# ikergarcia1996/AI-Generated-GTAV

Hardware: AMD Instinct MI355X
Metric: generated frames/sec (32-frame clip, 100 noise steps) (higher is better)
Workload: dtype fp16 (fp32 accumulate/residual)

## Files before the change

ai-generated-gtav_amd/csrc/api.hip:

```cpp
#include "api_internal.h"

#include <type_traits>

namespace gtav_shared {
thread_local hipEvent_t g_launch_ev[2] = {nullptr, nullptr};
static thread_local char g_err[1024] = "";
void set_error(const char* fmt, ...) {
    va_list ap;
    va_start(ap, fmt);
    vsnprintf(g_err, sizeof(g_err), fmt, ap);
    va_end(ap);
}
const char* last_error() { return g_err; }
}

namespace {
template <class T> struct twin_arg { typedef T type; };
template <> struct twin_arg<const f16*> { typedef const __bf16* type; };
template <> struct twin_arg<f16*> { typedef __bf16* type; };
#define GTAV_TWIN_STRUCT(S)                                                                                                                     \
    static_assert(sizeof(S) == sizeof(gtav_bf16::S) && alignof(S) == alignof(gtav_bf16::S) && std::is_standard_layout<S>::value &&             \
                      std::is_standard_layout<gtav_bf16::S>::value, #S ": the fp16 and the bf16 view differ");                                  \
    template <> struct twin_arg<const S&> { typedef const gtav_bf16::S& type; };                                                                \
    template <> struct twin_arg<const S*> { typedef const gtav_bf16::S* type; };
// ... 260 lines not shown
int gtav_op_gemm_dw_grouped(int32_t n, const void* const* x, const void* const* w, float* const* out, const int32_t* M, const int32_t* N, const int32_t* ldo,
                            int32_t K, void* stream) {
    GTAV_REQUIRE(n >= 1 && n <= GEMM_DW_MAX_GROUPS && x && w && out && M && N && ldo, "op_gemm_dw_grouped: 1 .. %d groups", GEMM_DW_MAX_GROUPS);
    GemmDwGroup g[GEMM_DW_MAX_GROUPS];
    for (int i = 0; i < n; ++i) g[i] = GemmDwGroup{(const f16*)x[i], (const f16*)w[i], out[i], M[i], N[i], ldo[i]};
    return op_ops().gemm_dw_grouped(g, n, K, nullptr, (hipStream_t)stream, false);
}
int gtav_op_gemm_splitk_ln(const void* x, int32_t ldx, const void* w, const float* bias, int32_t M, int32_t N, int32_t K,
                           int32_t splitk, float* parts, float* resid, const float* gate, int32_t gate_stride,
                           int32_t rows_per_gate, void* out_f16, const float* shift, const float* scale, int32_t mod_stride,
                           void* stream) {
    GemmParams g = gemm_params((const f16*)x, ldx, (const f16*)w, M, N, K);
    g.out = parts; g.ldo = N;
    g.splitk = splitk > 0 ? splitk : gemm_choose_splitk(M, N, K);
    RET_IF(op_ops().gemm(g, EPI_PARTIAL, (hipStream_t)stream));
    LnPending pd;
    memset(&pd, 0, sizeof(pd));
    pd.parts = parts; pd.nsplit = g.splitk; pd.slab_stride = (size_t)M * N; pd.ld = N; pd.bias = bias; pd.gate = gate;
    pd.gate_stride = gate_stride; pd.rows_per_gate = rows_per_gate;
    return op_ops().ln_modulate(resid, N, (f16*)out_f16, N, M, N, shift, scale, mod_stride, nullptr, rows_per_gate, &pd, nullptr, (hipStream_t)stream);
}
int gtav_op_ln_pending(int32_t mode, float* x, int32_t ldx, void* out, int32_t M, int32_t D, const float* p0, const float* p1, int32_t mod_stride,
                       const int32_t* rows, int32_t rows_per_mod, const float* parts, int32_t nsplit, int64_t slab_stride, int32_t ld,
                       const float* bias, const float* gate, int32_t gate_stride, const int32_t* gate_rows, int32_t rows_per_gate, float* x_out, void* y_save,
                       int32_t tperm_T, int32_t tperm_P, float* k_save, const float* k_load, int32_t* err, void* stream) {
    LnPending pd;
    memset(&pd, 0, sizeof(pd));
    pd.parts = parts; pd.nsplit = nsplit; pd.slab_stride = (size_t)slab_stride; pd.ld = ld; pd.bias = bias; pd.gate = gate;
    pd.gate_stride = gate_stride; pd.gate_rows = gate_rows; pd.rows_per_gate = rows_per_gate; pd.x_out = x_out; pd.y_save = (f16*)y_save;
    pd.tperm_T = tperm_T; pd.tperm_P = tperm_P; pd.k_save = k_save; pd.k_load = k_load;
    if (mode == 0) return op_ops().ln_modulate(x, ldx, (f16*)out, D, M, D, p0, p1, mod_stride, rows, rows_per_mod, &pd, err, (hipStream_t)stream);
    return op_ops().ln_affine(x, ldx, (f16*)out, D, M, D, p0, p1, &pd, err, (hipStream_t)stream);
}
int gtav_op_branch_rows(const float* parts, int32_t nsplit, int64_t slab_stride, int32_t ld, const float* bias, void* y, int32_t M, int32_t N, int32_t* err,
                        void* stream) {
    return op_ops().branch_rows(parts, nsplit, (size_t)slab_stride, ld, bias, (f16*)y, M, N, err, (hipStream_t)stream);
}
int gtav_op_rope_interleave(const float* cos_t, const float* sin_t, float* cs, int32_t npos, void* stream) {
    return launch_rope_interleave(cos_t, sin_t, cs, npos, (hipStream_t)stream);
}
int gtav_op_gemm_choose_splitk(int32_t M, int32_t N, int32_t K) { return gemm_choose_splitk(M, N, K); }
int gtav_op_gemm_resid_inplace(int32_t M, int32_t N, int32_t K) { return gemm_resid_inplace_ok(M, N, K, 0) ? 1 : 0; }
int gtav_op_gemm_plan(int32_t M, int32_t N, int32_t K, int32_t epilogue, int32_t qkv_mode, int32_t S, int32_t splitk, int32_t rows_per_gate, int32_t* plan8) {
    static_assert(sizeof(gtav_shared::GemmPlan) == 8 * sizeof(int32_t), "plan8 is the GemmPlan");
    GTAV_REQUIRE(plan8, "op_gemm_plan: null argument");
    return gtav_shared::gemm_plan(gtav_shared::GemmProblem{M, N, K, epilogue, qkv_mode, S, splitk, rows_per_gate}, (gtav_shared::GemmPlan*)plan8);
}
void gtav_op_gemm_set_stages(int32_t ns) { gtav_shared::gemm_set_stages(ns); }
#ifdef GTAV_EXPERIMENTS
void gtav_op_gemm_set_debug(int32_t bits) { gtav_shared::gemm_set_debug(bits); }
void gtav_op_gemm_set_stamps(void* buf_dev, int32_t max_blocks) { gemm_set_stamps((unsigned long long*)buf_dev, max_blocks); }
#endif
void gtav_op_gemm_set_wm(int32_t wm) { gtav_shared::gemm_set_wm(wm); }
void gtav_op_set_operand_dtype(int32_t dtype) { g_op_bf16 = dtype == GTAV_OPERAND_BF16; }

int gtav_timer_calibrate(int32_t spin_us, int32_t reps, double* event_us_mean, double* device_us_mean, void* stream) {
    GTAV_REQUIRE(spin_us >= 0 && spin_us <= 1000 && reps >= 1 && reps <= 256 && event_us_mean && device_us_mean, "timer_calibrate: bad argument");
    hipStream_t s = (hipStream_t)stream;
    unsigned long long* dev = nullptr;
    GTAV_CHECK_HIP(hipMalloc(&dev, sizeof(unsigned long long) * reps));
    std::vector<hipEvent_t> ev(2 * reps, nullptr);
    int rc = 0;
    for (int i = 0; i < 2 * reps && !rc; ++i)
        if (hipEventCreate(&ev[i]) != hipSuccess) { set_error("timer_calibrate: hipEventCreate failed"); rc = 1; }
    if (!rc) rc = launch_calib_spin((unsigned long long)spin_us * 100ull, dev, s);
    if (!rc && hipStreamSynchronize(s) != hipSuccess) { set_error("timer_calibrate: synchronize failed"); rc = 1; }
// ... 137 lines not shown
```

ai-generated-gtav_amd/csrc/api_dit.hip:

```cpp
#include "api_internal.h"

#ifdef GTAV_EXPERIMENTS
static int fold_alloc(gtav_dit* h) {
    gtav_dit::Fold& f = h->fold;
    if (f.ok) return 0;
    GTAV_REQUIRE(f.geom_ok, "dit_set_fold: this geometry has no LayerNorm fold (tokens per frame %d must be a multiple of 16 and >= 64, hidden %% 256 == 0)", h->P);
    Arena& a = h->arena;
    const int D = h->D;
    const size_t Mx = round_up(h->Mmax, 128);
    int rc = 0;
#define A_(expr) do { if (!rc) rc = (expr); } while (0)
    {
        const int nhb = h->L * 2, nseam = 2 * nhb + 1;
        f.col_c.assign(nseam, 0);
        int col = 0;
        for (int hb = 0; hb < nhb; ++hb) { f.col_c[2 * hb + 1] = col; col += 2 * h->Hm; }
        for (int hb = 0; hb < nhb; ++hb) { f.col_c[2 * hb] = col; col += 2 * 3 * D; }
        f.col_c[2 * nhb] = col; col += 2 * h->Nfin;
        f.CTW = col;
        f.n_groups = 2 * nseam; f.n_groups_a = 2 * nhb;
        f.Rp = round_up(h->max_rows, 128);
        A_(a.alloc_t(&f.ctab, (size_t)h->max_rows * f.CTW));
        A_(a.alloc_t(&f.ctab_cur, (size_t)h->maxB * h->maxT * f.CTW));
        A_(a.alloc_t(&f.stats, Mx * (size_t)(D / 64) * 2));
// ... 92 lines not shown
    const gtav_dit* h;
    int M, Tq, t0;
    bool on;
    DitPrefetch(const gtav_dit* h_, int M_, int Tq_, int t0_) : h(h_), M(M_), Tq(Tq_), t0(t0_) {
        const int pf_max_m = 1536;
        static const int pf_min_m = GTAV_ENV_INT("GTAV_PF_MIN_M", 256);
        on = h->w_prefetch && M >= pf_min_m && M <= pf_max_m;
        fill_on = M <= pf_max_m;
    }
    bool fill_on;
    int fill(int cls) const { return fill_on ? h->w_fill_cls[cls] : 0; }
    PrefetchDesc after(int hb, int pos) const {
        const int q = pos + 1, hb2 = hb + q / 4, consumer = (q + 3) % 4;
        if (!on || hb2 >= 2 * h->L) return kNoPrefetch;
        const int v = h->w_prefetch_cls[consumer];
        if (!v) return kNoPrefetch;
        const gtav_dit::Half& w2 = h->halves[hb2];
        const int D = h->D;
        const f16* W; int N, K, sk = 1;
        if (consumer == 3) { W = dit_half_fused(h, hb2, M, Tq, t0) ? w2.w_qkv_hm : w2.w_qkv; N = 3 * D; K = D; }
        else if (consumer == 0) { W = w2.w_out; N = D; K = D; sk = gemm_choose_splitk(M, D, D); }
        else if (consumer == 1) { W = w2.w_fc1; N = h->Hm; K = D; }
        else { W = w2.w_fc2; N = D; K = h->Hm_pad; sk = gemm_choose_splitk(M, D, h->Hm_pad); }
        const int nkt = K / 64;
        if (sk < 1 || nkt % sk || (sk >= 8 ? sk % 8 : 8 % sk)) sk = 1;
        return PrefetchDesc{W, cdiv(N, 128), nkt, sk, v >= 2 ? v : 0};
    }
};

static bool dit_resid_inplace(const gtav_dit* h, int M, int K) {
    return gemm_pp_ok(M, h->D, K, EPI_RESID) || (gemm_choose_splitk(M, h->D, K) == 1 && M >= h->resid_inplace_min_m) || gemm_resid_inplace_ok(M, h->D, K, h->P);
}

static int dit_forward_core(gtav_dit* h, const float* x_src, const int* frame_index, int B, int Tq, int t0,
                            const float* mod, const int* mod_rows, const float* ctab, float* v_out, hipStream_t s) {
    const int D = h->D, P = h->P, NB = B * Tq, M = NB * P;
    GTAV_REQUIRE(M <= h->Mmax, "forward: %d tokens exceed workspace (%d)", M, h->Mmax);
    bool fold_a, fold_b;
    fold_policy(h, M, fold_a, fold_b);
    const DitPrefetch pf(h, M, Tq, t0);
    DeferredResid rd{h->parts, h->parts_rows * (size_t)D, h->resid, M, D, &h->prof, s};
    auto gate = [&](const float* g) { return ResidGate{g, h->MODW, mod_rows, P}; };
    auto ln = [&](const OperandOps& o, const float* shift, const float* scale, int* ef) -> int {
        PROF(h, PC_LN, s, o.ln_modulate(h->resid, D, h->xn, D, M, D, shift, scale, h->MODW, mod_rows, P, rd.take(), ef, s));
        return 0;
    };
    const int g_embed = 2 * h->L, g_final = 2 * h->L + 1;
    PROF(h, PC_OTHER, s, h->ops(g_embed).patchify(x_src, frame_index, NB, h->C, h->H, h->W, h->p, h->xp, h->Kpe, 1.f, 0.f, h->err_of(g_embed), s));
    GemmParams pe = gemm_params(h->xp, h->Kpe, h->w_pe, M, D, h->Kpe);
    pe.bias = h->b_pe; pe.out = h->resid; pe.ldo = D;
    PROF(h, PC_OTHER, s, h->ops(g_embed).gemm(pe, EPI_F32, s));
    bool folded_in = false;
    for (int hb = 0; hb < 2 * h->L; ++hb) {
        const int l = hb / 2, hf = hb % 2;
        const gtav_dit::Half& w = h->halves[hb];
        const OperandOps& ops = h->ops(hb);
        int* const ef = h->err_of(hb);
        const float* mb = mod + (size_t)hb * 6 * D;
        const bool fused = dit_half_fused(h, hb, M, Tq, t0), fused_t = fused && hf == 1, fused_s = fused && hf == 0 && !folded_in;
        if (fused_t) rd.permute_rows(Tq, P);
        if (!folded_in) RET_IF(ln(ops, mb, mb + D, ef));
        GemmParams g = gemm_params(h->xn, D, fused_t || fused_s ? w.w_qkv_hm : w.w_qkv, M, 3 * D, D);
        g.D = D; g.S = P; g.err_flag = ef; g.pf = pf.after(hb, 0); g.wfill = pf.fill(3);
        if (folded_in) fold_consumer(h, g, 2 * hb, 3 * D, mod_rows, ctab);
        if (hf == 0) { g.qkv_mode = QKV_SPATIAL; g.rope_cs = h->rope_s.cs_dev; }
        else { g.qkv_mode = QKV_TEMPORAL; g.k = h->kvcache[l]; g.v = h->kvcache[l]; g.Tq = Tq; g.t0 = t0; g.Tmax = h->maxT; g.rope_cs = h->rope_t.cs_dev; }
        if (fused_t || fused_s) {
            g.out = h->ao; g.ldo = D;
            if (fused_t) PROF(h, PC_ATTN_T, s, launch_gemm_qkvt_attn(g, s));
            else PROF(h, PC_ATTN_S, s, launch_gemm_qkvs_attn(g, s));
        } else {
            if (hf == 0) { g.q = h->qs; g.k = h->ks; g.v = h->vts; }
            else g.q = h->qt;
            PROF(h, PC_QKV, s, ops.gemm(g, folded_in ? EPI_QKV_FOLD : EPI_QKV, s));
            if (hf == 0) PROF(h, PC_ATTN_S, s, ops.attn_spatial(h->qs, h->ks, h->vts, h->ao, NB, h->heads, P, s, false));
            else PROF(h, PC_ATTN_T, s, ops.attn_temporal(h->qt, h->kvcache[l], h->ao, B, P, D, Tq, t0, h->maxT, s));
        }
        folded_in = false;
        GemmParams fc1 = gemm_params(h->xn, D, w.w_fc1, M, h->Hm, D);
        fc1.bias = w.b_fc1; fc1.out = h->hbuf; fc1.ldo = h->Hm_pad; fc1.err_flag = ef; fc1.pf = pf.after(hb, 2); fc1.wfill = pf.fill(1);
        if (fold_a) {
            RET_IF(fold_producer(h, PC_OUT, h->ao, w.w_out, M, D, w.b_out, gate(mb + 2 * D), mb + 4 * D, s));
            fold_consumer(h, fc1, 2 * hb + 1, h->Hm, mod_rows, ctab);
            PROF(h, PC_FC1, s, launch_gemm(fc1, EPI_GELU_TANH_FOLD, s));
        } else {
            RET_IF(rd.gemm(ops, PC_OUT, h->ao, D, w.w_out, D, w.b_out, gate(mb + 2 * D), dit_resid_inplace(h, M, D), pf.after(hb, 1), nullptr, nullptr, pf.fill(0)));
            RET_IF(ln(ops, mb + 3 * D, mb + 4 * D, ef));
            PROF(h, PC_FC1, s, ops.gemm(fc1, EPI_GELU_TANH, s));
        }
        if (fold_b) {
            const float* next_scale = hb + 1 < 2 * h->L ? mod + (size_t)(hb + 1) * 6 * D + D : mod + (size_t)h->L * 12 * D + D;
            RET_IF(fold_producer(h, PC_FC2, h->hbuf, w.w_fc2, M, h->Hm_pad, w.b_fc2, gate(mb + 5 * D), next_scale, s));
            folded_in = true;
        } else {
            RET_IF(rd.gemm(ops, PC_FC2, h->hbuf, h->Hm_pad, w.w_fc2, h->Hm_pad, w.b_fc2, gate(mb + 5 * D), dit_resid_inplace(h, M, h->Hm_pad), pf.after(hb, 3), nullptr, nullptr, pf.fill(2)));
        }
    }
    const float* mf = mod + (size_t)h->L * 12 * D;
    if (!folded_in) RET_IF(ln(h->ops(g_final), mf, mf + D, h->err_of(g_final)));
    GemmParams fin = gemm_params(h->xn, D, h->w_final, M, h->Nfin, D);
    fin.bias = h->b_final; fin.out = h->fo; fin.ldo = h->Nfin;
    if (folded_in) fold_consumer(h, fin, 4 * h->L, h->Nfin, mod_rows, ctab);
    PROF(h, PC_OTHER, s, h->ops(g_final).gemm(fin, folded_in ? EPI_F32_FOLD : EPI_F32, s));
    PROF(h, PC_OTHER, s, launch_unpatchify(h->fo, h->Nfin, v_out, NB, h->C, h->H, h->W, h->p, 0, 1.f, 0.f, s));
    return h->prof.collect(s);
}

extern "C" {

int gtav_dit_create(const gtav_dit_config* c, gtav_dit** out) {
    GTAV_REQUIRE(c && out, "dit_create: null argument");
    GTAV_REQUIRE(c->hidden_size % 256 == 0 && c->hidden_size <= 2048, "hidden_size=%d must be a multiple of 256, <= 2048", c->hidden_size);
    GTAV_REQUIRE(c->num_heads > 0 && c->hidden_size / c->num_heads == 64 && c->hidden_size % c->num_heads == 0,
                 "only head_dim 64 is implemented (hidden %d, heads %d)", c->hidden_size, c->num_heads);
    GTAV_REQUIRE(c->input_h % c->patch_size == 0 && c->input_w % c->patch_size == 0, "input %dx%d not divisible by patch %d",
                 c->input_h, c->input_w, c->patch_size);
    GTAV_REQUIRE(c->max_frames >= 1 && c->max_frames <= 32, "max_frames=%d must be in [1, 32]", c->max_frames);
    GTAV_REQUIRE(c->max_batch >= 1 && c->depth >= 1, "bad max_batch/depth");
    RET_IF(skinny_init());
    gtav_dit* h = new gtav_dit();
    h->cfg = *c;
    h->D = c->hidden_size; h->L = c->depth; h->heads = c->num_heads; h->C = c->in_channels; h->p = c->patch_size;
    h->H = c->input_h; h->W = c->input_w; h->gh = h->H / h->p; h->gw = h->W / h->p; h->P = h->gh * h->gw;
    const int D = h->D;
    if ((h->P % 8) != 0) {
        set_error("tokens per frame P=%d must be a multiple of 8", h->P);
        delete h;
        return 2;
    }
    h->Hm = (int)(D * c->mlp_ratio); h->Hm_pad = round_up(h->Hm, 128);
    h->A = c->external_cond_dim > 0 ? c->external_cond_dim : 0; h->Apad = round_up(h->A > 0 ? h->A : 1, 32);
    h->MODW = h->L * 12 * D + 2 * D;
    h->Kpe = round_up(h->C * h->p * h->p, 64);
    h->Nfin = h->p * h->p * h->C;
    h->maxB = c->max_batch; h->maxT = c->max_frames; h->Mmax = h->maxB * h->maxT * h->P;
    h->max_rows = c->max_cond_rows > h->maxB * h->maxT ? c->max_cond_rows : h->maxB * h->maxT;
    Arena& a = h->arena;
// ... 143 lines not shown
    }
    RET_IF(launch_rope_interleave(h->rope_s.cos_dev, h->rope_s.sin_dev, h->rope_s.cs_dev, h->P, s));
    RET_IF(launch_rope_interleave(h->rope_t.cos_dev, h->rope_t.sin_dev, h->rope_t.cs_dev, h->maxT, s));
    GTAV_CHECK_HIP(hipStreamSynchronize(s));
    h->finalized = true;
    return 0;
}

int gtav_dit_forward(gtav_dit* h, const float* x, const int64_t* t, const float* actions, float* out, int32_t B, int32_t T,
                     void* stream) {
    GTAV_REQUIRE(h && x && t && out, "dit_forward: null argument");
    GTAV_REQUIRE(h->finalized, "dit_forward: call gtav_dit_finalize first");
    GTAV_REQUIRE(B >= 1 && B <= h->maxB && T >= 1 && T <= h->maxT, "dit_forward: B=%d T=%d outside capacity (%d, %d)", B, T, h->maxB, h->maxT);
    GTAV_REQUIRE(!actions || h->A > 0, "dit_forward: model has no external_cond");
    hipStream_t s = (hipStream_t)stream;
    h->prepared.valid = false;
    h->kvrec.valid = false;
    RET_IF(dit_cond(h, t, B * T, 1, nullptr, 0, actions, h->A, 0, s));
    return dit_forward_core(h, x, nullptr, B, T, 0, h->mod, nullptr, h->fold.ctab, out, s);
}

int gtav_dit_set_schedule(gtav_dit* h, const float* ac, int32_t n) {
    GTAV_REQUIRE(h && ac && n == 1000, "dit_set_schedule: expected 1000 alphas_cumprod values");
    h->ac_host.assign(ac, ac + n);
    GTAV_CHECK_HIP(hipMemcpy(h->ac_table, ac, n * sizeof(float), hipMemcpyHostToDevice));
    return 0;
}

static int denoise_step_body(gtav_dit* h, float* x, int B, int F, int T, const float* actions, int mode, float* v_out,
                             bool prepared, hipStream_t s) {
    const size_t fsz = (size_t)h->C * h->H * h->W;
    const int Tq = mode == 1 ? 1 : T, t0 = mode == 1 ? T - 1 : 0;
    if (!prepared) RET_IF(dit_cond(h, nullptr, B * Tq, Tq, h->step_dev, mode == 1, actions, (int64_t)F * h->A, h->A, s));
    RET_IF(dit_forward_core(h, x, h->frame_idx, B, Tq, t0, prepared ? h->mod_cur : h->mod, nullptr, prepared ? h->fold.ctab_cur : h->fold.ctab, h->vout, s));
    const float* vlast = h->vout + (size_t)(Tq - 1) * fsz;
    RET_IF(launch_ddim_update_step(x, F, vlast, (size_t)Tq * fsz, B, (int)fsz, h->step_dev, s));
    if (v_out) RET_IF(launch_copy_rows_f32(vlast, (size_t)Tq * fsz, v_out, fsz, B, fsz, s));
    return 0;
}

int gtav_dit_prepare_frame(gtav_dit* h, int32_t B, int32_t F, int32_t start, int32_t cur, int32_t t_ctx,
                           const int32_t* t_steps_host, int32_t n_steps, const float* actions, void* stream) {
    GTAV_REQUIRE(h && t_steps_host, "prepare_frame: null argument");
    GTAV_REQUIRE(h->finalized, "prepare_frame: finalize the model first");
    const int T = cur - start + 1;
    GTAV_REQUIRE(start >= 0 && cur < F && T >= 1 && T <= h->maxT && B >= 1 && B <= h->maxB && n_steps >= 1 && n_steps <= 1024,
                 "prepare_frame: bad window [%d, %d] / steps %d", start, cur, n_steps);
    GTAV_REQUIRE(!actions || h->A > 0, "prepare_frame: model has no external_cond");
    const int rows = B * (T - 1) + n_steps * B;
    GTAV_REQUIRE(rows <= h->max_rows, "prepare_frame: %d conditioning rows exceed max_cond_rows %d", rows, h->max_rows);
    hipStream_t s = (hipStream_t)stream;
    GTAV_CHECK_HIP(hipStreamSynchronize(s));
    GTAV_CHECK_HIP(hipMemcpy(h->t_steps_dev, t_steps_host, n_steps * sizeof(int), hipMemcpyHostToDevice));
    RET_IF(launch_cond_inputs_frame(rows, B, T, F, start, cur, t_ctx, h->t_steps_dev, h->sincos, h->E, actions, h->A, h->HC, h->D + h->Apad,
                                    h->D, h->Apad, h->err_flag, s));
    RET_IF(dit_cond_mlp(h, rows, actions != nullptr, s));
    {
        bool fa, fb, fa1, fb1;
        fold_policy(h, B * T * h->P, fa, fb);
        fold_policy(h, B * h->P, fa1, fb1);
        RET_IF(dit_fold_tables(h, rows, fa || fa1, fb || fb1, s));
        h->prepared.fold_tables = fa || fa1 || fb || fb1;
    }
    GTAV_CHECK_HIP(hipMemsetAsync(h->mod_last, 0xFF, (size_t)h->maxB * h->maxT * sizeof(int), s));
    h->prepared.valid = true; h->prepared.B = B; h->prepared.F = F; h->prepared.start = start; h->prepared.cur = cur;
    h->prepared.n_steps = n_steps; h->prepared.actions = actions;
    return 0;
// ... 70 lines not shown

int gtav_dit_set_graph(gtav_dit* h, int32_t enable) {
    GTAV_REQUIRE(h, "dit_set_graph: null handle");
    h->use_graph = enable != 0;
    return 0;
}

int gtav_dit_set_weight_prefetch(gtav_dit* h, int32_t enable) {
    GTAV_REQUIRE(h, "dit_set_weight_prefetch: null handle");
    GTAV_REQUIRE(enable == 0 || enable == 1 || (enable >> 16) == 1,
                 "dit_set_weight_prefetch: mode %d (0 off, 1 on, 0x10000 | per-class nibbles: bits 0-3 out-proj's weight, 4-7 fc1's, 8-11 fc2's, 12-15 to_qkv's; "
                 "nibble 0 = not prefetched, 1 = the whole slice, k >= 2 = the first k K tiles of every row tile)", enable);
    int cls[4];
    for (int c = 0; c < 4; ++c) cls[c] = enable == 0 ? 0 : enable == 1 ? 1 : (enable >> (4 * c)) & 15;
    const bool on = cls[0] || cls[1] || cls[2] || cls[3];
    if (h->w_prefetch != on || memcmp(cls, h->w_prefetch_cls, sizeof(cls))) h->drop_graphs();
    h->w_prefetch = on;
    memcpy(h->w_prefetch_cls, cls, sizeof(cls));
    return 0;
}

int gtav_dit_set_weight_fill_policy(gtav_dit* h, int32_t mode) {
    GTAV_REQUIRE(h, "dit_set_weight_fill_policy: null handle");
    GTAV_REQUIRE((mode & ~0x1111) == 0,
                 "dit_set_weight_fill_policy: mode %d (one nibble per class: bits 0-3 out-proj's weight, 4-7 fc1's, 8-11 fc2's, 12-15 to_qkv's; "
                 "nibble 0 = default cache policy, 1 = non-temporal fills)", mode);
    int cls[4];
    for (int c = 0; c < 4; ++c) cls[c] = (mode >> (4 * c)) & 15;
    if (memcmp(cls, h->w_fill_cls, sizeof(cls))) h->drop_graphs();
    memcpy(h->w_fill_cls, cls, sizeof(cls));
    return 0;
}

#ifdef GTAV_EXPERIMENTS
int gtav_dit_set_fold(gtav_dit* h, int32_t mode, int32_t min_tokens_a, int32_t min_tokens_b) {
    GTAV_REQUIRE(h && mode >= 0 && mode <= 2, "dit_set_fold: mode %d", mode);
    if (min_tokens_a >= 0) h->fold.min_m_a = min_tokens_a;
    if (min_tokens_b >= 0) h->fold.min_m_b = min_tokens_b;
    if (mode == 2 || (mode == 1 && (h->fold.min_m_a < (1 << 30) || h->fold.min_m_b < (1 << 30)))) RET_IF(fold_alloc(h));
    h->drop_graphs();
    h->prepared.valid = false;
    h->fold.mode = mode;
    return 0;
}
#endif

static int dit_set_fused(gtav_dit* h, bool& flag, int hf, bool geom_ok, bool enable) {
    if (flag != enable) h->drop_graphs();
    if (enable && geom_ok) {
        for (int l = 0; l < h->L; ++l) {
            gtav_dit::Half& w = h->halves[l * 2 + hf];
            if (w.w_qkv_hm) continue;
            RET_IF(h->arena.alloc_t(&w.w_qkv_hm, (size_t)3 * h->D * h->D));
            if (h->finalized) RET_IF(launch_qkv_head_major(w.w_qkv, w.w_qkv_hm, h->D, nullptr, hf ? 0 : 1));
        }
        if (h->finalized) GTAV_CHECK_HIP(hipDeviceSynchronize());
    }
    flag = enable;
    return 0;
}
int gtav_dit_set_fused_temporal(gtav_dit* h, int32_t enable) {
    GTAV_REQUIRE(h, "dit_set_fused_temporal: null handle");
    return dit_set_fused(h, h->fuse_tattn, 1, h->P % 16 == 0 && h->D % 256 == 0 && h->maxT >= 5, enable != 0);
}
int gtav_dit_set_fused_spatial(gtav_dit* h, int32_t enable) {
    GTAV_REQUIRE(h, "dit_set_fused_spatial: null handle");
// ... 96 lines not shown
```

ai-generated-gtav_amd/csrc/api_internal.h:

```cpp
#pragma once
#include "../../include/gtav_amd.h"
#include "../../include/gtav_amd_testing.h"
#include "ops.h"
#include "ops_bf16.h"

#include <cmath>
#include <cstdarg>
#include <cstdio>
#include <cstdlib>
#include <cstring>
#include <map>
#include <string>
#include <tuple>
#include <vector>

using namespace gtav;

#define RET_IF(expr)            \
    do {                        \
        int _rc = (expr);       \
        if (_rc) return _rc;    \
    } while (0)

namespace gtav {
// ... 202 lines not shown
#define PROF(h, c, s, expr)            \
    do {                               \
        RET_IF((h)->prof.begin(c, s)); \
        RET_IF(expr);                  \
        RET_IF((h)->prof.end(s));      \
    } while (0)

inline int report_err_flag(int flag, const char* who) {
    GTAV_REQUIRE(!(flag & ERR_TIMESTEP), "%s: a timestep outside [0, 999] was passed", who);
    GTAV_REQUIRE(!(flag & ERR_NONFINITE), "%s: a NaN or inf was found in the input tensor", who);
    GTAV_REQUIRE(!(flag & ERR_F16_SAT), "%s: an activation exceeded the fp16 range (|x| > 65504) and was saturated; results since the "
                 "last check are finite but clipped (the reference runs this path in bf16, which has fp32 range)", who);
    return 0;
}

inline GemmParams gemm_params(const f16* X, int ldx, const f16* W, int M, int N, int K) {
    GemmParams g;
    memset(&g, 0, sizeof(g));
    g.X = X; g.ldx = ldx; g.W = W; g.M = M; g.N = N; g.K = K;
    return g;
}

const PrefetchDesc kNoPrefetch{nullptr, 0, 0, 0, 0};

struct ResidGate { const float* gate; int stride; const int* rows; int rows_per_gate; };
struct DeferredResid {
    float* parts; size_t parts_floats;
    float* resid;
    int M, N;
    Profiler* prof;
    hipStream_t s;
    LnPending pend;
    bool pending = false;
    int gemm(const OperandOps& ops, int cls, const f16* X, int ldx, const f16* W, int K, const float* bias, const ResidGate& gt, bool inplace,
             const PrefetchDesc& pf = kNoPrefetch, float* x_out = nullptr, f16* y_save = nullptr, int wfill = 0) {
        GemmParams q = gemm_params(X, ldx, W, M, N, K);
        q.out = parts; q.ldo = N; q.pf = pf; q.wfill = wfill;
        if (inplace) {
            q.out = resid; q.bias = bias; q.gate = gt.gate; q.gate_stride = gt.stride; q.gate_rows = gt.rows; q.rows_per_gate = gt.rows_per_gate;
        } else {
            q.splitk = gemm_choose_splitk(M, N, K);
            GTAV_REQUIRE((size_t)q.splitk * M * N <= parts_floats, "split-K slabs exceed workspace");
        }
        if (prof) RET_IF(prof->begin(cls, s));
        RET_IF(ops.gemm(q, inplace ? EPI_RESID : EPI_PARTIAL, s));
        if (prof) RET_IF(prof->end(s));
        pending = !inplace;
        if (inplace) return 0;
        memset(&pend, 0, sizeof(pend));
        pend.parts = parts; pend.nsplit = q.splitk; pend.slab_stride = (size_t)M * N; pend.ld = N; pend.bias = bias;
        pend.gate = gt.gate; pend.gate_stride = gt.stride; pend.gate_rows = gt.rows; pend.rows_per_gate = gt.rows_per_gate;
        pend.x_out = x_out; pend.y_save = y_save;
        return 0;
    }
    const LnPending* take() {
        const bool was = pending;
        pending = false;
        return was ? &pend : nullptr;
    }
    void permute_rows(int T, int P) {
        if (!pending) memset(&pend, 0, sizeof(pend));
        pend.tperm_T = T; pend.tperm_P = P;
        pending = true;
    }
    void save_shift(float* k) { pend.k_save = k; }
    int load_shift(const float* k) {
        GTAV_REQUIRE(!pending, "train_block_forward: a re-run starts from a stored block input");
        memset(&pend, 0, sizeof(pend));
        pend.k_load = k;
        pending = true;
// ... 20 lines not shown
    bool sincos_set = false;
    RopeTable rope_s, rope_t;
    std::vector<float> freqs_s, freqs_t;
    float *freqs_s_dev = nullptr, *freqs_t_dev = nullptr;
    f16 *xp, *xn, *qs, *ks, *vts, *qt, *ao, *hbuf;
    std::vector<f16*> kvcache;
    float *resid, *fo, *vout, *E, *HC, *Sc, *mod, *parts;
    size_t parts_rows = 0;
    int* err_flag = nullptr;
    std::vector<unsigned char> grp_bf16;
    int n_groups = 0;
    bool any_bf16 = false;
    const OperandOps& ops(int g) const { return operand_ops(grp_bf16[g] != 0); }
    int* err_of(int g) const { return err_flag + 4 + g; }
    int* frame_idx = nullptr;
    StepParams* step_dev = nullptr;
    int* mod_rows_dev = nullptr;
    float* mod_cur = nullptr;
    int *mod_last = nullptr, *mod_changed = nullptr;
    int* t_steps_dev = nullptr;
    struct { bool valid = false, fold_tables = false; int B = 0, F = 0, start = 0, cur = 0, n_steps = 0; const float* actions = nullptr; } prepared;
    struct { bool valid = false; int B = 0, F = 0, start = 0, cur = 0; const void* x = nullptr; } kvrec;
    struct GraphKey {
        int B, F, T, mode;
        const void *x, *actions, *vout;
        bool operator<(const GraphKey& o) const {
            return std::tie(B, F, T, mode, x, actions, vout) < std::tie(o.B, o.F, o.T, o.mode, o.x, o.actions, o.vout);
        }
    };
    std::map<GraphKey, hipGraphExec_t> graphs;
    bool use_graph = true;
    bool fuse_tattn = false;
    bool fuse_sattn = false;
    bool w_prefetch = true;
    int w_prefetch_cls[4] = {1, 4, 4, 1};
    int w_fill_cls[4] = {0, 0, 0, 0};
    int resid_inplace_min_m = GTAV_ENV_INT("GTAV_RESID_INPLACE_MIN_M", 1 << 30);
    struct Fold {
        bool geom_ok = false;
        bool ok = false;
        int mode = 1;
        int min_m_a = 1 << 30, min_m_b = 1 << 30;
        int CTW = 0, n_groups = 0, n_groups_a = 0, Rp = 0;
        std::vector<int> col_c;
        float *ctab = nullptr, *ctab_cur = nullptr, *stats = nullptr;
        f16* sx = nullptr;
        GemmGroup* groups_dev = nullptr;
        int *gcol_dev = nullptr, *gscale_dev = nullptr;
    } fold;
    hipStream_t cap_stream = nullptr;
    void drop_graphs() {
        for (auto& kv : graphs)
            if (kv.second) (void)hipGraphExecDestroy(kv.second);
        graphs.clear();
    }
    ~gtav_dit() {
        drop_graphs();
        if (cap_stream) (void)hipStreamDestroy(cap_stream);
    }
    float* ac_table = nullptr;
    std::vector<float> ac_host;
    bool finalized = false;
    struct Train {
        bool on = false, have_fwd = false, have_actions = false;
        bool bf16 = false;
        bool mixed = false;
// ... 37 lines not shown
```

ai-generated-gtav_amd/csrc/common.h:

```cpp
#pragma once
#include <hip/hip_runtime.h>
#include <hip/hip_fp16.h>
#include <hip/hip_ext.h>
#include <stdint.h>

#ifdef GTAV_BF16_OPERANDS
#define GTAV_F16_T __bf16
#else
#define GTAV_F16_T _Float16
#endif

namespace gtav {

typedef GTAV_F16_T f16;
typedef GTAV_F16_T f16x4 __attribute__((ext_vector_type(4)));
typedef GTAV_F16_T f16x8 __attribute__((ext_vector_type(8)));
typedef GTAV_F16_T f16x2 __attribute__((ext_vector_type(2)));
typedef float f32x4 __attribute__((ext_vector_type(4)));
typedef float f32x16 __attribute__((ext_vector_type(16)));

__device__ __forceinline__ f32x4 mfma16(f16x8 a, f16x8 b, f32x4 c, int, int, int) {
#ifdef GTAV_BF16_OPERANDS
    return __builtin_amdgcn_mfma_f32_16x16x32_bf16(a, b, c, 0, 0, 0);
#else
// ... 50 lines not shown
#define GTAV_REQUIRE(cond, ...)                                                           \
    do {                                                                                  \
        if (!(cond)) {                                                                    \
            gtav::set_error(__VA_ARGS__);                                                 \
            return 2;                                                                     \
        }                                                                                 \
    } while (0)

#ifdef GTAV_EXPERIMENTS
#define GTAV_ENV_INT(name, dflt) (getenv(name) ? atoi(getenv(name)) : (dflt))
#define GTAV_DBG(p, bits) ((p).debug & (bits))
#define GTAV_LAB_BUILD true
#else
#define GTAV_ENV_INT(name, dflt) (dflt)
#define GTAV_DBG(p, bits) false
#define GTAV_LAB_BUILD false
#endif

static inline int cdiv(int a, int b) { return (a + b - 1) / b; }
static inline int round_up(int a, int b) { return cdiv(a, b) * b; }

__host__ __device__ __forceinline__ size_t tiled_off(int r, int k, int K) {
    return ((size_t)(r >> 7) * (size_t)(K >> 6) + (size_t)(k >> 6)) * 8192 + (size_t)((r & 127) * 64) +
           (size_t)(((((k >> 3) & 7) ^ (r & 7)) << 3) + (k & 7));
}

}
namespace gtav_shared {
struct PrefetchDesc {
    const void* next;
    int rt, nkt, splitk;
    int kt_limit;
};
}
namespace gtav {
using gtav_shared::PrefetchDesc;
__device__ __forceinline__ void l2_prefetch_slice(const PrefetchDesc& d, int xcd, int j, int nb, int t, int nt, unsigned& sink) {
    const int sk = d.splitk;
    int ks0, ksn, rt0, rtn;
    if (sk >= 8) {
        ksn = sk >> 3; ks0 = xcd * ksn; rt0 = 0; rtn = d.rt;
    } else {
        const int per = 8 / sk, part = xcd % per;
        ks0 = xcd / per; ksn = 1;
        rt0 = part * d.rt / per; rtn = (part + 1) * d.rt / per - rt0;
    }
    const int kpt = d.nkt / sk;
    const int lim = d.kt_limit > 0 && d.kt_limit < kpt ? d.kt_limit : kpt;
    const int per_rt = ksn * lim;
    const int lines = rtn * per_rt * 128;
    const int l0 = (int)((long long)lines * j / nb), l1 = (int)((long long)lines * (j + 1) / nb);
    for (int l = l0 + t; l < l1; l += nt) {
        const int tile = l >> 7, r = tile / per_rt, rem = tile - r * per_rt, sl = rem / lim, k = rem - sl * lim;
        const char* a = (const char*)d.next + ((size_t)(rt0 + r) * d.nkt + (size_t)(ks0 + sl) * kpt + k) * 16384 + (l & 127) * 128;
        asm volatile("global_load_dword %0, %1, off" : "+v"(sink) : "v"(a) : "memory");
    }
}
static inline bool prefetch_desc_ok(const PrefetchDesc& d) {
    return !d.next || (d.rt > 0 && d.nkt > 0 && d.splitk >= 1 && d.nkt % d.splitk == 0 && (d.splitk >= 8 ? d.splitk % 8 == 0 : 8 % d.splitk == 0));
}

#ifdef GTAV_BF16_OPERANDS
constexpr float F16_MAX = 3.3895313892515355e38f;
#else
constexpr float F16_MAX = 65504.0f;
#endif
constexpr int ERR_TIMESTEP = 1, ERR_F16_SAT = 2, ERR_NONFINITE = 4;
__device__ __forceinline__ f16x4 sat4(float a, float b, float c, float d, float& amax) {
    amax = __builtin_fmaxf(__builtin_fmaxf(__builtin_fabsf(a), __builtin_fabsf(b)), amax);
// ... 129 lines not shown
```

ai-generated-gtav_amd/csrc/elementwise.hip:

```cpp
#include "ops.h"

#include <cstdlib>
#include <type_traits>

#include <cstring>

namespace gtav {

namespace {

template <int MODE, int NV>
__global__ __launch_bounds__(256) void ln_wave_row_kernel(const float* __restrict__ x, int ldx, f16* __restrict__ out, int M, int D,
                                                          const float* __restrict__ p0, const float* __restrict__ p1, int mod_stride,
                                                          const int* __restrict__ rows, int rows_per_mod, int flags, int* err_flag) {
    const int lane = threadIdx.x & 63;
    const int m = blockIdx.x * 4 + (threadIdx.x >> 6);
    if (m >= M) return;
    const float* xr = x + (size_t)m * ldx;
    f32x4 v[NV], av[NV], bv[NV];
#pragma unroll
    for (int i = 0; i < NV; ++i) v[i] = *(const f32x4*)(xr + i * 256 + lane * 4);
    const float *a, *b;
    if (MODE == 0) {
        int row = m / rows_per_mod;
// ... 15 lines not shown
    for (int i = 0; i < NV; ++i) {
        const float a0 = v[i][0] - kshift, a1 = v[i][1] - kshift, a2 = v[i][2] - kshift, a3 = v[i][3] - kshift;
        s1 += (a0 + a1) + (a2 + a3);
        s2 += (a0 * a0 + a1 * a1) + (a2 * a2 + a3 * a3);
    }
    const float t1 = wave_sum_dpp(s1), t2 = wave_sum_dpp(s2);
    const float m1 = t1 / (float)D;
    const float var = fmaxf(t2 / (float)D - m1 * m1, 0.f);
    const float rstd = 1.0f / sqrtf(var + 1e-6f);
    float amax = 0.f;
#pragma unroll
    for (int i = 0; i < NV; ++i) {
        float yv[4];
#pragma unroll
        for (int e = 0; e < 4; ++e) {
            const float xh = ((v[i][e] - kshift) - m1) * rstd;
            if (MODE == 0) {
                const float sc = av[i][e] + 1e-6f;
                yv[e] = xh * (1.0f + sc) + bv[i][e];
            } else {
                yv[e] = xh * av[i][e] + bv[i][e];
            }
        }
        store_f16x4_paired<1>(out + tiled_off(m, i * 256 + lane * 4, D), sat4(yv[0], yv[1], yv[2], yv[3], amax), lane, flags & 2);
    }
    sat_report(amax, err_flag);
}

#ifdef GTAV_EXPERIMENTS
#define LN_DBG(pd, b) ((pd).flags & (b))
#else
#define LN_DBG(pd, b) false
#endif
template <int MODE, bool PEND, int KS = 0>
__global__ __launch_bounds__(512) void ln_row_block_kernel(float* __restrict__ x, int ldx, int D, const float* __restrict__ h_parts, size_t h_slab_stride, int h_ld,
                                                           int h_nsplit, int h_flags, int rows_per_mod, f16* __restrict__ out, int M,
                                                           const float* __restrict__ p0, const float* __restrict__ p1,
                                                           int mod_stride, const int* __restrict__ rows,
                                                           LnPending pd) {
    __shared__ float red[16];
    pd.parts = h_parts; pd.slab_stride = h_slab_stride; pd.ld = h_ld; pd.nsplit = h_nsplit; pd.flags = h_flags;
    const int m = blockIdx.x;
    const int c = threadIdx.x * 4;
    const int nw = (blockDim.x + 63) >> 6, wid = threadIdx.x >> 6, lane = threadIdx.x & 63;
    float* xr = x + (size_t)m * ldx;
    const bool act = c < D;
    const bool nt = PEND && (pd.flags & 4);
    f32x4 v = f32x4{0.f, 0.f, 0.f, 0.f}, av = v, bv = v;
    if (act) v = nt ? __builtin_nontemporal_load((const f32x4*)(xr + c)) : *(const f32x4*)(xr + c);
    f32x4 sl[8];
    int nchunk = 0;
    if (PEND && act) {
        const float* pp = pd.parts + (size_t)m * pd.ld + c;
        auto slab = [&](int sp) -> f32x4 {
            const f32x4* q = (const f32x4*)(pp + (size_t)sp * pd.slab_stride);
            return nt ? __builtin_nontemporal_load(q) : *q;
        };
        nchunk = pd.nsplit <= 1 ? 1 : pd.nsplit <= 2 ? 2 : pd.nsplit <= 4 ? 4 : 8;
        if (nchunk == 1) {
            sl[0] = slab(0);
        } else if (nchunk == 2) {
#pragma unroll
            for (int sp = 0; sp < 2; ++sp) sl[sp] = slab(sp < pd.nsplit ? sp : 0);
        } else if (nchunk == 4) {
#pragma unroll
            for (int sp = 0; sp < 4; ++sp) sl[sp] = slab(sp < pd.nsplit ? sp : 0);
        } else {
#pragma unroll
            for (int sp = 0; sp < 8; ++sp) sl[sp] = slab(sp < pd.nsplit ? sp : 0);
        }
    }
    int row = 0, gr = 0;
    if (MODE == 0) {
        row = m / rows_per_mod;
        if (rows && !LN_DBG(pd, 0x2000)) row = rows[row];
// ... 108 lines not shown
    const int x = m % gw, y = (m / gw) % gh, nb = m / (gw * gh);
    const int f = frame_index ? frame_index[nb] : nb;
    const float* base = img + ((size_t)f * C * H + (size_t)y * p) * W + x * p;
    int flags = 0;
    for (int k = 4 * threadIdx.x; k < ldo; k += 4 * blockDim.x) {
        float v[4] = {0.f, 0.f, 0.f, 0.f};
        if (k < Kp) {
            const int c = k / pp, rem = k - c * pp, ph = rem / p, pw = rem - ph * p;
            const float4 t = *(const float4*)(base + ((size_t)c * H + ph) * W + pw);
            v[0] = a * t.x + b; v[1] = a * t.y + b; v[2] = a * t.z + b; v[3] = a * t.w + b;
#pragma unroll
            for (int e = 0; e < 4; ++e)
                if (!(__builtin_fabsf(v[e]) <= F16_MAX)) {
                    flags |= (v[e] != v[e] || __builtin_isinf(v[e])) ? ERR_NONFINITE : ERR_F16_SAT;
                    if (v[e] == v[e]) v[e] = __builtin_amdgcn_fmed3f(v[e], -F16_MAX, F16_MAX);
                }
        }
        *(f16x4*)(out + tiled_off(m, k, ldo)) = f16x4{(f16)v[0], (f16)v[1], (f16)v[2], (f16)v[3]};
    }
    if (flags && err_flag) atomicOr(err_flag, flags);
}

__global__ void unpatchify_kernel(const float* __restrict__ y, int ldy, float* __restrict__ img, int NB, int C, int H, int W,
                                  int p, int order, float a, float b) {
    const int gh = H / p, gw = W / p;
    const size_t total = (size_t)NB * C * H * W;
    for (size_t idx = (size_t)blockIdx.x * blockDim.x + threadIdx.x; idx < total; idx += (size_t)gridDim.x * blockDim.x) {
        const int xx = (int)(idx % W), yy = (int)((idx / W) % H), c = (int)((idx / ((size_t)W * H)) % C);
        const int nb = (int)(idx / ((size_t)W * H * C));
        const int ph = yy % p, pw = xx % p;
        const size_t m = ((size_t)nb * gh + yy / p) * gw + xx / p;
        const int f = order == 0 ? (ph * p + pw) * C + c : (c * p + ph) * p + pw;
        img[idx] = a * y[m * ldy + f] + b;
    }
}

__global__ void convert_pad_f16_kernel(const float* __restrict__ src, int lds, int R, int C, f16* __restrict__ dst, int Rp,
                                       int Cp, float scale, int tiled, int* err_flag) {
    const size_t total = (size_t)Rp * Cp;
    bool sat = false;
    for (size_t idx = (size_t)blockIdx.x * blockDim.x + threadIdx.x; idx < total; idx += (size_t)gridDim.x * blockDim.x) {
        const int c = (int)(idx % Cp);
        const size_t r = idx / Cp;
        float v = 0.f;
        if (r < (size_t)R && c < C) v = src[r * lds + c] * scale;
        if (v == v) {
            sat |= __builtin_fabsf(v) > F16_MAX;
            v = __builtin_amdgcn_fmed3f(v, -F16_MAX, F16_MAX);
        }
        dst[tiled ? tiled_off((int)r, c, Cp) : idx] = (f16)v;
    }
    if (sat && err_flag) atomicOr(err_flag, ERR_F16_SAT);
}

__global__ void copy_f32_kernel(const float* __restrict__ src, int lds, int R, int C, float* __restrict__ dst, int ldd, int c0) {
    const size_t total = (size_t)R * C;
    for (size_t idx = (size_t)blockIdx.x * blockDim.x + threadIdx.x; idx < total; idx += (size_t)gridDim.x * blockDim.x) {
        const int c = (int)(idx % C);
        const size_t r = idx / C;
        dst[r * ldd + c0 + c] = src[r * lds + c];
    }
}

__global__ void rope_interleave_kernel(const float* cos_t, const float* sin_t, float* cs, int npos) {
    const int i = blockIdx.x * blockDim.x + threadIdx.x;
    if (i < npos * 32) {
// ... 402 lines not shown
    const int nd = (int)(i / cpr), kc = (int)(i - (size_t)nd * cpr);
    const int hd = nd / 192, rem = nd - hd * 192;
    int which, d;
    if (mode == 0) {
        which = rem >> 6;
        d = rem & 63;
    } else {
        const int w = rem / 48, r48 = rem - w * 48;
        which = r48 >> 4;
        d = 16 * w + (r48 & 15);
    }
    const int ns = which * D + hd * 64 + d;
    *(uint4*)(dst + tiled_off(nd, kc * 8, D)) = *(const uint4*)(src + tiled_off(ns, kc * 8, D));
}

__global__ void calib_spin_kernel(unsigned long long ticks, unsigned long long* __restrict__ dev_ticks) {
    const unsigned long long t0 = __builtin_amdgcn_s_memrealtime();
    unsigned long long t1 = t0;
    while (t1 - t0 < ticks) {
        __builtin_amdgcn_s_sleep(2);
        t1 = __builtin_amdgcn_s_memrealtime();
    }
    if (threadIdx.x == 0) dev_ticks[0] = t1 - t0;
}

}

static int g_ln_flags = GTAV_ENV_INT("GTAV_LN_FLAGS", 7);

static int g_ln_wave_row_min = GTAV_ENV_INT("GTAV_LN_WAVE_ROW_MIN", 0);

#define LN_WAVE_ROW_(MODE, NV, P0, P1, STRIDE, ROWS, RPM) \
    GTAV_LAUNCH((ln_wave_row_kernel<MODE, NV>), dim3(cdiv(M, 4)), dim3(256), 0, stream, x, ldx, out, M, D, P0, P1, STRIDE, ROWS, RPM, pd_.flags, err_flag)
#define LN_ROW_BLOCK_ARGS_(P0, P1, STRIDE, ROWS, RPM) x, ldx, D, pd_.parts, pd_.slab_stride, pd_.ld, pd_.nsplit, pd_.flags, RPM, out, M, P0, P1, STRIDE, ROWS, pd_
#define LN_DISPATCH(MODE, P0, P1, STRIDE, ROWS, RPM)                                                     \
    do {                                                                                                  \
        LnPending pd_;                                                                                    \
        memset(&pd_, 0, sizeof(pd_));                                                                     \
        if (pend) pd_ = *pend;                                                                            \
        pd_.flags = g_ln_flags;                                                                           \
        pd_.err_flag = err_flag;                                                                          \
        GTAV_REQUIRE(pd_.tperm_T == 0 || (pd_.tperm_P % 16 == 0 && M % (pd_.tperm_T * pd_.tperm_P) == 0), "ln: bad output row permutation"); \
        const bool upd_ = pend && pend->parts;    \
        GTAV_REQUIRE(!pd_.k_save || (upd_ && !pd_.k_load), "ln: k_save needs a pending update and excludes k_load");                          \
        GTAV_REQUIRE(!pd_.k_load || !upd_, "ln: k_load excludes a pending update");                                                            \
        if (pd_.k_save || pd_.k_load) {                  \
            const dim3 g_(M), b_(round_up(D / 4, 64));                                                    \
            if (pd_.k_save) GTAV_LAUNCH((ln_row_block_kernel<MODE, true, 1>), g_, b_, 0, stream, LN_ROW_BLOCK_ARGS_(P0, P1, STRIDE, ROWS, RPM)); \
            else GTAV_LAUNCH((ln_row_block_kernel<MODE, false, 2>), g_, b_, 0, stream, LN_ROW_BLOCK_ARGS_(P0, P1, STRIDE, ROWS, RPM));      \
        } else if (!upd_ && pd_.tperm_T == 0 && M >= g_ln_wave_row_min && (D == 256 || D == 512 || D == 1024 || D == 2048)) { \
            if (D == 256) LN_WAVE_ROW_(MODE, 1, P0, P1, STRIDE, ROWS, RPM);                               \
            else if (D == 512) LN_WAVE_ROW_(MODE, 2, P0, P1, STRIDE, ROWS, RPM);                          \
            else if (D == 1024) LN_WAVE_ROW_(MODE, 4, P0, P1, STRIDE, ROWS, RPM);                         \
            else LN_WAVE_ROW_(MODE, 8, P0, P1, STRIDE, ROWS, RPM);                                        \
        } else {                                                                   \
            const dim3 g_(M), b_(round_up(D / 4, 64));                                                    \
            if (upd_) GTAV_LAUNCH((ln_row_block_kernel<MODE, true>), g_, b_, 0, stream, LN_ROW_BLOCK_ARGS_(P0, P1, STRIDE, ROWS, RPM)); \
            else GTAV_LAUNCH((ln_row_block_kernel<MODE, false>), g_, b_, 0, stream, LN_ROW_BLOCK_ARGS_(P0, P1, STRIDE, ROWS, RPM));     \
        }                                                                                                 \
    } while (0)

int launch_ln_modulate(float* x, int ldx, f16* out, int ldo, int M, int D, const float* shift, const float* scale,
                       int mod_stride, const int* rows, int rows_per_mod, const LnPending* pend, int* err_flag, hipStream_t stream) {
    GTAV_REQUIRE(D % 64 == 0 && D <= 2048 && rows_per_mod > 0 && ldo == D, "ln_modulate: D=%d must be %%64, <= 2048, ldo == D", D);
    GTAV_REQUIRE(!pend || !pend->parts || (pend->nsplit >= 1 && pend->nsplit <= 8 && pend->ld % 4 == 0 && (!pend->gate || pend->rows_per_gate > 0)),
                 "ln_modulate: bad pending update");
    LN_DISPATCH(0, shift, scale, mod_stride, rows, rows_per_mod);
    GTAV_CHECK_HIP(hipGetLastError());
    return 0;
}

int launch_ln_affine(float* x, int ldx, f16* out, int ldo, int M, int D, const float* gamma, const float* beta,
                     const LnPending* pend, int* err_flag, hipStream_t stream) {
    GTAV_REQUIRE(D % 64 == 0 && D <= 2048 && ldo == D, "ln_affine: D=%d must be %%64, <= 2048, ldo == D", D);
    GTAV_REQUIRE(!pend || !pend->parts || (pend->nsplit >= 1 && pend->nsplit <= 8 && pend->ld % 4 == 0 && (!pend->gate || pend->rows_per_gate > 0)),
                 "ln_affine: bad pending update");
    LN_DISPATCH(1, gamma, beta, 0, (const int*)nullptr, 1);
    GTAV_CHECK_HIP(hipGetLastError());
    return 0;
}
#undef LN_DISPATCH
#undef LN_WAVE_ROW_

int launch_branch_rows(const float* parts, int nsplit, size_t slab_stride, int ld, const float* bias, f16* y, int M, int N, int* err_flag, hipStream_t stream) {
    GTAV_REQUIRE(parts && y && nsplit >= 1 && nsplit <= 8 && M > 0 && N > 0 && N % 4 == 0 && ld % 4 == 0 && N <= ld && slab_stride >= (size_t)M * ld,
                 "branch_rows: bad slabs (nsplit=%d, M=%d, N=%d, ld=%d)", nsplit, M, N, ld);
    const size_t n4 = (size_t)M * (N / 4);
    hipLaunchKernelGGL(branch_rows_kernel, dim3((unsigned)cdiv((long long)n4, 256)), dim3(256), 0, stream, parts, nsplit, slab_stride, ld, bias, y, N, n4, err_flag);
    GTAV_CHECK_HIP(hipGetLastError());
    return 0;
}

int launch_patchify(const float* img, const int* frame_index, int NB, int C, int H, int W, int p, f16* out, int ldo,
                    float a, float b, int* err_flag, hipStream_t stream) {
    GTAV_REQUIRE(H % p == 0 && W % p == 0 && ldo >= C * p * p, "patchify: bad geometry");
    const size_t total = (size_t)NB * (H / p) * (W / p) * ldo;
    if (p % 4 == 0 && W % 4 == 0 && ldo % 4 == 0 && ((uintptr_t)img & 15) == 0 && (size_t)NB * (H / p) * (W / p) < (1u << 31)) {
        hipLaunchKernelGGL(patchify4_kernel, dim3(NB * (H / p) * (W / p)), dim3(256), 0, stream, img, frame_index, C, H, W, p, out, ldo, a, b, err_flag);
        GTAV_CHECK_HIP(hipGetLastError());
        return 0;
    }
    hipLaunchKernelGGL(patchify_kernel, dim3(grid_for(total)), dim3(256), 0, stream, img, frame_index, NB, C, H, W, p, out,
                       ldo, a, b, err_flag);
    GTAV_CHECK_HIP(hipGetLastError());
    return 0;
}

int launch_unpatchify(const float* y, int ldy, float* img, int NB, int C, int H, int W, int p, int order, float a,
                      float b, hipStream_t stream) {
    GTAV_REQUIRE(H % p == 0 && W % p == 0 && ldy >= C * p * p, "unpatchify: bad geometry");
    const size_t total = (size_t)NB * C * H * W;
    hipLaunchKernelGGL(unpatchify_kernel, dim3(grid_for(total)), dim3(256), 0, stream, y, ldy, img, NB, C, H, W, p, order,
                       a, b);
    GTAV_CHECK_HIP(hipGetLastError());
    return 0;
}

int launch_convert_pad_f16(const float* src, int lds, int R, int C, f16* dst, int Rp, int Cp, float scale, int tiled,
                           hipStream_t stream, int* err_flag) {
    GTAV_REQUIRE(Rp >= R && Cp >= C, "convert_pad: padded shape smaller than source");
    GTAV_REQUIRE(!tiled || (Rp % 128 == 0 && Cp % 64 == 0), "convert_pad: tile-major needs Rp %% 128 == 0 and Cp %% 64 == 0");
    hipLaunchKernelGGL(convert_pad_f16_kernel, dim3(grid_for((size_t)Rp * Cp)), dim3(256), 0, stream, src, lds, R, C, dst,
                       Rp, Cp, scale, tiled, err_flag);
    GTAV_CHECK_HIP(hipGetLastError());
    return 0;
}

int launch_qkv_head_major(const f16* src, f16* dst, int D, hipStream_t stream, int mode) {
    GTAV_REQUIRE(D % 128 == 0 && (mode == 0 || mode == 1), "qkv_head_major: D=%d must be a multiple of 128, mode=%d 0 or 1", D, mode);
    const size_t total = (size_t)3 * D * (D / 8);
    hipLaunchKernelGGL(qkv_head_major_kernel, dim3((unsigned)cdiv((long long)total, 256)), dim3(256), 0, stream, src, dst, D, mode);
    GTAV_CHECK_HIP(hipGetLastError());
    return 0;
}

int launch_copy_f32(const float* src, int lds, int R, int C, float* dst, int ldd, int c0, hipStream_t stream) {
    hipLaunchKernelGGL(copy_f32_kernel, dim3(grid_for((size_t)R * C)), dim3(256), 0, stream, src, lds, R, C, dst, ldd, c0);
    GTAV_CHECK_HIP(hipGetLastError());
    return 0;
}

int launch_rope_interleave(const float* cos_t, const float* sin_t, float* cs, int npos, hipStream_t stream) {
    hipLaunchKernelGGL(rope_interleave_kernel, dim3(cdiv(npos * 32, 256)), dim3(256), 0, stream, cos_t, sin_t, cs, npos);
    GTAV_CHECK_HIP(hipGetLastError());
    return 0;
}

int launch_fill_f32(float* dst, size_t n, float v, hipStream_t stream) {
    hipLaunchKernelGGL(fill_f32_kernel, dim3(grid_for(n)), dim3(256), 0, stream, dst, n, v);
    GTAV_CHECK_HIP(hipGetLastError());
// ... 177 lines not shown
```

ai-generated-gtav_amd/csrc/gemm.hip:

```cpp
#include "gemm.h"
#include "attn_tile.h"

#include <cstdlib>
#include <cstring>
#include <type_traits>
#include <hip/hip_ext.h>

namespace gtav {
using namespace gtav_shared;

namespace {

constexpr int TN = 128, TK = 64;
constexpr int TILE_BYTES = 128 * TK * 2;

typedef const __attribute__((address_space(1))) void* gptr_t;
typedef __attribute__((address_space(3))) void* lptr_t;

__device__ __forceinline__ void glds16(const char* src, char* lds_wave_base) {
    __builtin_amdgcn_global_load_lds((gptr_t)src, (lptr_t)lds_wave_base, 16, 0, 0);
}

__device__ __forceinline__ void glds16_s(const void* sbase, unsigned voff, unsigned lds_addr) {
    unsigned keep;
// ... 792 lines not shown

template <int EPIX, int FI, int WM, int WN = 2, int WOFF = 0>
__device__ __forceinline__ void prefetch_bias(const GemmParams& p, int n0, f32x4 (&pbias)[FI]) {
    constexpr int EPI = epi_base(EPIX);
    const int w = (int)(threadIdx.x >> 6) - WOFF;
    const int lane = threadIdx.x & 63, wn = w % WN, g = lane >> 4;
#pragma unroll
    for (int i = 0; i < FI; ++i) {
        const int n = n0 + 16 * FI * wn + 16 * i + 4 * g;
        pbias[i] = f32x4{0.f, 0.f, 0.f, 0.f};
        if (EPI != EPI_PARTIAL && p.bias && n < p.N && w >= 0 && w < WN * WM) pbias[i] = *(const f32x4*)(p.bias + n);
    }
}

template <int FI, int FJ, int WM, int WN = 2, int WOFF = 0>
__device__ __forceinline__ void prefetch_resid(const GemmParams& p, int n0, int m0, f32x4 (&xpre)[FI][FJ], int qlo, int qhi) {
    const int lane = threadIdx.x & 63, w = (int)(threadIdx.x >> 6) - WOFF;
    const int wn = w % WN, wm = w / WN, li = lane & 15, g = lane >> 4;
    const bool cw = w >= 0 && w < WN * WM;
#pragma unroll
    for (int i = 0; i < FI; ++i) {
        const int n = n0 + 16 * FI * wn + 16 * i + 4 * g;
#pragma unroll
        for (int j = 0; j < FJ; ++j) {
            const int q = i * FJ + j;
            if (q < qlo || q >= qhi) continue;
            const int m = m0 + 16 * FJ * wm + 16 * j + li;
            xpre[i][j] = f32x4{0.f, 0.f, 0.f, 0.f};
            if (cw && n < p.N && m < p.M) xpre[i][j] = *(const f32x4*)((const float*)p.out + (size_t)m * p.ldo + n);
        }
    }
}

template <int EPIX, int FI, int FJ, int WM, int WN = 2, int WOFF = 0, bool PRE = false>
__device__ __forceinline__ void epilogue(const GemmParams& p, f32x4 (&acc)[FI][FJ], const f32x4 (&pbias)[FI], char* smem, int n0, int m0, int ks, bool tr,
                                         const f32x4 (&prope)[FI][FJ], FoldTok<FJ>& ft) {
    constexpr int EPI = epi_base(EPIX);
    constexpr bool FOLD = epi_is_fold_consumer(EPIX);
    constexpr int TM = WM * 16 * FJ, TNB = 16 * FI * WN;
    constexpr int CT = 16 * FI * WN / 64;
    const int lane = threadIdx.x & 63, wraw = threadIdx.x >> 6, w = wraw - WOFF;
    const int wn = w % WN, wm = w / WN, li = lane & 15, g = lane >> 4;
    const bool compute_wave = w >= 0 && w < WN * WM;
    float amax = 0.f;

    if constexpr (EPI == EPI_RESID_FOLD) {
        static_assert(EPI != EPI_RESID_FOLD || (FI == 2 || FI == 4), "a 64-feature statistics slot is one wave (FI = 4) or two (FI = 2)");
        constexpr int WPS = 4 / FI;
        float2* sc = (float2*)(smem + CT * TM * 128);
        __syncthreads();
        if (compute_wave) {
            int rowA, rowB, boundary;
            fold_frames(p, __builtin_amdgcn_readfirstlane(m0 + 16 * FJ * wm), rowA, rowB, boundary);
            const float *gA = p.gate + (size_t)rowA * p.gate_stride, *gB = p.gate + (size_t)rowB * p.gate_stride;
            const float *sA = p.f_scale + (size_t)rowA * p.gate_stride, *sB = p.f_scale + (size_t)rowB * p.gate_stride;
            float s1[FJ], s2[FJ];
#pragma unroll
            for (int j = 0; j < FJ; ++j) s1[j] = 0.f, s2[j] = 0.f;
#pragma unroll
            for (int i = 0; i < FI; ++i) {
                const int nl = 16 * FI * wn + 16 * i + 4 * g;
                const int n = n0 + nl;
                const bool nok = n < p.N;
                const int nc = nok ? n : 0;
                const f32x4 bv = pbias[i];
                f32x4 gA4, gB4, sA4, sB4;
                if (GTAV_DBG(p, 0x100000)) {
// ... 85 lines not shown
                        const float* cf = (const float*)ft.cb + fold_frame_of(ft, m0 + 16 * FJ * wm + 16 * j) * 2 * TNB + nl;
                        v = fold_apply(acc[i][j], ft.mu[j], ft.rs[j], *(const f32x4*)cf, *(const f32x4*)(cf + TNB));
                    } else {
                        v = acc[i][j] + bv;
                    }
                    if constexpr (EPI == EPI_GELU_TANH)
                        {
                            if (GTAV_DBG(p, 16384)) {
                                *(uint2*)dst = pack4(amax, gelu_tanh_f(v[0]), gelu_tanh_f(v[1]), gelu_tanh_f(v[2]), gelu_tanh_f(v[3]));
                            } else {
                                const float xin[4] = {v[0], v[1], v[2], v[3]};
                                float yo[4];
                                gelu_tanh_f4(xin, yo);
                                *(uint2*)dst = pack4(amax, yo[0], yo[1], yo[2], yo[3]);
                            }
                        }
                    else if constexpr (EPI == EPI_GELU_ERF) {
                        const float xin[4] = {v[0], v[1], v[2], v[3]};
                        float yo[4];
                        gelu_erf_f4(xin, yo);
                        *(uint2*)dst = pack4(amax, yo[0], yo[1], yo[2], yo[3]);
                    } else
                        *(uint2*)dst = pack4(amax, v[0], v[1], v[2], v[3]);
                }
            }
        }
        sat_report(amax, p.err_flag);
        __syncthreads();
        const int nkt_out = p.ldo >> 6, last_rt = (p.M - 1) >> 7;
        constexpr int PR = TM / 8;
        auto copy_out = [&](void* out) {
            for (int q = wraw; q < CT * PR; q += (int)(blockDim.x >> 6)) {
                const int cs = q / PR, pq = q - cs * PR;
                const int gr = m0 + 8 * pq;
                const int rt = gr >> 7;
                if (rt > last_rt || (n0 >> 6) + cs >= nkt_out) continue;
                const uint4 val = *(const uint4*)(smem + (cs * TM + 8 * pq) * 128 + lane * 16);
                char* dst = (char*)out + ((size_t)rt * nkt_out + (n0 >> 6) + cs) * TILE_BYTES + ((gr & 127) >> 3) * 1024 + lane * 16;
                if (p.out_sc1) store16q_sc1(dst, val);
                else *(uint4*)dst = val;
            }
        };
        copy_out(p.out);
        if constexpr (EPI == EPI_F16_TILED && !FOLD) {
            if (p.out2) {
                __syncthreads();
                if (compute_wave) {
                    float dummy = 0.f;
#pragma unroll
                    for (int i = 0; i < FI; ++i) {
                        const int nl = 16 * FI * wn + 16 * i + 4 * g;
                        const f32x4 bv = pbias[i];
                        const int c = nl & 63;
#pragma unroll
                        for (int j = 0; j < FJ; ++j) {
                            const int ml = 16 * FJ * wm + 16 * j + li;
                            char* dst = smem + ((nl >> 6) * TM + ml) * 128 + (((c >> 3) ^ (ml & 7)) << 4) + (c & 7) * 2;
                            const f32x4 v = acc[i][j] + bv;
                            const f16x4 u16 = sat4(v[0], v[1], v[2], v[3], dummy);
                            *(uint2*)dst = pack4(dummy, gelu_tanh_f((float)u16[0]), gelu_tanh_f((float)u16[1]), gelu_tanh_f((float)u16[2]), gelu_tanh_f((float)u16[3]));
                        }
                    }
                }
                __syncthreads();
                copy_out(p.out2);
            }
        }
        return;
    }
// ... 85 lines not shown
#pragma unroll
        for (int i = 0; i < FI; ++i) {
            if (i + 1 < FI) loads(i + 1, xo[(i + 1) & 1], gt[(i + 1) & 1]);
            const int n = n0 + 16 * FI * wn + 16 * i + 4 * g;
#pragma unroll
            for (int j = 0; j < FJ; ++j) {
                const int m = m0 + 16 * FJ * wm + 16 * j + li;
                if (n < p.N && m < p.M) {
                    const f32x4 x = xo[i & 1][j] + gt[i & 1][j] * (acc[i][j] + pbias[i]);
                    float* dst = (float*)p.out + (size_t)m * p.ldo + n;
                    if (p.out_sc1) store16_sc1(dst, x);
                    else *(f32x4*)dst = x;
                }
            }
        }
        return;
    }
#pragma unroll
    for (int i = 0; i < FI; ++i) {
        const int n = n0 + 16 * FI * wn + 16 * i + 4 * g;
        if (n >= p.N) continue;
        const f32x4 bv = pbias[i];
        int which = 0, nn = n, head = 0, d = 0;
        if constexpr (EPI == EPI_QKV) {
            which = n >= 2 * p.D ? 2 : (n >= p.D ? 1 : 0);
            nn = n - which * p.D;
            head = nn >> 6;
            d = nn & 63;
        }
#pragma unroll
        for (int j = 0; j < FJ; ++j) {
            const int m = m0 + 16 * FJ * wm + 16 * j + li;
            if (m >= p.M) continue;
            f32x4 v;
            if constexpr (FOLD) {
                const float* cf = (const float*)ft.cb + fold_frame_of(ft, m0 + 16 * FJ * wm + 16 * j) * 2 * TNB + (n - n0);
                v = fold_apply(acc[i][j], ft.mu[j], ft.rs[j], *(const f32x4*)cf, *(const f32x4*)(cf + TNB));
            } else {
                v = acc[i][j] + bv;
            }
            if constexpr (EPI == EPI_PARTIAL) {
                float* dst = (float*)p.out + ((size_t)ks * p.M + m) * p.ldo + n;
                if (p.out_sc1) store16_sc1(dst, v);
                else *(f32x4*)dst = v;
            } else if constexpr (EPI == EPI_F32) {
                *(f32x4*)((float*)p.out + (size_t)m * p.ldo + n) = v;
            } else if constexpr (EPI == EPI_F16) {
                *(uint2*)((f16*)p.out + (size_t)m * p.ldo + n) = pack4(amax, v[0], v[1], v[2], v[3]);
            } else if constexpr (EPI == EPI_QKV) {
                if (which < 2) {
                    const f32x4 cs = *(const f32x4*)(rope_tab(p, n) + tok_pos[j] * 64 + d);
                    v = rope4(v, cs);
                }
                const uint2 pk = pack4(amax, v[0], v[1], v[2], v[3]);
                if (p.qkv_mode == QKV_SPATIAL) {
                    const int heads = p.D >> 6;
                    f16* base = which == 0 ? p.q : p.k;
                    f16* dst = base + ((size_t)(tok_a[j] * heads + head) * p.S + tok_b[j]) * 64 + d;
                    *(uint2*)dst = pk;
                } else {
                    if (which == 0) {
                        *(uint2*)(p.q + (size_t)m * p.D + nn) = pk;
                    } else {
                        f16* base = p.k + (size_t)tok_a[j] * 2 * p.D + (which == 2 ? p.D : 0);
                        *(uint2*)(base + nn) = pk;
                    }
                }
            }
        }
    }
    if constexpr (EPI == EPI_F16 || EPI == EPI_QKV) sat_report(amax, p.err_flag);
}

template <int EPIX, int FI, int FJ, int WM, int WN = 2, int WOFF = 0>
__device__ __forceinline__ void epilogue(const GemmParams& p, f32x4 (&acc)[FI][FJ], const f32x4 (&pbias)[FI], char* smem, int n0, int m0, int ks, bool tr) {
    static_assert(!epi_is_fold_consumer(EPIX), "a fold consumer passes its prefetched FoldTok");
    FoldTok<FJ> ft;
    epilogue<EPIX, FI, FJ, WM, WN, WOFF, false>(p, acc, pbias, smem, n0, m0, ks, tr, acc, ft);
}
// ... 371 lines not shown
    bs.end(p);
}

template <int NS, int FI, int FJ, int WM>
__global__ __launch_bounds__(128 * WM, 1) void gemm_grouped_kernel(GemmParams p0, const GemmGroup* __restrict__ groups) {
    constexpr int TNB = 32 * FI, TM = 16 * FJ * WM;
    constexpr int STAGE = (4 * FI + 2 * FJ * WM) * 1024;
    __shared__ __attribute__((aligned(16))) char smem[NS * STAGE];
    GemmParams p = p0;
    {
        const GemmGroup* gr = groups + blockIdx.y;
        p.X = gr->X; p.W = gr->W; p.out = gr->out; p.bias = gr->bias; p.N = gr->N; p.ldo = gr->ldo;
    }
    const int tiles_m = (p.M + TM - 1) / TM, tiles_n = (p.N + TNB - 1) / TNB, tiles = tiles_m * tiles_n;
    const int bid = blockIdx.x;
    if (bid >= tiles) return;
    const int xcd = bid & 7, qq = tiles >> 3, rr = tiles & 7;
    const bool inrange = (bid >> 3) < qq + (xcd < rr ? 1 : 0);
    const int tile_id = inrange ? (xcd < rr ? xcd * (qq + 1) : rr * (qq + 1) + (xcd - rr) * qq) + (bid >> 3) : bid;
    const int tile_m = tile_id / tiles_n, tile_n = tile_id - tile_m * tiles_n;
    const int n0 = tile_n * TNB, m0 = tile_m * TM;
    BlockStamps bs;
    f32x4 acc[FI][FJ];
#pragma unroll
    for (int i = 0; i < FI; ++i)
#pragma unroll
        for (int j = 0; j < FJ; ++j) acc[i][j] = f32x4{0.f, 0.f, 0.f, 0.f};
    f32x4 pbias[FI];
    auto pf = [&]() { prefetch_bias<EPI_F32, FI, WM>(p, n0, pbias); };
    mainloop_g<false, NS, FI, FJ, WM>(p, smem, n0, m0, 0, p.K / TK, acc, bs, pf);
    epilogue<EPI_F32, FI, FJ, WM>(p, acc, pbias, smem, n0, m0, 0, false);
}

template <bool TR, int NS, int FI, int FJ, int WN, int WM, int NL, int TRI = FI, bool HALFSTEP = (FI * FJ >= 16), typename AfterPrologue>
__device__ __forceinline__ void mainloop_l(const GemmParams& p, char* smem, int n0, int m0, int kt0, int nkt,
                                           f32x4 (&acc)[FI][FJ], BlockStamps& bs, AfterPrologue after_prologue) {
    static_assert(NS >= 3 && NL >= 1, "loader-wave ring: at least 3 stages and one loader wave");
    constexpr int NCW = WN * WM;
    constexpr int WPC = 2 * FI * WN, XPC = 2 * FJ * WM, NP = WPC + XPC;
    constexpr int G = (NP + NL - 1) / NL;
    constexpr int STAGE_BYTES = NP * 1024;
    const int tid = threadIdx.x, lane = tid & 63;
    const int wraw = __builtin_amdgcn_readfirstlane(tid >> 6);
    const int nktot = p.K / TK;
    if (wraw < NL) {
        const int lw = wraw;
        const int last_wt = ((p.N + 127) >> 7) - 1, last_rt = (p.M - 1) >> 7;
        const unsigned voff = (unsigned)lane * 16u;
        const unsigned smem0 = lds_offset(smem);
        const char* sb[G];
        unsigned ldso[G];
        unsigned wmask = 0;
#pragma unroll
        for (int i = 0; i < G; ++i) {
            int q = lw * G + i;
            q = q < NP ? q : NP - 1;
            const bool isw = q < WPC;
            wmask |= (unsigned)isw << i;
            const int row = isw ? n0 + 8 * q : m0 + 8 * (q - WPC);
            int rt = row >> 7;
            const int lim = isw ? last_wt : last_rt;
            rt = rt < lim ? rt : lim;
            sb[i] = (const char*)(isw ? p.W : p.X) + ((size_t)rt * nktot + kt0) * TILE_BYTES + ((row & 127) >> 3) * 1024;
            ldso[i] = smem0 + q * 1024;
        }
        auto stage = [&](int t) {
            const unsigned so = (unsigned)(t % NS) * STAGE_BYTES;
            const size_t go = (size_t)t * TILE_BYTES;
#pragma unroll
            for (int i = 0; i < G; ++i) glds16_s(sb[i] + go, voff, ldso[i] + so);
        };
        const int npro = nkt < NS - 1 ? nkt : NS - 1;
        GTAV_STAMP_SLOT(lw == 0 && lane == 0, 7);
        if (p.wfill) {
            auto stage_nt = [&](int t) {
                const unsigned so = (unsigned)(t % NS) * STAGE_BYTES;
                const size_t go = (size_t)t * TILE_BYTES;
#pragma unroll
                for (int i = 0; i < G; ++i) {
                    if (wmask >> i & 1) glds16_s_nt(sb[i] + go, voff, ldso[i] + so);
                    else glds16_s(sb[i] + go, voff, ldso[i] + so);
                }
            };
            for (int t = 0; t < npro; ++t) stage_nt(t);
            for (int t = 0; t < nkt; ++t) {
                wait_vm_ring<NS, G>(nkt - 1 - t);
                GTAV_STAMP_SLOT_HI(t == 0 && lw == 0 && lane == 0, 6);
                wg_barrier();
                if (t == 0) GTAV_STAMP(bs.t[1]);
                if (t + NS - 1 < nkt) stage_nt(t + NS - 1);
            }
            return;
// ... 79 lines not shown
            __builtin_amdgcn_sched_barrier(0);
        }
        if (domm) mmh(wb, xb);
    } else {
        f16x8 wA[2][FI], xA[2][FJ], wB[2][FI], xB[2][FJ];
        auto step = [&](int t, f16x8 (&wr)[2][FI], f16x8 (&xr)[2][FJ], const f16x8 (&wm_)[2][FI], const f16x8 (&xm_)[2][FJ]) {
            GTAV_STAMP_SLOT(GTAV_DBG(p, 32) && w == 0 && lane == 0 && t < 24, 32 + t);
            wait_lgkm0();
            wg_barrier();
            if (t == 0) GTAV_STAMP(bs.t[1]);
            if (t > 0 && !GTAV_DBG(p, 2)) {
                rd(t, wr, xr);
                mm(wm_, xm_);
                interleave_mfma_dsread<2 * FI * FJ, 2 * (FI + FJ), 1>();
            } else {
                rd(t, wr, xr);
            }
            __builtin_amdgcn_sched_barrier(0);
        };
        int t = 0;
        for (; t + 1 < nkt; t += 2) {
            step(t, wA, xA, wB, xB);
            step(t + 1, wB, xB, wA, xA);
        }
        if (t < nkt) {
            step(t, wA, xA, wB, xB);
            if (!GTAV_DBG(p, 2)) mm(wA, xA);
        } else if (!GTAV_DBG(p, 2)) {
            mm(wB, xB);
        }
    }
}

template <int EPIX, int NS, int FI, int FJ, int WN, int WM, int NL>
__global__ __launch_bounds__(64 * (WN * WM + NL), 1) void gemm_l_kernel(GTAV_HEAD_PARAMS, GemmParams p) {
    constexpr int EPI = epi_base(EPIX);
    constexpr int TNB = 16 * FI * WN, TM = 16 * FJ * WM;
    constexpr int STAGE = (2 * FI * WN + 2 * FJ * WM) * 1024;
    constexpr int PNB = (TNB / 8 + 7) / 8 * 8 * 16, PTB = (TM / 8 + 7) / 8 * 8 * 16;
    constexpr int EPIB = (TM * PNB > TNB * PTB ? TM * PNB : TNB * PTB) + TM * 8 + (epi_is_fold_consumer(EPIX) ? fold_lds_bytes(TNB) : 0);
    extern __shared__ __attribute__((aligned(16))) char smem_l[];
    static_assert(NS * STAGE >= EPIB, "the ring must cover the epilogue's LDS image");
    char* smem = smem_l;
    GTAV_HEAD_APPLY(p);
    auto pin_args = [&]() { asm volatile("" ::"s"(p.bias), "s"(p.out), "s"(p.ldo), "s"(p.qkv_mode), "s"(p.D)); };
    BlockStamps bs;
    bs.begin(p);
    int n0, m0, ks, kt0, nkt;
    tile_map_fast<EPI == EPI_PARTIAL, TNB, TM>(p, n0, m0, ks, kt0, nkt, EPI == EPI_PARTIAL ? p.tm.tiles * p.splitk : p.tm.tiles);
    f32x4 acc[FI][FJ];
#pragma unroll
    for (int i = 0; i < FI; ++i)
#pragma unroll
        for (int j = 0; j < FJ; ++j) acc[i][j] = f32x4{0.f, 0.f, 0.f, 0.f};
    bool tr = false;
    f32x4 pbias[FI];
    constexpr bool FOLDC = epi_is_fold_consumer(EPIX), FOLDP = EPI == EPI_RESID_FOLD;
    FoldTok<FJ> ft;
    auto pff = [&]() {
        if constexpr (FOLDC) {
            const int cw = (int)(threadIdx.x >> 6) - NL;
            fold_prefetch<TNB, TM, FJ>(p, n0, m0, (int)threadIdx.x - 64 * NL, __builtin_amdgcn_readfirstlane(m0 + 16 * FJ * (cw / WN)), cw >= 0, ft);
        }
    };
    if constexpr (EPI == EPI_QKV && FI * FJ <= 6 && WN * WM + NL <= 12) {
        tr = (p.qkv_mode == QKV_SPATIAL) && (n0 >= 2 * p.D);
        f32x4 prope[FI][FJ];
        auto pfq = [&]() {
            pin_args();
            prefetch_bias<EPI, FI, WM, WN, NL>(p, n0, pbias);
            prefetch_rope<FI, FJ, WM, WN, NL>(p, n0, m0, prope);
            pff();
        };
        if (tr) mainloop_l<true, NS, FI, FJ, WN, WM, NL>(p, smem, n0, m0, kt0, nkt, acc, bs, pfq);
        else mainloop_l<false, NS, FI, FJ, WN, WM, NL>(p, smem, n0, m0, kt0, nkt, acc, bs, pfq);
        GTAV_STAMP(bs.t[2]);
        epilogue<EPIX, FI, FJ, WM, WN, NL, true>(p, acc, pbias, smem, n0, m0, ks, tr, prope, ft);
    } else if constexpr (EPI == EPI_QKV) {
        tr = (p.qkv_mode == QKV_SPATIAL) && (n0 >= 2 * p.D);
        auto pf = [&]() { pin_args(); prefetch_bias<EPI, FI, WM, WN, NL>(p, n0, pbias); pff(); };
        if (tr) mainloop_l<true, NS, FI, FJ, WN, WM, NL>(p, smem, n0, m0, kt0, nkt, acc, bs, pf);
        else mainloop_l<false, NS, FI, FJ, WN, WM, NL>(p, smem, n0, m0, kt0, nkt, acc, bs, pf);
        GTAV_STAMP(bs.t[2]);
        epilogue<EPIX, FI, FJ, WM, WN, NL, false>(p, acc, pbias, smem, n0, m0, ks, tr, acc, ft);
    } else if constexpr (FOLDP) {
        f32x4 xpre[FI][FJ];
        auto pf = [&]() { pin_args(); prefetch_bias<EPI, FI, WM, WN, NL>(p, n0, pbias); prefetch_resid<FI, FJ, WM, WN, NL>(p, n0, m0, xpre, 0, FI * FJ); };
        mainloop_l<false, NS, FI, FJ, WN, WM, NL>(p, smem, n0, m0, kt0, nkt, acc, bs, pf);
        GTAV_STAMP(bs.t[2]);
        epilogue<EPIX, FI, FJ, WM, WN, NL, true>(p, acc, pbias, smem, n0, m0, ks, tr, xpre, ft);
    } else {
        auto pf = [&]() { pin_args(); prefetch_bias<EPI, FI, WM, WN, NL>(p, n0, pbias); pff(); };
        mainloop_l<false, NS, FI, FJ, WN, WM, NL>(p, smem, n0, m0, kt0, nkt, acc, bs, pf);
        GTAV_STAMP(bs.t[2]);
        epilogue<EPIX, FI, FJ, WM, WN, NL, false>(p, acc, pbias, smem, n0, m0, ks, tr, acc, ft);
    }
    bs.template end<true>(p);
}

template <int NS>
__global__ __launch_bounds__(512, 1) void gemm_qkvt_attn_kernel(GTAV_HEAD_PARAMS, GemmParams p) {
    constexpr int FI = 3, FJ = 5, WN = 4, WM = 1, NL = 4, TNB = 192, TM = 80, TMAX = 5;
    constexpr int PN = 384;
    extern __shared__ __attribute__((aligned(16))) char smem_l[];
    static_assert(NS * (2 * FI * WN + 2 * FJ * WM) * 1024 >= TM * PN, "the ring must cover the epilogue's LDS image");
    char* smem = smem_l;
    GTAV_HEAD_APPLY(p);
    BlockStamps bs;
    bs.begin(p);
    int n0, m0, ks, kt0, nkt;
    tile_map_fast<false, TNB, TM>(p, n0, m0, ks, kt0, nkt, p.tm.tiles);
    f32x4 acc[FI][FJ];
#pragma unroll
    for (int i = 0; i < FI; ++i)
#pragma unroll
        for (int j = 0; j < FJ; ++j) acc[i][j] = f32x4{0.f, 0.f, 0.f, 0.f};
    mainloop_l<false, NS, FI, FJ, WN, WM, NL>(p, smem, n0, m0, kt0, nkt, acc, bs, []() {});
    GTAV_STAMP(bs.t[2]);
    const int tid = threadIdx.x, lane = tid & 63, w = (tid >> 6) - NL, li = lane & 15, g = lane >> 4;
    const int head = n0 / TNB;
    const int pgs = p.S >> 4, tile_m = m0 / TM, b = tile_m / pgs, pg = tile_m - b * pgs;
    float amax = 0.f;
    __syncthreads();
    if (w >= 0) {
#pragma unroll
        for (int i = 0; i < FI; ++i) {
            const int nl = 16 * FI * w + 16 * i + 4 * g;
            const bool rope = nl < 128;
// ... 407 lines not shown
    }
    if (cus) *cus = n;
    return 0;
}

static int fill_tile_map(GemmParams::TileMap& tm, int M, int N, int tmb, int tnb, int splitk, int gn) {
    tm.tiles_m = cdiv(M, tmb);
    tm.tiles_n = cdiv(N, tnb);
    tm.tiles = tm.tiles_m * tm.tiles_n;
    tm.gn = gn;
    tm.group = tm.tiles_m * tm.gn;
    const int gnlast = tm.tiles_n % tm.gn ? tm.tiles_n % tm.gn : tm.gn;
    auto rcp = [](int d) { return (unsigned)((0x100000000ull + (unsigned)d - 1) / (unsigned)d); };
    GTAV_REQUIRE((long long)tm.tiles * splitk < 65536, "gemm: grid of %d tiles x %d slices is too large for the 32-bit reciprocal tile map", tm.tiles, splitk);
    tm.rcp_tiles = tm.tiles > 1 ? rcp(tm.tiles) : 0;
    tm.rcp_group = tm.group > 1 ? rcp(tm.group) : 0;
    tm.rcp_gn = tm.gn > 1 ? rcp(tm.gn) : 0;
    tm.rcp_gnlast = gnlast > 1 ? rcp(gnlast) : 0;
    return 0;
}

template <int EPI, int SHAPE>
static int launch_plain(const GemmParams& p, const GemmPlan& plan, hipStream_t stream) {
    constexpr GemmShape R = *gemm_shape(SHAPE);
    static_assert(R.wn == 2 && (R.family == GF_G || R.family == GF_T256 || (R.family == GF_K128 && R.features() == TN)), "two waves along the features");
    const dim3 grid(plan.blocks), block(R.threads());
    if constexpr (R.family == GF_G) GEMM_LAUNCH((gemm_g_kernel<EPI, R.ns, R.fi, R.fj, R.wm>), grid, block);
    else if constexpr (R.family == GF_T256) GEMM_LAUNCH((gemm256_kernel<EPI>), grid, block);
    else if (plan.ns <= 2) GEMM_LAUNCH((gemm_kernel<EPI, 2, R.wm, R.fj>), grid, block);
    else GEMM_LAUNCH((gemm_kernel<EPI, 4, R.wm, R.fj>), grid, block);
    GTAV_CHECK_HIP(hipGetLastError());
    return 0;
}
template <int EPI, int SHAPE>
static int launch_l(const GemmParams& p, const GemmPlan& plan, hipStream_t stream) {
    constexpr GemmShape R = *gemm_shape(SHAPE);
    static_assert(R.family == GF_L, "gemm_l_kernel");
    if (int rc_ = lds_opt_in<gemm_l_kernel<EPI, R.ns, R.fi, R.fj, R.wn, R.wm, R.nl>>(R.ring_bytes())) return rc_;
    GemmParams q = p;
    if (int rc_ = fill_tile_map(q.tm, p.M, p.N, R.tokens(), R.features(), plan.splitk, plan.gn)) return rc_;
    GTAV_REQUIRE(q.splitk >= 0 && q.splitk < 256, "gemm: %d K slices do not fit the launch-head arguments", q.splitk);
    GTAV_LAUNCH((gemm_l_kernel<EPI, R.ns, R.fi, R.fj, R.wn, R.wm, R.nl>), dim3(plan.blocks), dim3(R.threads()), R.ring_bytes(), stream, GTAV_HEAD_VALUES(q), q);
    GTAV_CHECK_HIP(hipGetLastError());
    return 0;
}

template <int EPI, int SHAPE>
static int launch_lp(const GemmParams& p, const GemmPlan& plan, hipStream_t stream) {
    constexpr GemmShape R = *gemm_shape(SHAPE);
    static_assert(R.family == GF_LP, "gemm_lp_kernel");
    if constexpr (!(EPI == EPI_GELU_TANH || EPI == EPI_PARTIAL || EPI == EPI_F16_TILED || EPI == EPI_RESID)) {
        GTAV_REQUIRE(false, "gemm: the persistent loader-wave kernel (shape %d) has no epilogue %d", SHAPE, (int)EPI);
    } else {
        constexpr int TNB = R.features(), TM = R.tokens();
        constexpr int LDS = R.ns * (TNB + TM) * 128 + (EPI == EPI_RESID ? 2 * (LP_MAXF + 1) * TNB * 4 : 0);
        GTAV_REQUIRE(plan.splitk == 1 && p.N % 8 == 0, "gemm: the persistent loader-wave kernel runs the whole K in one slice (N %% 8 == 0)");
        if constexpr (EPI == EPI_RESID) GTAV_REQUIRE(!p.gate || (p.rows_per_gate > 0 && (TM - 1) / p.rows_per_gate + 2 <= LP_MAXF), "gemm/resid on the persistent kernel: %d tokens per gate row are too few (a tile may touch at most %d rows)", p.rows_per_gate, LP_MAXF);
        int cus = 0;
        if (int rc_ = lds_opt_in<gemm_lp_kernel<EPI, R.ns, R.fi, R.fj, R.wn, R.wm>>(LDS, &cus)) return rc_;
        GemmParams q = p;
        if (EPI == EPI_RESID && !q.gate) q.rows_per_gate = 1 << 30;
        GTAV_LAUNCH((gemm_lp_kernel<EPI, R.ns, R.fi, R.fj, R.wn, R.wm>), dim3(plan.blocks < cus ? plan.blocks : cus), dim3(R.threads()), LDS, stream, q);
        GTAV_CHECK_HIP(hipGetLastError());
    }
    return 0;
}

#ifdef GTAV_EXPERIMENTS
#include "gemm_experiments.inc"
#endif

template <int EPI>
static int launch_epi(const GemmParams& p, const GemmPlan& plan, hipStream_t stream) {
    const int shape = plan.shape;
    constexpr bool FOLDISH = EPI == EPI_RESID_FOLD || epi_is_fold_consumer(EPI);
    if constexpr (FOLDISH) GTAV_REQUIRE(shape == 2 || shape == 3 || shape == 11 || shape == 12 || shape == 13 || shape == 14 || shape == 20 || shape == 24 || shape == 26 || shape == 27 || shape == 28,
                                        "gemm: block shape %d has no LayerNorm-fold epilogue", shape);
    if (shape == 20) return launch_l<EPI, 20>(p, plan, stream);
    if (shape == 24) return launch_l<EPI, 24>(p, plan, stream);
    if (shape == 26) return launch_l<EPI, 26>(p, plan, stream);
    GTAV_REQUIRE(!p.out2 || (EPI == EPI_F16_TILED && shape != 31), "gemm: a second output image (out2) exists for EPI_F16_TILED on the staged epilogue only (epilogue %d, block shape %d)", (int)EPI, shape);
    if (shape == 31) return launch_lp<EPI, 31>(p, plan, stream);
    if constexpr (!FOLDISH) if (shape == 29) return launch_l<EPI, 29>(p, plan, stream);
    if (shape == 14) return launch_plain<EPI, 14>(p, plan, stream);
    if (shape == 13) return launch_plain<EPI, 13>(p, plan, stream);
    if (shape == 12) return launch_plain<EPI, 12>(p, plan, stream);
    if (shape == 11) return launch_plain<EPI, 11>(p, plan, stream);
    if (shape == 3) return launch_plain<EPI, 3>(p, plan, stream);
    if (shape == 2) return launch_plain<EPI, 2>(p, plan, stream);
    if (shape == 7) {
#ifndef GTAV_EXPERIMENTS
        if constexpr (EPI == EPI_QKV) {
            GTAV_REQUIRE(false, "gemm: the 256 x 256 tile has no QKV epilogue in the product build");
        } else
#endif
        if constexpr (!FOLDISH) return launch_plain<EPI, 7>(p, plan, stream);
    }
#ifdef GTAV_EXPERIMENTS
    return launch_experiment_shape<EPI>(p, plan, stream);
#endif
    GTAV_REQUIRE(false, "gemm: block shape %d has no kernel for epilogue %d", shape, (int)EPI);
    return 0;
}

bool gemm_qkvt_attn_ok(int M, int D, int S, int Tq, int t0) {
    static const int max_blocks = GTAV_ENV_INT("GTAV_QKVT_MAX_BLOCKS", 256);
    return Tq == 5 && t0 == 0 && S % 16 == 0 && D % 64 == 0 && M % (Tq * S) == 0 && (M / 80) * (D / 64) <= max_blocks;
}
int launch_gemm_qkvt_attn(const GemmParams& p_in, hipStream_t stream) {
    GemmParams q = p_in;
    GTAV_REQUIRE(gemm_qkvt_attn_ok(q.M, q.D, q.S, q.Tq, q.t0), "gemm/qkvt_attn: unsupported geometry M=%d D=%d S=%d Tq=%d t0=%d", q.M, q.D, q.S, q.Tq, q.t0);
    GTAV_REQUIRE(q.N == 3 * q.D && q.K % TK == 0 && q.k && q.out && q.rope_cs && q.Tmax >= q.Tq, "gemm/qkvt_attn: missing buffers");
    GTAV_REQUIRE(((uintptr_t)q.X & 15) == 0 && ((uintptr_t)q.W & 15) == 0, "gemm: operands must be 16-byte aligned");
    constexpr int NS = 4, LDS = NS * 34 * 1024;
    if (int rc_ = lds_opt_in<gemm_qkvt_attn_kernel<NS>>(LDS)) return rc_;
    lab_fields(q, 3 | 32 | 512);
    q.out_sc1 = 1;
    q.splitk = 1;
    if (int rc_ = fill_tile_map(q.tm, q.M, q.N, 80, 192, 1, gemm_choose_gn(q.M, q.N, q.K, 80, 192, 1))) return rc_;
    GTAV_LAUNCH((gemm_qkvt_attn_kernel<NS>), dim3(q.tm.tiles), dim3(512), LDS, stream, GTAV_HEAD_VALUES(q), q);
    GTAV_CHECK_HIP(hipGetLastError());
    return 0;
}

bool gemm_qkvs_attn_ok(int M, int D, int S) {
    static const int max_blocks = GTAV_ENV_INT("GTAV_QKVS_MAX_BLOCKS", 65535);
    return S == 144 && D % 64 == 0 && M > 0 && M % S == 0 && (long long)(M / S) * (D / 64) <= max_blocks;
}
int launch_gemm_qkvs_attn(const GemmParams& p_in, hipStream_t stream) {
    GemmParams q = p_in;
    GTAV_REQUIRE(gemm_qkvs_attn_ok(q.M, q.D, q.S), "gemm/qkvs_attn: unsupported geometry M=%d D=%d S=%d", q.M, q.D, q.S);
    GTAV_REQUIRE(q.N == 3 * q.D && q.K % TK == 0 && q.out && q.rope_cs && !q.rope_cs_q && !q.bias, "gemm/qkvs_attn: missing buffers (or a bias / a separate q table)");
    GTAV_REQUIRE(((uintptr_t)q.X & 15) == 0 && ((uintptr_t)q.W & 15) == 0, "gemm: operands must be 16-byte aligned");
    constexpr int NS = 3, LDS = NS * 44 * 1024;
    if (int rc_ = lds_opt_in<gemm_qkvs_attn_kernel<NS>>(LDS)) return rc_;
    lab_fields(q, 3 | 32 | 64);
    q.splitk = 1;
// ... 79 lines not shown
    const bool fold_c = epi_is_fold_consumer(epi_x), fold_p = epi_x == EPI_RESID_FOLD;
    if (fold_c || fold_p) {
        GTAV_REQUIRE(p.f_P > 0 && p.f_P % 16 == 0 && p.M % p.f_P == 0, "gemm/fold: %d tokens per frame must be a multiple of 16 and divide M=%d", p.f_P, p.M);
        if (fold_c) {
            GTAV_REQUIRE(p.f_stats && p.f_c1 && p.f_c2 && p.f_ldc >= p.N && p.f_nslot == p.K / 64 && p.f_nslot % 4 == 0,
                         "gemm/fold: consumer needs the row statistics (K/64 = %d slots, a multiple of 4) and the c1 / c2 tables", p.K / 64);
            GTAV_REQUIRE(!p.bias, "gemm/fold: the bias of a fold consumer lives in its c2 table");
            if (epi == EPI_QKV) GTAV_REQUIRE(p.qkv_mode == QKV_TEMPORAL || p.S % 16 == 0, "gemm/fold: spatial QKV needs S %% 16 == 0");
        } else {
            GTAV_REQUIRE(p.gate && p.f_scale && p.f_stats_out && p.f_a && p.N % 64 == 0 && p.ldo >= p.N,
                         "gemm/fold: producer needs gate, next scale, statistics and operand buffers, N %% 64 == 0");
        }
    }
    GTAV_REQUIRE(prefetch_desc_ok(p.pf), "gemm: bad prefetch descriptor (row tiles %d, K tiles %d, K slices %d)", p.pf.rt, p.pf.nkt, p.pf.splitk);
    GTAV_REQUIRE(p.K > 0 && p.K % TK == 0, "gemm: K=%d must be a positive multiple of %d", p.K, TK);
    GTAV_REQUIRE(p.M > 0 && p.N > 0 && p.N % 4 == 0, "gemm: bad M=%d N=%d", p.M, p.N);
    GTAV_REQUIRE(((uintptr_t)p.X & 15) == 0 && ((uintptr_t)p.W & 15) == 0, "gemm: operands must be 16-byte aligned");
    if (epi == EPI_QKV) {
        GTAV_REQUIRE(p.N == 3 * p.D && p.D % 128 == 0, "gemm/qkv: N=%d must equal 3*D, D=%d %% 128 == 0", p.N, p.D);
        GTAV_REQUIRE(p.S > 0 && p.q && p.k && p.rope_cs, "gemm/qkv: missing buffers");
        if (p.qkv_mode == QKV_SPATIAL) {
            GTAV_REQUIRE(p.S % 4 == 0 && p.M % p.S == 0 && p.v, "gemm/qkv spatial: S=%d must divide M=%d, S %% 4 == 0", p.S, p.M);
        } else {
            GTAV_REQUIRE(p.Tq > 0 && p.M % (p.S * p.Tq) == 0 && p.t0 + p.Tq <= p.Tmax, "gemm/qkv temporal: bad frame geometry");
        }
    } else {
        GTAV_REQUIRE(p.out && p.ldo >= p.N && p.ldo % 4 == 0, "gemm: bad output ldo=%d", p.ldo);
        if (epi == EPI_RESID && p.gate) GTAV_REQUIRE(p.rows_per_gate > 0, "gemm/resid: rows_per_gate");
        if (epi == EPI_GELU_TANH || epi == EPI_GELU_ERF || epi == EPI_F16_TILED) GTAV_REQUIRE(p.ldo % 64 == 0, "gemm/gelu: tile-major output needs ldo %% 64 == 0");
        if (fold_p) GTAV_REQUIRE(p.splitk <= 1, "gemm/fold: the producer epilogue needs the complete sum (no split-K)");
        if (epi == EPI_PARTIAL) GTAV_REQUIRE(p.splitk >= 1 && (p.K / TK) % p.splitk == 0, "gemm/partial: splitk=%d must divide K/64=%d", p.splitk, p.K / TK);
    }
    GemmPlan plan;
    if (int rc_ = gemm_plan(GemmProblem{p.M, p.N, p.K, epi_x, p.qkv_mode, p.S, p.splitk, p.gate ? p.rows_per_gate : 0}, &plan)) return rc_;
    if (fold_c || fold_p) {
        const int span = gemm_shape(plan.shape)->span();
        GTAV_REQUIRE(p.f_P >= span, "gemm/fold: frames of %d tokens are shorter than the token span (%d) of a wave of block shape %d", p.f_P, span, plan.shape);
    }
    const int dbg = gemm_debug();
    p.tm.gn = plan.gn;
    lab_fields(p, 3 | 16 | 32 | 2048 | 8192 | 16384 | 0x1F0000);
    p.out_sc1 = (dbg & 8) ? 0 : 1;
    if (dbg & 0x800000) p.pf.next = nullptr;
    switch (epi_x) {
#ifdef GTAV_EXPERIMENTS
        case EPI_RESID_FOLD: return launch_epi<EPI_RESID_FOLD>(p, plan, stream);
        case EPI_QKV_FOLD: return launch_epi<EPI_QKV_FOLD>(p, plan, stream);
        case EPI_GELU_TANH_FOLD: return launch_epi<EPI_GELU_TANH_FOLD>(p, plan, stream);
        case EPI_F32_FOLD: return launch_epi<EPI_F32_FOLD>(p, plan, stream);
#else
        case EPI_RESID_FOLD: case EPI_QKV_FOLD: case EPI_GELU_TANH_FOLD: case EPI_F32_FOLD:
            GTAV_REQUIRE(false, "gemm: the LayerNorm-fold epilogues exist only in the experiments build (csrc/build.sh exp)");
#endif
        case EPI_F32: return launch_epi<EPI_F32>(p, plan, stream);
        case EPI_F16: return launch_epi<EPI_F16>(p, plan, stream);
        case EPI_GELU_TANH: return launch_epi<EPI_GELU_TANH>(p, plan, stream);
        case EPI_GELU_ERF: return launch_epi<EPI_GELU_ERF>(p, plan, stream);
        case EPI_RESID: return launch_epi<EPI_RESID>(p, plan, stream);
        case EPI_QKV: return launch_epi<EPI_QKV>(p, plan, stream);
        case EPI_PARTIAL: return launch_epi<EPI_PARTIAL>(p, plan, stream);
        case EPI_F16_TILED: return launch_epi<EPI_F16_TILED>(p, plan, stream);
        default: GTAV_REQUIRE(false, "gemm: unknown epilogue %d", epi_x);
    }
    return 0;
}

}
```

ai-generated-gtav_amd/csrc/gemm_plan.h:

```cpp
#pragma once

namespace gtav_shared {

constexpr int GEMM_TK = 64;

enum GemmFamily : int {
    GF_K128,
    GF_G,
    GF_T256,
    GF_L,
    GF_LP,
    GF_LW,
    GF_LAB,
};

struct GemmShape {
    int id, family;
    int ns;
    int fi, fj, wn, wm, nl;
    bool product;
    constexpr int tokens() const { return 16 * fj * wm; }
    constexpr int features() const { return 16 * fi * wn; }
    constexpr int threads() const { return 64 * (wn * wm + nl); }
    constexpr int span() const { return 16 * fj; }
// ... 18 lines not shown
    {22, GF_LW,     4, 2, 3, 4, 2, 4, false},
    {23, GF_L,      4, 4, 3, 2, 2, 4, false},
    {24, GF_L,      4, 2, 1, 2, 3, 2, true},
    {25, GF_L,      5, 2, 3, 4, 2, 4, false},
    {26, GF_L,      4, 2, 2, 2, 3, 2, true},
    {27, GF_L,      8, 2, 1, 2, 3, 2, false},
    {28, GF_L,      8, 2, 1, 2, 3, 4, false},
    {29, GF_L,      4, 2, 3, 4, 3, 4, true},
    {30, GF_LP,     4, 4, 3, 2, 4, 4, false},
    {31, GF_LP,     3, 4, 3, 2, 4, 4, true},
    {32, GF_LP,     3, 4, 4, 4, 2, 4, false},
    {33, GF_LP,     3, 4, 4, 2, 4, 4, false},
    {40, GF_LAB,    2, 8, 4, 2, 4, 0, false},
    {41, GF_LAB,    2, 6, 4, 2, 4, 0, false},
    {42, GF_LAB,    2, 4, 4, 4, 4, 0, false},
};

constexpr const GemmShape* gemm_shape(int id) {
    for (const GemmShape& s : GEMM_SHAPES)
        if (s.id == id) return &s;
    return nullptr;
}
inline int gemm_tiles(int shape, int M, int N) {
    const GemmShape& s = *gemm_shape(shape);
    return ((M + s.tokens() - 1) / s.tokens()) * ((N + s.features() - 1) / s.features());
}

struct GemmProblem { int M, N, K, epi, qkv_mode, S, splitk, rows_per_gate; };
struct GemmPlan { int shape, ns, splitk, gn, tile_tokens, tile_features, blocks, threads; };

constexpr bool GEMM_LAB_BUILD = GTAV_LAB_BUILD;

int gemm_plan(const GemmProblem& g, GemmPlan* plan, bool lab = GEMM_LAB_BUILD);
int gemm_choose_gn(int M, int N, int K, int tmb, int tnb, int splitk, bool lab = GEMM_LAB_BUILD);
bool gemm_pp_ok(int M, int N, int K, int epi, bool lab = GEMM_LAB_BUILD);
bool gemm_resid_inplace_ok(int M, int N, int K, int rows_per_gate, bool lab = GEMM_LAB_BUILD);
int gemm_choose_splitk(int M, int N, int K, bool lab = GEMM_LAB_BUILD);

void gemm_set_stages(int ns);
void gemm_set_wm(int wm);
bool gemm_forced_wfill();
int gemm_debug(bool lab = GEMM_LAB_BUILD);
void gemm_set_debug(int bits);

}
```

ai-generated-gtav_amd/csrc/gemm_plan.hip:

```cpp
#include "gemm.h"

#include <cstdlib>

namespace gtav_shared {
using namespace gtav;

static thread_local int t_force_stages = 0, t_force_shape = 0, t_force_wfill = 0;
static thread_local int t_env_shape = GTAV_ENV_INT("GTAV_GEMM_SHAPE", 0);
void gemm_set_stages(int ns) { t_force_stages = ns; }
void gemm_set_wm(int wm) { t_force_shape = wm & 0xFF; t_force_wfill = wm >> 8 & 1; t_env_shape = 0; }
bool gemm_forced_wfill() { return t_force_wfill != 0; }
static int forced_shape(bool lab) { return t_force_shape ? t_force_shape : lab ? t_env_shape : 0; }

struct LabKnobs {
    int debug = 0;
    int lp = 1;
    int resid_inplace = 1;
    int splitk_old = 0;
    int l_for_8 = 1;
    int gn = 0;
    int pp = 0;
};
static const LabKnobs g_lab_off = {};
#ifdef GTAV_EXPERIMENTS
// ... 105 lines not shown
        else if (t13 > 256 && t13 <= 512 && !fold_p) wm = 13, narrow_pick = true;
        else if (fold_p && t12 > 128) wm = 12, narrow_pick = true;
    }
    if (splitk == 1 && ((epi_x == EPI_PARTIAL && lp_takes(M, N, K, lab)) || (epi_x == EPI_RESID && gemm_resid_inplace_ok(M, N, K, g.rows_per_gate, lab)))) wm = 31, narrow_pick = true;
    if (wm == 31 && epi_x == EPI_RESID && N % 256 == 0 && N <= 1024 && K >= 1024) {
        const int t256 = tiles(7), rounds = cdiv(t256, 256);
        if (rounds >= 2 && t256 * 10 >= rounds * 256 * 9) wm = 7;
    }
    wm = lab_shape_for_fc1(k, wm, epi_x, M, N);
    if (splitk == 1 && gemm_pp_ok(M, N, K, epi, lab) && !(spatial_qkv && g.S % 8 != 0)) wm = 16;
    if (splitk == 1 && epi != EPI_QKV && !foldish && !narrow_pick && N % 256 == 0 && N <= 1024 && K >= 1024) {
        const int t256 = tiles(7), rounds = cdiv(t256, 256);
        if (t256 * 10 >= rounds * 256 * 7) wm = 7;
    }
    return wm;
}

int gemm_plan(const GemmProblem& g, GemmPlan* plan, bool lab) {
    const int splitk = g.epi == EPI_PARTIAL ? g.splitk : 1;
    GTAV_REQUIRE(g.M > 0 && g.N > 0 && g.K > 0 && splitk >= 1, "gemm: bad M=%d N=%d K=%d splitk=%d", g.M, g.N, g.K, splitk);
    const int forced = forced_shape(lab);
    const int wm = forced ? forced : heuristic_shape(g, splitk, lab);
    const GemmShape* s = gemm_shape(wm);
    GTAV_REQUIRE(s, "gemm: unknown block shape %d", wm);
    GTAV_REQUIRE(s->product || (lab && GEMM_LAB_BUILD), "gemm: block shape %d exists only in the experiments build (csrc/build.sh exp)", wm);
    GTAV_REQUIRE(!(wm == 8 && epi_base(g.epi) == EPI_QKV && g.qkv_mode == QKV_SPATIAL), "gemm: 96-feature tiles straddle the K / V boundary (spatial QKV)");
    int gn = gemm_choose_gn(g.M, g.N, g.K, s->tokens(), s->features(), splitk, lab);
    if (s->family == GF_T256 && !knobs(lab).gn && splitk == 1 && g.N <= 1024 && (size_t)g.M >= 8 * (size_t)g.N) gn = cdiv(g.N, s->features());
    const int ns = t_force_stages ? t_force_stages : ((wm == 12 || wm == 13) ? 2 : wm >= 8 ? 4 : wm == 3 ? 4 : 2);
    *plan = GemmPlan{wm, ns, splitk, gn, s->tokens(), s->features(), gemm_tiles(wm, g.M, g.N) * splitk, s->threads()};
    return 0;
}

}
```

ai-generated-gtav_amd/csrc/gemm_typed.inc:

```
struct GemmParams {
    const f16* X;
    int ldx;
    int wfill;
    const f16* W;
    int M, N, K;
    int debug;
    unsigned long long* stamps;
    int* err_flag;
    int out_sc1;
    int splitk;
    const float* bias;
    void* out2;
    void* out;
    int ldo;
    const float* gate;
    int gate_stride;
    const int* gate_rows;
    int rows_per_gate;
    int qkv_mode;
    f16* q;
    f16* k;
    f16* v;
    int D;
    int S;
    int Tq;
    int t0;
    int Tmax;
    const float* rope_cs;
    const float* rope_cs_q;
    struct TileMap { int tiles_m, tiles_n, gn, group, tiles; unsigned rcp_tiles, rcp_group, rcp_gn, rcp_gnlast; } tm;
    int f_P;
    const int* f_rows;
    const float* f_stats;
    int f_nslot;
    const float* f_c1;
    const float* f_c2;
    int f_ldc;
    float* f_stats_out;
    const float* f_scale;
    f16* f_a;
    PrefetchDesc pf;
    float* sk_ws;
    int* sk_flags;
    int sk_dp, sk_r;
};
static_assert(sizeof(GemmParams) == 352, "GemmParams: every build and both operand types must see the same struct");

struct GemmGroup { const f16* X; const f16* W; float* out; const float* bias; int N; int ldo; };
int launch_gemm_grouped(const GemmGroup* groups_dev, int n_groups, int max_N, int M, int K, hipStream_t stream);

constexpr int GEMM_DW_MAX_GROUPS = 4;
struct GemmDwGroup { const f16* X; const f16* W; float* out; int M; int N; int ldo; };
static_assert(sizeof(GemmDwGroup) == 40, "GemmDwGroup: every build and both operand types must see the same struct");
bool gemm_dw_grouped_ok(const GemmDwGroup* g, int n, int K);
int launch_gemm_dw_grouped(const GemmDwGroup* g, int n, int K, int* err_flag, hipStream_t stream, bool tn = false);

int launch_gemm(const GemmParams& p, int epi, hipStream_t stream);
bool gemm_qkvt_attn_ok(int M, int D, int S, int Tq, int t0);
int launch_gemm_qkvt_attn(const GemmParams& p, hipStream_t stream);
bool gemm_qkvs_attn_ok(int M, int D, int S);
int launch_gemm_qkvs_attn(const GemmParams& p, hipStream_t stream);
bool gemm_tn_ok(int M, int N, int K);
bool gemm_tn_pays(int M, int N, int K);
int launch_gemm_tn(const GemmParams& p, hipStream_t stream);
```

ai-generated-gtav_amd/csrc/ops.h:

```cpp
#pragma once
#include "common.h"
#include "gemm.h"

namespace gtav {

#include "ops_typed.inc"

int launch_skinny_f32(const float* X, int ldx, const float* W, const float* bias, float* Y, int ldy, int M, int N,
                      int K, int act_silu, hipStream_t stream);
int skinny_init();

struct StepParams {
    int first;
    int cur;
    int t_ctx;
    int t_cur;
    int is_final;
    float alpha_t, alpha_next;
    int cond_step;
};
int launch_step_setup(StepParams* dst, const StepParams& v, int* frame_idx, int* mod_rows, int* last_rows, int* changed, int B, int Tq, int T, int F,
                      int use_cur, hipStream_t stream);
int launch_gather_rows(const float* table, const int* rows, const int* changed, float* cur, int slots, int W, const float* table2, float* cur2, int W2,
                       hipStream_t stream);
int launch_cond_inputs_frame(int rows, int B, int T, int F, int start, int cur, int t_ctx, const int* t_steps, const float* sincos,
                             float* E, const float* actions, int A, float* HC, int ldhc, int D, int Apad, int* err_flag,
                             hipStream_t stream);

int launch_unpatchify(const float* y, int ldy, float* img, int NB, int C, int H, int W, int p, int order, float a,
                      float b, hipStream_t stream);

int launch_copy_f32_strided(const float* src, int lds, int R, int C, float* dst, int ldd, hipStream_t stream);
int launch_copy_rows_f32(const float* src, size_t src_stride, float* dst, size_t dst_stride, int rows, size_t n, hipStream_t stream);
int launch_clamp_cols(float* buf, int M, int ld, int c0, int c1, float lo, float hi, hipStream_t stream);
int launch_frames_to_u8(const float* img, uint8_t* out, int N, int H, int W, hipStream_t stream);
int launch_moments_to_latents(const float* mom, float* lat, int N, int hw, int latent, int mom_ch, float scale, hipStream_t stream);
int launch_latents_to_tokens(const float* lat, float* z, int N, int hw, int latent, hipStream_t stream);
int launch_resize_aa(const void* src, int src_is_u8_strip, float* dst, int n, int H, int W, int OH, int OW, hipStream_t stream);
int launch_copy_f32(const float* src, int lds, int R, int C, float* dst, int ldd, int c0, hipStream_t stream);
int launch_fill_f32(float* dst, size_t n, float v, hipStream_t stream);
int launch_rope_interleave(const float* cos_t, const float* sin_t, float* cs, int npos, hipStream_t stream);
int launch_add_f32(const float* a, const float* b, float* out, size_t n, hipStream_t stream);
int launch_calib_spin(unsigned long long ticks, unsigned long long* dev_ticks, hipStream_t stream);
int launch_axpy_f32(float* y, const float* x, float alpha, size_t n, hipStream_t stream);

int launch_cond_inputs(const int64_t* t64, int rows, int Tq, const StepParams* sp, int use_cur, const float* sincos ,
                       float* E, const float* actions, int64_t act_outer, int64_t act_inner, int A, float* HC, int ldhc,
                       int D, int Apad, int* err_flag, hipStream_t stream);

int launch_ddim_update(const float* x, size_t x_stride, const float* v, size_t v_stride, float* out, size_t out_stride,
                       int B, int n, const float* alpha_t, const float* alpha_next, int is_final, hipStream_t stream);
int launch_ddim_update_step(float* x, size_t frames_per_sample, const float* v, size_t v_stride, int B, int n,
                            const StepParams* sp, hipStream_t stream);

int launch_add_noise(const float* x, const float* noise, const float* alpha , float* out, int rows, int n,
                     float clamp_abs, hipStream_t stream);
int launch_vtarget(const float* x, const float* noise, const float* alpha , float* vt, int rows, int n,
                   float clamp_abs, hipStream_t stream);
int launch_mse(const float* a, size_t a_stride, const float* b, size_t b_stride, int rows, int n, float* out_scalar,
               hipStream_t stream);

struct RngDraw {
    uint64_t seed;
// ... 40 lines not shown
```

ai-generated-gtav_amd/csrc/ops_bf16.h:

```cpp
#pragma once
#include "ops.h"

namespace gtav_bf16 {
typedef __bf16 f16;
using gtav_shared::PrefetchDesc;
#include "gemm_typed.inc"
#include "ops_typed.inc"
}

namespace gtav {

#define GTAV_OPERAND_OPS(F)                                 \
    F(gemm, launch_gemm)                                    \
    F(ln_modulate, launch_ln_modulate)                      \
    F(ln_affine, launch_ln_affine)                          \
    F(patchify, launch_patchify)                            \
    F(convert_pad, launch_convert_pad_f16)                  \
    F(unpad, launch_unpad_f16_to_f32)                       \
    F(attn_spatial, launch_attn_spatial)                    \
    F(attn_temporal, launch_attn_temporal)                  \
                     \
    F(gemm_tn, launch_gemm_tn)                              \
    F(gemm_dw_grouped, launch_gemm_dw_grouped)              \
    F(transpose_tiled, launch_transpose_tiled_f16)          \
    F(convert_T, launch_convert_T_f16)                      \
    F(gelu_tiled, launch_gelu_tiled)                        \
    F(gelu_bwd_tiled, launch_gelu_bwd_tiled)                \
    F(gelu_bwd_tiled_colsum, launch_gelu_bwd_tiled_colsum)  \
    F(gate_bwd, launch_gate_bwd)                            \
    F(frame_reduce_gate, launch_frame_reduce_gate)          \
    F(gate_bwd_fused, launch_gate_bwd_fused)                \
    F(colsum_tiled, launch_colsum_tiled_f16)                \
    F(to_tiled, launch_to_tiled_f16)                        \
    F(mse_bwd_patch, launch_mse_bwd_patch)                  \
    F(attn_spatial_bwd, launch_attn_spatial_bwd)            \
    F(attn_temporal_bwd, launch_attn_temporal_bwd)          \
    F(adamw_multi, launch_adamw_multi)                      \
    F(branch_rows, launch_branch_rows)

struct OperandOps {
#define GTAV_OPS_FIELD(field, launcher) decltype(&launcher) field;
    GTAV_OPERAND_OPS(GTAV_OPS_FIELD)
#undef GTAV_OPS_FIELD
    bool bf16;
};
const OperandOps& operand_ops(bool bf16);

// ... 2 lines not shown
```

ai-generated-gtav_amd/csrc/ops_typed.inc:

```

int launch_ctab_inputs(const float* mod, int MODW, int R, int Rp, int D, const int* col, const int* is_scale, int n_groups, f16* sx, size_t group_stride,
                       hipStream_t stream);

struct LnPending {
    const float* parts;
    int nsplit;
    size_t slab_stride;
    int ld;
    const float* bias;
    const float* gate;
    int gate_stride;
    const int* gate_rows;
    int rows_per_gate;
    int flags;
    int* err_flag;
    float* x_out;
    f16* y_save;
    int tperm_T, tperm_P;
    float* k_save;
    const float* k_load;
};
static_assert(sizeof(LnPending) == 120, "LnPending: every build and both operand types must see the same struct");

int launch_ln_modulate(float* x, int ldx, f16* out, int ldo, int M, int D, const float* shift, const float* scale,
                       int mod_stride, const int* rows, int rows_per_mod, const LnPending* pend, int* err_flag, hipStream_t stream);
int launch_ln_affine(float* x, int ldx, f16* out, int ldo, int M, int D, const float* gamma, const float* beta,
                     const LnPending* pend, int* err_flag, hipStream_t stream);
int launch_branch_rows(const float* parts, int nsplit, size_t slab_stride, int ld, const float* bias, f16* y, int M, int N, int* err_flag, hipStream_t stream);

int launch_patchify(const float* img, const int* frame_index, int NB, int C, int H, int W, int p, f16* out, int ldo,
                    float a, float b, int* err_flag, hipStream_t stream);

int launch_convert_pad_f16(const float* src, int lds, int R, int C, f16* dst, int Rp, int Cp, float scale, int tiled,
                           hipStream_t stream, int* err_flag = nullptr);
int launch_unpad_f16_to_f32(const f16* src, int lds, int R, int C, float* dst, int tiled, hipStream_t stream);
int launch_qkv_head_major(const f16* src, f16* dst, int D, hipStream_t stream, int mode = 0);

int launch_transpose_tiled_f16(const f16* src, int R, int C, f16* dst, hipStream_t stream);
int launch_convert_T_f16(const float* src, int lds, int R, int C, f16* dst, hipStream_t stream);
int launch_gelu_tiled(const f16* u, f16* h, size_t n, hipStream_t stream);
int launch_gelu_bwd_tiled(const f16* dh, const f16* u, f16* du, size_t n, int* err_flag, hipStream_t stream);
int launch_gelu_bwd_tiled_colsum(const f16* dh, const f16* u, f16* du, int M, int N, float* db, float* ws, int* err_flag, hipStream_t stream);
int launch_gate_bwd(const float* dres, const float* gate, int mod_stride, int rows_per_mod, int M, int D, f16* dy_tiled, int* err_flag, hipStream_t stream);
int launch_frame_reduce_gate(const float* dres, const f16* y, int frames, int P, int D, float* dgate, int mod_stride, hipStream_t stream);
int launch_gate_bwd_fused(const float* dres, const f16* y, const float* gate, int mod_stride, int frames, int P, int D, f16* dy_tiled, float* dgate, float* db,
                          float* ws, int* err_flag, hipStream_t stream);
int launch_colsum_tiled_f16(const f16* dy, int M, int N, float* db, float* ws, hipStream_t stream);
int launch_to_tiled_f16(const float* a, int M, int D, f16* out, int* err_flag, hipStream_t stream);
int launch_mse_bwd_patch(const float* vpred, const float* vtarget, int B, int T, int C, int H, int W, int p, float scale, f16* dfo, int ldf, int* err_flag,
                         hipStream_t stream);
int launch_attn_spatial_bwd(const f16* Q, const f16* K, const f16* Vt, const f16* dO, int NB, int heads, int S, int D, const float* rope_cs, f16* dqkv,
                            int* err_flag, hipStream_t stream);
int launch_attn_temporal_bwd(const f16* q, const f16* kv, const f16* dO, int B, int P, int D, int T, int Tmax, const float* rope_cs, f16* dqkv, int* err_flag,
                             hipStream_t stream);
struct AdamParam {
    float* p; int ldp, R, C;
    const float* g; float *m, *v;
    f16* w16; int Cp16;
// ... 12 lines not shown
```

ai-generated-gtav_amd/lib.py:

```python
from __future__ import annotations

import ctypes as C
import os
import subprocess

_HERE = os.path.dirname(os.path.abspath(__file__))
LIB_PATH = os.path.join(_HERE, "libgtav_amd.so")
HEADER_PATH = os.path.join(os.path.dirname(_HERE), "include", "gtav_amd.h")


class GtavError(RuntimeError):
    pass


class GtavRangeSwitch(GtavError):

    def __init__(self, msg, groups=()):
        super().__init__(msg)
        self.groups = list(groups)


def build(force: bool = False) -> str:
    src_dir = os.path.join(_HERE, "csrc")
    srcs = [os.path.join(src_dir, f) for f in os.listdir(src_dir)] + [HEADER_PATH]
# ... 35 lines not shown
    "gtav_dit_operand_groups": [_p, C.POINTER(C.c_int32)],
    "gtav_dit_set_operand_dtype": [_p, _i, _i],
    "gtav_dit_get_operand_dtype": [_p, _i, C.POINTER(C.c_int32)],
    "gtav_dit_autorange": [_p, C.POINTER(C.c_int32), _p],
    "gtav_dit_train_param_count": [_p, C.POINTER(C.c_int64)],
    "gtav_dit_train_allow_window": [_p, _i],
    "gtav_dit_train_set_recompute": [_p, _i],
    "gtav_dit_train_saved_bytes": [_p, C.POINTER(C.c_int64)],
    "gtav_dit_train_allow_mixed": [_p, _i],
    "gtav_dit_train_set_group_dtype": [_p, _i, _i, _p],
    "gtav_dit_train_range_words": [_p, C.POINTER(C.c_int32), _p],
    "gtav_dit_train_autorange": [_p, C.POINTER(C.c_int32), C.POINTER(C.c_int32), _p],
    "gtav_dit_train_enable": [_p, _p, _l],
    "gtav_dit_train_enable_typed": [_p, _p, _l, _i],
    "gtav_dit_set_loss_scale": [_p, _f],
    "gtav_dit_set_grad_divisor": [_p, _f],
    "gtav_dit_zero_grad": [_p, _p],
    "gtav_dit_train_forward": [_p, _p, _p, _p, _p, _i, _i, _p],
    "gtav_dit_train_backward": [_p, _p, _p, _p],
    "gtav_dit_train_backward_phases": [_p, _p, _p, _i, _i, _p],
    "gtav_dit_train_param_range": [_p, C.c_char_p, C.POINTER(C.c_int64), C.POINTER(C.c_int64)],
    "gtav_dit_get_grad": [_p, C.c_char_p, _p, _l, _p],
    "gtav_dit_train_get_residual": [_p, _i, _p, _l, _p],
    "gtav_dit_adamw_step": [_p, _f, _f, _f, _f, _f, _f, _p],
    "gtav_dit_train_stats": [_p, C.POINTER(C.c_float), _p],
    "gtav_dit_get_opt_state": [_p, C.c_char_p, _p, _p, _l, _p],
    "gtav_dit_set_opt_state": [_p, C.c_char_p, _p, _p, _l, _p],
    "gtav_dit_get_opt_step": [_p, C.POINTER(C.c_int64), C.POINTER(C.c_int64), _p],
    "gtav_dit_set_opt_step": [_p, _l, _l, _p],
    "gtav_dit_set_graph": [_p, _i],
    "gtav_dit_set_fused_temporal": [_p, _i],
    "gtav_dit_set_fused_spatial": [_p, _i],
    "gtav_dit_fused_launches": [_p, _i, _i, _i],
    "gtav_dit_set_weight_prefetch": [_p, _i],
    "gtav_dit_set_weight_fill_policy": [_p, _i],
    "gtav_dit_profile": [_p, _i],
    "gtav_dit_profile_read": [_p, C.POINTER(C.c_double), C.POINTER(C.c_int64)],
    "gtav_timer_calibrate": [_i, _i, C.POINTER(C.c_double), C.POINTER(C.c_double), _p],
    "gtav_comm_unique_id": [_p],
    "gtav_comm_init": [C.POINTER(_p), _i, _i, _p],
    "gtav_comm_allreduce_f32": [_p, _p, _l, _i, _p],
    "gtav_comm_allgather": [_p, _p, _p, _l, _p],
    "gtav_comm_destroy": [_p],
    "gtav_vae_create": [C.POINTER(VaeConfig), C.POINTER(_p)],
    "gtav_vae_destroy": [_p],
    "gtav_vae_set_weight": [_p, C.c_char_p, _p, _l, _p],
    "gtav_vae_finalize": [_p, _p],
    "gtav_vae_get_weight": [_p, C.c_char_p, _p, _l, _p],
    "gtav_vae_encode": [_p, _p, _f, _f, _p, _i, _p],
    "gtav_vae_decode": [_p, _p, _f, _p, _f, _f, _i, _p],
    "gtav_vae_check": [_p, _p],
    "gtav_vae_set_operand_dtype": [_p, _i],
    "gtav_vae_get_operand_dtype": [_p, C.POINTER(C.c_int32)],
    "gtav_vae_profile": [_p, _i],
    "gtav_vae_profile_read": [_p, C.POINTER(C.c_double), C.POINTER(C.c_int64)],
    "gtav_clamp_frames": [_p, _i, _i, _i, _i, _f, _f, _p],
    "gtav_ddim_update": [_p, _p, _p, _i, _i, _p, _p, _i, _p],
    "gtav_add_noise": [_p, _p, _p, _p, _i, _i, _f, _p],
    "gtav_vtarget": [_p, _p, _p, _p, _i, _i, _f, _p],
    "gtav_rng_normal": [_p, _l, _i, _i, _u64, _u32, _u32, _u32, _u32, _f, _p],
    "gtav_noise_window_rng": [_p, _p, _p, _p, _i, _i, _i, _u64, _u32, _u32, _f, _p],
    "gtav_vae_posterior_sample": [_p, _p, _i, _i, _i, _u64, _u32, _u32, _u32, _u32, _p],
    "gtav_op_rng_bits": [_p, _i, _i, _u64, _u32, _u32, _u32, _u32, _p],
    "gtav_mse": [_p, _l, _p, _l, _i, _i, _p, _p],
    "gtav_axpy_f32": [_p, _p, _f, _l, _p],
    "gtav_frames_to_u8": [_p, _p, _i, _i, _i, _p],
    "gtav_moments_to_latents": [_p, _p, _i, _i, _i, _i, _f, _p],
    "gtav_latents_to_tokens": [_p, _p, _i, _i, _i, _p],
    "gtav_strip_to_frames": [_p, _i, _i, _i, _p, _i, _i, _p],
    "gtav_resize_frames": [_p, _p, _i, _i, _i, _i, _i, _p],
    "gtav_op_gemm_f16": [_p, _i, _p, _p, _p, _i, _i, _i, _i, _i, _p, _i, _i, _p],
    "gtav_op_gemm_qkv": [_p, _i, _p, _p, _i, _i, _i, _p, _p, _p, _i, _i, _i, _i, _p, _p],
    "gtav_op_rope_interleave": [_p, _p, _p, _i, _p],
    "gtav_op_skinny_f32": [_p, _i, _p, _p, _p, _i, _i, _i, _i, _i, _p],
    "gtav_op_ln_modulate": [_p, _p, _i, _i, _p, _p, _i, _i, _p],
    "gtav_op_ln_affine": [_p, _p, _i, _i, _p, _p, _p],
    "gtav_op_attn_spatial": [_p, _p, _p, _p, _i, _i, _i, _p],
    "gtav_op_attn_temporal": [_p, _p, _p, _i, _i, _i, _i, _i, _i, _p],
    "gtav_op_attn_temporal_bf16": [_p, _p, _p, _i, _i, _i, _i, _i, _i, _p],
    "gtav_op_qkv_head_major": [_p, _p, _i, _p],
    "gtav_op_gemm_tn": [_p, _p, _i, _i, _i, _p, _i, _p],
    "gtav_op_gemm_dw_grouped": [_i, _p, _p, _p, _p, _p, _p, _i, _p],
    "gtav_op_attn_spatial_bwd": [_p, _p, _p, _p, _i, _i, _i, _p, _p, _p],
    "gtav_op_attn_spatial_bwd_bf16": [_p, _p, _p, _p, _i, _i, _i, _p, _p, _p],
    "gtav_op_attn_temporal_bwd": [_p, _p, _p, _i, _i, _i, _i, _i, _p, _p, _p],
    "gtav_op_attn_temporal_bwd_bf16": [_p, _p, _p, _i, _i, _i, _i, _i, _p, _p, _p],
    "gtav_op_gemm_qkvt_attn": [_p, _p, _i, _i, _i, _i, _i, _i, _p, _p, _p, _p],
    "gtav_op_qkv_head_major_spatial": [_p, _p, _i, _p],
    "gtav_op_gemm_qkvs_attn": [_p, _p, _i, _i, _i, _p, _p, _p],
    "gtav_op_convert_f16": [_p, _i, _i, _i, _p, _i, _i, _i, _p],
    "gtav_op_gemm_splitk_ln": [_p, _i, _p, _p, _i, _i, _i, _i, _p, _p, _p, _i, _i, _p, _p, _p, _i, _p],
    "gtav_op_gemm_choose_splitk": [_i, _i, _i],
    "gtav_op_gemm_plan": [_i, _i, _i, _i, _i, _i, _i, _i, _p],
    "gtav_op_gemm_resid_inplace": [_i, _i, _i],
    "gtav_op_gemm_set_stages": [_i],
    "gtav_op_gemm_set_wm": [_i],
    "gtav_op_set_operand_dtype": [_i],
    "gtav_op_attn_spatial_prescaled": [_p, _p, _p, _p, _i, _i, _i, _p],
    "gtav_op_train_ln_mod_bwd": [_i, _p, _p, _p, _i, _i, _i, _i, _p, _i, _p, _p, _p, _l, _p],
    "gtav_op_train_gate_bwd": [_i, _p, _p, _p, _i, _i, _i, _i, _p, _p, _p, _p, _l, _p, _p],
    "gtav_op_train_gelu_bwd": [_i, _p, _p, _p, _i, _i, _p, _p, _l, _p, _p],
    "gtav_op_train_colsum_tiled": [_p, _i, _i, _p, _p, _l, _p],
    "gtav_op_train_colsum_f32": [_p, _i, _i, _i, _p, _p, _l, _p],
    "gtav_op_train_colsum_reduce_multi": [C.POINTER(_p), C.POINTER(_p), C.POINTER(_i), C.POINTER(_i), _i, _p],
    "gtav_op_train_mse_bwd_patch": [_p, _p, _i, _i, _i, _i, _i, _i, _f, _p, _i, _p, _p],
    "gtav_op_train_to_tiled": [_p, _i, _i, _p, _p, _p],
    "gtav_op_train_transpose_tiled": [_p, _i, _i, _p, _p],
    "gtav_op_train_convert_t": [_p, _i, _i, _i, _p, _p],
    "gtav_op_train_silu": [_p, _i, _p, _i, _i, _i, _p],
    "gtav_op_train_silu_bwd": [_p, _i, _p, _i, _p, _i, _i, _i, _p],
    "gtav_op_train_gemm_tn_f32": [_p, _i, _p, _i, _i, _i, _i, _p, _i, _p],
    "gtav_op_train_gemm_nn_f32": [_p, _i, _p, _i, _i, _i, _i, _p, _i, _p],
    "gtav_op_train_ada_bwd_dx": [_p, _i, _p, _i, _i, _p, _p, _l, _p],
    "gtav_op_ln_pending": [_i, _p, _i, _p, _i, _i, _p, _p, _i, _p, _i, _p, _i, _l, _i, _p, _p, _i, _p, _i, _p, _p, _i, _i, _p, _p, _p, _p],
    "gtav_op_branch_rows": [_p, _i, _l, _i, _p, _p, _i, _i, _p, _p],
}
_RESTYPES = {"gtav_last_error": C.c_char_p, "gtav_dit_destroy": None, "gtav_vae_destroy": None, "gtav_op_gemm_set_stages": None,
             "gtav_op_gemm_set_wm": None, "gtav_op_set_operand_dtype": None}

_lib = None


def load() -> C.CDLL:
    global _lib
    if _lib is not None:
        return _lib
# ... 61 lines not shown
```

ai-generated-gtav_amd/model/dit.py:

```python
from __future__ import annotations

import ctypes as C
import math
from collections import OrderedDict
from typing import Dict, Iterator, Optional

import torch

from .. import lib as _lib
from .. import weights as _w


def _rope_tables_axial(freqs: torch.Tensor, gh: int, gw: int):
    def ang(n):
        a = torch.linspace(-1, 1, steps=n)[:, None] * freqs[None, :]
        return a.repeat_interleave(2, dim=-1)
    ah, aw = ang(gh), ang(gw)
    a = torch.cat([ah[:, None, :].expand(gh, gw, -1), aw[None, :, :].expand(gh, gw, -1)], dim=-1).reshape(gh * gw, -1)
    cos, sin = torch.ones(gh * gw, 64), torch.zeros(gh * gw, 64)
    cos[:, : a.shape[1]] = a.cos()
    sin[:, : a.shape[1]] = a.sin()
    return cos.contiguous(), sin.contiguous()


# ... 208 lines not shown
                v = torch.randn(shp) * 0.02
            self._sd[k] = v
        self._dirty = True

    def _ensure(self, B: int, T: int, cond_rows: int = 0):
        if T > MAX_FRAMES:
            raise ValueError(f"a window of {T} frames: the temporal attention serves at most {MAX_FRAMES} (max_frames <= {MAX_FRAMES})")
        if self._trainable and self._train_max_frames is not None and T > self._train_max_frames:
            raise ValueError(f"a window of {T} frames on a trainable DiT constructed with train_max_frames={self._train_max_frames}: the handle's saved "
                             f"activations are sized for at most {self._train_max_frames} frames (train_max_frames <= {MAX_FRAMES})")
        if self._trainable and self._train_max_frames is None and T > TRAIN_MAX_FRAMES:
            raise ValueError(f"a window of {T} frames on a trainable DiT: the training step (backward temporal attention, adaLN-gradient reduction) is "
                             f"implemented for at most {TRAIN_MAX_FRAMES} frames; windows up to {MAX_FRAMES} need trainable=False")
        grow = (cond_rows > max(self._capacity_rows, self._capacity_b * self._capacity_t)) or T > self._capacity_t or B > self._capacity_b
        if grow and self._handle and self._trainable and self._grads is not None:
            raise RuntimeError(f"a trainable DiT cannot grow its workspace after training was enabled (batch {B} > {self._capacity_b}, window {T} > "
                               f"{self._capacity_t} or {cond_rows} conditioning rows > {max(self._capacity_rows, self._capacity_b * self._capacity_t)}): "
                               "size it with max_batch / max_frames / reserve() before the first step")
        if grow:
            self._capacity_rows = max(self._capacity_rows, cond_rows)
            self._capacity_t = max(self._capacity_t, T)
            self._capacity_b = max(self._capacity_b, B)
            self._free()
        if not self._handle:
            L = _lib.load()
            cfg = _lib.DitConfig(max_frames=self._capacity_t, max_batch=self._capacity_b,
                                 max_cond_rows=max(self._capacity_b * self._capacity_t, self._capacity_rows), **self._cfg_kwargs)
            with torch.cuda.device(self.device):
                _lib.check(L.gtav_dit_create(C.byref(cfg), C.byref(self._handle)))
                if getattr(self, "_fused_temporal", False):
                    _lib.check(L.gtav_dit_set_fused_temporal(self._handle, 1))
                if getattr(self, "_fused_spatial", None) is not None:
                    _lib.check(L.gtav_dit_set_fused_spatial(self._handle, int(self._fused_spatial)))
                if getattr(self, "_fold", None) is not None:
                    _lib.check(L.gtav_dit_set_fold(self._handle, *self._fold))
                if getattr(self, "_weight_prefetch", None) is not None:
                    _lib.check(L.gtav_dit_set_weight_prefetch(self._handle, int(self._weight_prefetch)))
                if getattr(self, "_weight_fill_policy", None) is not None:
                    _lib.check(L.gtav_dit_set_weight_fill_policy(self._handle, int(self._weight_fill_policy)))
                if not self._train_mixed:
                    for g in sorted(self._bf16_groups):
                        _lib.check(L.gtav_dit_set_operand_dtype(self._handle, g, 1))
                if self._trainable:
                    n = C.c_int64(0)
                    _lib.check(L.gtav_dit_train_param_count(self._handle, C.byref(n)))
                    self._grads = torch.zeros(n.value, device=self.device, dtype=torch.float32)
                    if self._train_max_frames is not None:
                        _lib.check(L.gtav_dit_train_allow_window(self._handle, self._train_max_frames))
                    if self._train_recompute:
                        _lib.check(L.gtav_dit_train_set_recompute(self._handle, 1))
                    if self._train_mixed:
                        _lib.check(L.gtav_dit_train_allow_mixed(self._handle, 1))
                    if self._train_bf16:
                        _lib.check(L.gtav_dit_train_enable_typed(self._handle, self._grads.data_ptr(), n.value, 1))
                    else:
                        _lib.check(L.gtav_dit_train_enable(self._handle, self._grads.data_ptr(), n.value))
                    if self._train_mixed:
                        start = set(range(self.n_operand_groups)) if self._train_bf16 else set()
                        for g in sorted(self._bf16_groups ^ start):
                            _lib.check(L.gtav_dit_train_set_group_dtype(self._handle, g, 1 if g in self._bf16_groups else 0, _lib.current_stream()))
                    _lib.check(L.gtav_dit_set_loss_scale(self._handle, self._loss_scale))
                    if self.grad_divisor != 1.0:
                        _lib.check(L.gtav_dit_set_grad_divisor(self._handle, self.grad_divisor))
            self._dirty = True
        if self._dirty:
            gh, gw = self.input_h // self.patch_size, self.input_w // self.patch_size
# ... 257 lines not shown
        B, F = x.shape[:2]
        if cond_step < 0:
            self._ensure(B, cur - start + 1)
        with torch.cuda.device(self.device):
            _lib.check(_lib.load().gtav_dit_denoise_step(
                self._handle, x.data_ptr(), B, F, start, cur, int(t_ctx), int(t_cur), int(t_next), int(bool(is_final)),
                _lib.ptr(actions), 1 if cached else 0, int(cond_step), _lib.ptr(v_out), _lib.current_stream()))

    PROFILE_CLASSES = ("ln_modulate", "gemm_qkv", "attn_spatial", "attn_temporal", "gemm_out", "gemm_fc1", "gemm_fc2", "other",
                       "empty_event_pair")

    def profile(self, enable: bool):
        _lib.check(_lib.load().gtav_dit_profile(self._handle, int(bool(enable))))

    def profile_read(self):
        ms = (C.c_double * 9)()
        n = (C.c_int64 * 9)()
        _lib.check(_lib.load().gtav_dit_profile_read(self._handle, ms, n))
        return {k: (ms[i], n[i]) for i, k in enumerate(self.PROFILE_CLASSES)}

    def set_graph(self, enable: bool):
        _lib.check(_lib.load().gtav_dit_set_graph(self._handle, int(bool(enable))))

    def set_fused_temporal(self, enable: bool):
        self._fused_temporal = bool(enable)
        if self._handle:
            _lib.check(_lib.load().gtav_dit_set_fused_temporal(self._handle, int(self._fused_temporal)))

    def set_fused_spatial(self, enable: bool):
        self._fused_spatial = bool(enable)
        if self._handle:
            _lib.check(_lib.load().gtav_dit_set_fused_spatial(self._handle, int(self._fused_spatial)))

    def fused_launches(self, B: int, T: int, t0: int = 0) -> int:
        self._ensure(B, T)
        return int(_lib.load().gtav_dit_fused_launches(self._handle, int(B), int(T), int(t0)))

    def set_weight_prefetch(self, mode):
        mode = int(mode)
        if mode not in (0, 1) and (mode >> 16) != 1:
            raise ValueError(f"set_weight_prefetch: mode {mode:#x} is neither 0, 1 nor a per-class word (gtav_amd.generate.prefetch_mode)")
        self._weight_prefetch = mode
        if self._handle:
            _lib.check(_lib.load().gtav_dit_set_weight_prefetch(self._handle, mode))

    def set_weight_fill_policy(self, mode: int):
        mode = int(mode)
        if mode & ~0x1111:
            raise ValueError(f"set_weight_fill_policy: mode {mode:#x} is not a per-class word of nibbles 0 / 1 (gtav_amd.generate.fill_policy_mode)")
        self._weight_fill_policy = mode
        if self._handle:
            _lib.check(_lib.load().gtav_dit_set_weight_fill_policy(self._handle, mode))

    def set_fold(self, mode: int, min_tokens_a: int = -1, min_tokens_b: int = -1):
        if not getattr(_lib.load(), "_gtav_experiments", False):
            raise _lib.GtavError("set_fold: the LayerNorm fold exists only in the experiments build (gtav_amd.lib.load_experiments())")
        self._fold = (int(mode), int(min_tokens_a), int(min_tokens_b))
        if self._handle:
            _lib.check(_lib.load().gtav_dit_set_fold(self._handle, *self._fold))

    def set_operand_dtype(self, dtype, groups=None):
        if dtype not in (torch.float16, torch.bfloat16):
            raise ValueError(f"set_operand_dtype: {dtype} (torch.float16 or torch.bfloat16)")
        if self._train_bf16 and dtype == torch.float16:
            raise _lib.GtavError("set_operand_dtype: a bf16-trainable DiT (train_dtype=torch.bfloat16) keeps bf16 operands in every layer group")
        if self._trainable and not self._train_bf16 and dtype == torch.bfloat16:
# ... 49 lines not shown
```

include/gtav_amd.h:

```cpp
#ifndef GTAV_AMD_H
#define GTAV_AMD_H

#include <stdint.h>

#ifdef __cplusplus
extern "C" {
#endif

const char* gtav_last_error(void);
int gtav_abi_version(void);

typedef struct gtav_dit_config {
    int32_t input_h, input_w, patch_size, in_channels, hidden_size, depth, num_heads;
    float mlp_ratio;
    int32_t external_cond_dim, max_frames;
    int32_t max_batch;
    int32_t max_cond_rows;
} gtav_dit_config;

typedef struct gtav_dit gtav_dit;

int gtav_dit_create(const gtav_dit_config* cfg, gtav_dit** out);
void gtav_dit_destroy(gtav_dit* h);
int gtav_dit_set_weight(gtav_dit* h, const char* name, const float* src_dev, int64_t numel, void* stream);
int gtav_dit_finalize(gtav_dit* h, void* stream);
int gtav_dit_get_weight(gtav_dit* h, const char* name, float* dst_dev, int64_t numel, void* stream);

int gtav_dit_forward(gtav_dit* h, const float* x_dev, const int64_t* t_dev, const float* actions_dev, float* out_dev,
                     int32_t B, int32_t T, void* stream);

int gtav_dit_set_schedule(gtav_dit* h, const float* alphas_cumprod_host, int32_t n);

int gtav_dit_denoise_step(gtav_dit* h, float* x_dev, int32_t B, int32_t F, int32_t start, int32_t cur, int32_t t_ctx,
                          int32_t t_cur, int32_t t_next, int32_t is_final, const float* actions_dev, int32_t mode,
                          int32_t cond_step, float* v_out_dev, void* stream);
int gtav_dit_prepare_frame(gtav_dit* h, int32_t B, int32_t F, int32_t start, int32_t cur, int32_t t_ctx,
                           const int32_t* t_steps_host, int32_t n_steps, const float* actions_dev, void* stream);

int gtav_dit_set_graph(gtav_dit* h, int32_t enable);

int gtav_dit_set_fused_temporal(gtav_dit* h, int32_t enable);

int gtav_dit_set_fused_spatial(gtav_dit* h, int32_t enable);
int gtav_dit_fused_launches(gtav_dit* h, int32_t B, int32_t T, int32_t t0);

int gtav_dit_set_weight_prefetch(gtav_dit* h, int32_t mode);

int gtav_dit_set_weight_fill_policy(gtav_dit* h, int32_t mode);

#define GTAV_PROFILE_CLASSES 9
int gtav_dit_profile(gtav_dit* h, int32_t enable);
int gtav_dit_profile_read(gtav_dit* h, double* ms_by_class, int64_t* launches_by_class);

int gtav_timer_calibrate(int32_t spin_us, int32_t reps, double* event_us_mean, double* device_us_mean, void* stream);

int gtav_dit_train_allow_window(gtav_dit* h, int32_t max_frames);
int gtav_dit_train_set_recompute(gtav_dit* h, int32_t enable);
int gtav_dit_train_allow_mixed(gtav_dit* h, int32_t enable);
int gtav_dit_train_set_group_dtype(gtav_dit* h, int32_t group, int32_t dtype, void* stream);
int gtav_dit_train_range_words(gtav_dit* h, int32_t* words_host, void* stream);
int gtav_dit_train_autorange(gtav_dit* h, const int32_t* merged_words_host, int32_t* n_switched, void* stream);
int gtav_dit_train_saved_bytes(gtav_dit* h, int64_t* bytes);
int gtav_dit_train_param_count(gtav_dit* h, int64_t* numel);
int gtav_dit_train_enable(gtav_dit* h, float* grad_arena_dev, int64_t grad_arena_numel);
int gtav_dit_train_enable_typed(gtav_dit* h, float* grad_arena_dev, int64_t grad_arena_numel, int32_t dtype);
int gtav_dit_set_loss_scale(gtav_dit* h, float scale);
int gtav_dit_set_grad_divisor(gtav_dit* h, float divisor);
int gtav_dit_zero_grad(gtav_dit* h, void* stream);
int gtav_dit_train_forward(gtav_dit* h, const float* x_dev, const int64_t* t_dev, const float* actions_dev, float* out_dev,
                           int32_t B, int32_t T, void* stream);
int gtav_dit_train_backward(gtav_dit* h, const float* v_pred_dev, const float* v_target_dev, void* stream);
int gtav_dit_train_get_residual(gtav_dit* h, int32_t k, float* dst_dev, int64_t numel, void* stream);
int gtav_dit_train_backward_phases(gtav_dit* h, const float* v_pred_dev, const float* v_target_dev, int32_t phase_begin, int32_t phase_end,
                                   void* stream);
int gtav_dit_train_param_range(gtav_dit* h, const char* prefix, int64_t* offset, int64_t* count);
int gtav_dit_get_grad(gtav_dit* h, const char* name, float* dst_dev, int64_t numel, void* stream);
// ... 77 lines not shown
                       int32_t ldy, int32_t M, int32_t N, int32_t K, int32_t act_silu, void* stream);
int gtav_op_ln_modulate(const float* x_dev, void* out_f16_dev, int32_t M, int32_t D, const float* shift_dev,
                        const float* scale_dev, int32_t mod_stride, int32_t rows_per_mod, void* stream);
int gtav_op_ln_affine(const float* x_dev, void* out_f16_dev, int32_t M, int32_t D, const float* gamma_dev,
                      const float* beta_dev, void* stream);
int gtav_op_attn_spatial(const void* q_dev, const void* k_dev, const void* vt_dev, void* o_dev, int32_t NB,
                         int32_t heads, int32_t S, void* stream);
int gtav_op_attn_temporal(const void* q_dev, const void* kv_dev, void* o_dev, int32_t B, int32_t P, int32_t D,
                          int32_t Tq, int32_t t0, int32_t Tmax, void* stream);
int gtav_op_attn_temporal_bf16(const void* q_dev, const void* kv_dev, void* o_dev, int32_t B, int32_t P, int32_t D,
                               int32_t Tq, int32_t t0, int32_t Tmax, void* stream);
int gtav_op_qkv_head_major(const void* w_f16_dev, void* w_hm_f16_dev, int32_t D, void* stream);
int gtav_op_gemm_qkvt_attn(const void* x_tperm_f16_dev, const void* w_hm_f16_dev, int32_t M, int32_t D, int32_t P, int32_t Tq,
                           int32_t t0, int32_t Tmax, const float* rope_cs_dev, void* kv_dev, void* o_dev, void* stream);
int gtav_op_qkv_head_major_spatial(const void* w_f16_dev, void* w_hm_f16_dev, int32_t D, void* stream);
int gtav_op_gemm_qkvs_attn(const void* x_f16_dev, const void* w_hm_f16_dev, int32_t M, int32_t D, int32_t P, const float* rope_cs_dev, void* o_dev,
                           void* stream);
int gtav_op_attn_spatial_bwd(const void* q_dev, const void* k_dev, const void* vt_dev, const void* d_o_dev, int32_t NB, int32_t heads,
                             int32_t S, const float* rope_cs_dev, void* dqkv_dev, void* stream);
int gtav_op_attn_spatial_bwd_bf16(const void* q_dev, const void* k_dev, const void* vt_dev, const void* d_o_dev, int32_t NB, int32_t heads,
                                  int32_t S, const float* rope_cs_dev, void* dqkv_dev, void* stream);
int gtav_op_attn_temporal_bwd(const void* q_dev, const void* kv_dev, const void* d_o_dev, int32_t B, int32_t P, int32_t D, int32_t T, int32_t Tmax,
                              const float* rope_cs_dev, void* dqkv_dev, void* stream);
int gtav_op_attn_temporal_bwd_bf16(const void* q_dev, const void* kv_dev, const void* d_o_dev, int32_t B, int32_t P, int32_t D, int32_t T, int32_t Tmax,
                                   const float* rope_cs_dev, void* dqkv_dev, void* stream);
int gtav_op_gemm_tn(const void* x_f16_dev, const void* w_f16_dev, int32_t M, int32_t N, int32_t K, float* out_dev, int32_t ldo, void* stream);
int gtav_op_gemm_dw_grouped(int32_t n, const void* const* x_f16_dev, const void* const* w_f16_dev, float* const* out_dev, const int32_t* M,
                            const int32_t* N, const int32_t* ldo, int32_t K, void* stream);
int gtav_op_gemm_splitk_ln(const void* x_f16_dev, int32_t ldx, const void* w_f16_dev, const float* bias_dev, int32_t M,
                           int32_t N, int32_t K, int32_t splitk, float* parts_dev, float* resid_dev, const float* gate_dev,
                           int32_t gate_stride, int32_t rows_per_gate, void* out_f16_dev, const float* shift_dev,
                           const float* scale_dev, int32_t mod_stride, void* stream);
int gtav_op_gemm_choose_splitk(int32_t M, int32_t N, int32_t K);
int gtav_op_gemm_plan(int32_t M, int32_t N, int32_t K, int32_t epilogue, int32_t qkv_mode, int32_t S, int32_t splitk, int32_t rows_per_gate, int32_t* plan8);
int gtav_op_gemm_resid_inplace(int32_t M, int32_t N, int32_t K);
int gtav_op_convert_f16(const float* src_dev, int32_t lds, int32_t R, int32_t C, void* dst_f16_dev, int32_t Rp,
                        int32_t Cp, int32_t tiled, void* stream);

typedef struct gtav_comm gtav_comm;
int gtav_comm_unique_id(void* id128_host);
int gtav_comm_init(gtav_comm** out, int32_t nranks, int32_t rank, const void* id128_host);
int gtav_comm_allreduce_f32(gtav_comm* c, float* buf_dev, int64_t count, int32_t average, void* stream);
int gtav_comm_allgather(gtav_comm* c, const void* send_dev, void* recv_dev, int64_t bytes_per_rank, void* stream);
int gtav_comm_destroy(gtav_comm* c);

#ifdef __cplusplus
}
#endif
#endif
```

Before: 5.545.

## Compute only last-frame rows in final DiT block MLP and output head

When the forward pass runs over all frames but only the last frame's velocity is consumed (mode 0), the last block's FC1/FC2 GEMMs, the LayerNorms after them, the final projection and the unpatchify now process only the rows of the last frame in each batch item. It does this through a RowWindow row remap. The intent is to skip MLP and head work on rows whose outputs are never read. It adds windowed GEMM and LN paths and a debug option that fills dead rows with NaN. The path is disabled when fold or in-place residual epilogues apply.

Result: slower. 5.407 (-2.5%).

```diff
diff --git a/ai-generated-gtav_amd/csrc/api.hip b/ai-generated-gtav_amd/csrc/api.hip
--- a/ai-generated-gtav_amd/csrc/api.hip
+++ b/ai-generated-gtav_amd/csrc/api.hip
@@ -316,6 +316,27 @@
     if (mode == 0) return op_ops().ln_modulate(x, ldx, (f16*)out, D, M, D, p0, p1, mod_stride, rows, rows_per_mod, &pd, err, (hipStream_t)stream);
     return op_ops().ln_affine(x, ldx, (f16*)out, D, M, D, p0, p1, &pd, err, (hipStream_t)stream);
 }
+int gtav_op_gemm_live_rows(const void* x, const void* w, const float* bias, void* out, int32_t ldo, int32_t N, int32_t K, int32_t epilogue, int32_t splitk,
+                           int32_t first, int32_t seg_rows, int32_t seg_stride, int32_t segs, int32_t total_rows, void* stream) {
+    GemmParams g = gemm_params((const f16*)x, K, (const f16*)w, segs * seg_rows, N, K);
+    g.bias = bias; g.out = out; g.ldo = ldo; g.splitk = splitk;
+    g.win = row_window(first, seg_rows, seg_stride, segs, total_rows);
+    return op_ops().gemm(g, epilogue, (hipStream_t)stream);
+}
+int gtav_op_ln_live_rows(float* x, void* out, int32_t D, const float* shift, const float* scale, int32_t mod_stride, int32_t rows_per_mod, const float* parts,
+                         int32_t nsplit, int64_t slab_stride, const float* bias, const float* gate, int32_t gate_stride, int32_t rows_per_gate, int32_t first,
+                         int32_t seg_rows, int32_t seg_stride, int32_t segs, int32_t total_rows, int32_t* err, void* stream) {
+    LnPending pd;
+    memset(&pd, 0, sizeof(pd));
+    pd.parts = parts; pd.nsplit = nsplit; pd.slab_stride = (size_t)slab_stride; pd.ld = D; pd.bias = bias; pd.gate = gate; pd.gate_stride = gate_stride;
+    pd.rows_per_gate = rows_per_gate;
+    const RowWindow win = row_window(first, seg_rows, seg_stride, segs, total_rows);
+    return op_ops().ln_modulate_rows(x, D, (f16*)out, D, segs * seg_rows, D, shift, scale, mod_stride, nullptr, rows_per_mod, &pd, &win, err, (hipStream_t)stream);
+}
+int gtav_op_gemm_plan_live_rows(int32_t M, int32_t N, int32_t K, int32_t epilogue, int32_t splitk, int32_t* plan8) {
+    GTAV_REQUIRE(plan8, "op_gemm_plan_live_rows: null argument");
+    return gtav_shared::gemm_plan_live_rows(gtav_shared::GemmProblem{M, N, K, epilogue, 0, 0, splitk, 0}, (gtav_shared::GemmPlan*)plan8);
+}
 int gtav_op_branch_rows(const float* parts, int32_t nsplit, int64_t slab_stride, int32_t ld, const float* bias, void* y, int32_t M, int32_t N, int32_t* err,
                         void* stream) {
     return op_ops().branch_rows(parts, nsplit, (size_t)slab_stride, ld, bias, (f16*)y, M, N, err, (hipStream_t)stream);
diff --git a/ai-generated-gtav_amd/csrc/api_dit.hip b/ai-generated-gtav_amd/csrc/api_dit.hip
--- a/ai-generated-gtav_amd/csrc/api_dit.hip
+++ b/ai-generated-gtav_amd/csrc/api_dit.hip
@@ -148,17 +148,29 @@
     return gemm_pp_ok(M, h->D, K, EPI_RESID) || (gemm_choose_splitk(M, h->D, K) == 1 && M >= h->resid_inplace_min_m) || gemm_resid_inplace_ok(M, h->D, K, h->P);
 }
 
+static bool dit_live_rows(const gtav_dit* h, int B, int Tq, bool fold_a, bool fold_b) {
+    const int M = B * Tq * h->P;
+    return h->live_rows && Tq > 1 && !fold_a && !fold_b && h->P % 8 == 0 && B * h->P < 65536 && !dit_resid_inplace(h, M, h->D) && !dit_resid_inplace(h, M, h->Hm_pad);
+}
+
+static int dit_poison_dead_rows(gtav_dit* h, const RowWindow& win, hipStream_t s) {
+    RET_IF(launch_poison_dead_rows(h->resid, 4, 0, h->D, win, s));
+    RET_IF(launch_poison_dead_rows(h->xn, 2, 1, h->D, win, s));
+    return launch_poison_dead_rows(h->hbuf, 2, 1, h->Hm_pad, win, s);
+}
+
 static int dit_forward_core(gtav_dit* h, const float* x_src, const int* frame_index, int B, int Tq, int t0,
-                            const float* mod, const int* mod_rows, const float* ctab, float* v_out, hipStream_t s) {
+                            const float* mod, const int* mod_rows, const float* ctab, float* v_out, hipStream_t s, bool last_frame_only = false) {
     const int D = h->D, P = h->P, NB = B * Tq, M = NB * P;
     GTAV_REQUIRE(M <= h->Mmax, "forward: %d tokens exceed workspace (%d)", M, h->Mmax);
     bool fold_a, fold_b;
     fold_policy(h, M, fold_a, fold_b);
+    const bool live = last_frame_only && dit_live_rows(h, B, Tq, fold_a, fold_b);
     const DitPrefetch pf(h, M, Tq, t0);
     DeferredResid rd{h->parts, h->parts_rows * (size_t)D, h->resid, M, D, &h->prof, s};
     auto gate = [&](const float* g) { return ResidGate{g, h->MODW, mod_rows, P}; };
     auto ln = [&](const OperandOps& o, const float* shift, const float* scale, int* ef) -> int {
-        PROF(h, PC_LN, s, o.ln_modulate(h->resid, D, h->xn, D, M, D, shift, scale, h->MODW, mod_rows, P, rd.take(), ef, s));
+        PROF(h, PC_LN, s, o.ln_modulate_rows(h->resid, D, h->xn, D, rd.rows(), D, shift, scale, h->MODW, mod_rows, P, rd.take(), rd.window(), ef, s));
         return 0;
     };
     const int g_embed = 2 * h->L, g_final = 2 * h->L + 1;
@@ -193,7 +205,15 @@
             else PROF(h, PC_ATTN_T, s, ops.attn_temporal(h->qt, h->kvcache[l], h->ao, B, P, D, Tq, t0, h->maxT, s));
         }
         folded_in = false;
-        GemmParams fc1 = gemm_params(h->xn, D, w.w_fc1, M, h->Hm, D);
+        if (live && hb == 2 * h->L - 1) {
+            rd.win = row_window((Tq - 1) * P, P, Tq * P, B, M);
+#ifdef GTAV_EXPERIMENTS
+            static const int poison = GTAV_ENV_INT("GTAV_POISON_DEAD_ROWS", 1);
+            if (poison) RET_IF(dit_poison_dead_rows(h, rd.win, s));
+#endif
+        }
+        GemmParams fc1 = gemm_params(h->xn, D, w.w_fc1, rd.rows(), h->Hm, D);
+        fc1.win = rd.win;
         fc1.bias = w.b_fc1; fc1.out = h->hbuf; fc1.ldo = h->Hm_pad; fc1.err_flag = ef; fc1.pf = pf.after(hb, 2); fc1.wfill = pf.fill(1);
         if (fold_a) {
             RET_IF(fold_producer(h, PC_OUT, h->ao, w.w_out, M, D, w.b_out, gate(mb + 2 * D), mb + 4 * D, s));
@@ -214,11 +234,12 @@
     }
     const float* mf = mod + (size_t)h->L * 12 * D;
     if (!folded_in) RET_IF(ln(h->ops(g_final), mf, mf + D, h->err_of(g_final)));
-    GemmParams fin = gemm_params(h->xn, D, h->w_final, M, h->Nfin, D);
-    fin.bias = h->b_final; fin.out = h->fo; fin.ldo = h->Nfin;
+    GemmParams fin = gemm_params(h->xn, D, h->w_final, rd.rows(), h->Nfin, D);
+    fin.bias = h->b_final; fin.out = h->fo; fin.ldo = h->Nfin; fin.win = rd.win;
     if (folded_in) fold_consumer(h, fin, 4 * h->L, h->Nfin, mod_rows, ctab);
     PROF(h, PC_OTHER, s, h->ops(g_final).gemm(fin, folded_in ? EPI_F32_FOLD : EPI_F32, s));
-    PROF(h, PC_OTHER, s, launch_unpatchify(h->fo, h->Nfin, v_out, NB, h->C, h->H, h->W, h->p, 0, 1.f, 0.f, s));
+    if (rd.win.segs) PROF(h, PC_OTHER, s, launch_unpatchify_frames(h->fo, h->Nfin, v_out, B, Tq - 1, Tq, h->C, h->H, h->W, h->p, 0, 1.f, 0.f, s));
+    else PROF(h, PC_OTHER, s, launch_unpatchify(h->fo, h->Nfin, v_out, NB, h->C, h->H, h->W, h->p, 0, 1.f, 0.f, s));
     return h->prof.collect(s);
 }
 
@@ -428,7 +449,7 @@
     const size_t fsz = (size_t)h->C * h->H * h->W;
     const int Tq = mode == 1 ? 1 : T, t0 = mode == 1 ? T - 1 : 0;
     if (!prepared) RET_IF(dit_cond(h, nullptr, B * Tq, Tq, h->step_dev, mode == 1, actions, (int64_t)F * h->A, h->A, s));
-    RET_IF(dit_forward_core(h, x, h->frame_idx, B, Tq, t0, prepared ? h->mod_cur : h->mod, nullptr, prepared ? h->fold.ctab_cur : h->fold.ctab, h->vout, s));
+    RET_IF(dit_forward_core(h, x, h->frame_idx, B, Tq, t0, prepared ? h->mod_cur : h->mod, nullptr, prepared ? h->fold.ctab_cur : h->fold.ctab, h->vout, s, mode == 0));
     const float* vlast = h->vout + (size_t)(Tq - 1) * fsz;
     RET_IF(launch_ddim_update_step(x, F, vlast, (size_t)Tq * fsz, B, (int)fsz, h->step_dev, s));
     if (v_out) RET_IF(launch_copy_rows_f32(vlast, (size_t)Tq * fsz, v_out, fsz, B, fsz, s));
@@ -565,6 +586,23 @@
     return 0;
 }
 
+int gtav_dit_set_live_rows(gtav_dit* h, int32_t enable) {
+    GTAV_REQUIRE(h && (enable == 0 || enable == 1), "dit_set_live_rows: 0 or 1");
+    if (h->live_rows != (enable != 0)) h->drop_graphs();
+    h->live_rows = enable != 0;
+    return 0;
+}
+
+int gtav_dit_poison_dead_rows(gtav_dit* h, int32_t B, int32_t T, void* stream) {
+    GTAV_REQUIRE(h && B >= 1 && T >= 2 && B <= h->maxB && T <= h->maxT && h->P % 8 == 0, "dit_poison_dead_rows: B=%d T=%d", B, T);
+    const int M = B * T * h->P;
+    const RowWindow win = row_window((T - 1) * h->P, h->P, T * h->P, B, M);
+    RET_IF(dit_poison_dead_rows(h, win, (hipStream_t)stream));
+    for (size_t sl = 0; (sl + 1) * M <= h->parts_rows && sl < 8; ++sl)
+        RET_IF(launch_poison_dead_rows(h->parts + sl * (size_t)M * h->D, 4, 0, h->D, win, (hipStream_t)stream));
+    return 0;
+}
+
 #ifdef GTAV_EXPERIMENTS
 int gtav_dit_set_fold(gtav_dit* h, int32_t mode, int32_t min_tokens_a, int32_t min_tokens_b) {
     GTAV_REQUIRE(h && mode >= 0 && mode <= 2, "dit_set_fold: mode %d", mode);
diff --git a/ai-generated-gtav_amd/csrc/api_internal.h b/ai-generated-gtav_amd/csrc/api_internal.h
--- a/ai-generated-gtav_amd/csrc/api_internal.h
+++ b/ai-generated-gtav_amd/csrc/api_internal.h
@@ -258,10 +258,14 @@
     hipStream_t s;
     LnPending pend;
     bool pending = false;
+    RowWindow win = {};
+    int rows() const { return win.segs ? win.rows() : M; }
+    const RowWindow* window() const { return win.segs ? &win : nullptr; }
     int gemm(const OperandOps& ops, int cls, const f16* X, int ldx, const f16* W, int K, const float* bias, const ResidGate& gt, bool inplace,
              const PrefetchDesc& pf = kNoPrefetch, float* x_out = nullptr, f16* y_save = nullptr, int wfill = 0) {
-        GemmParams q = gemm_params(X, ldx, W, M, N, K);
-        q.out = parts; q.ldo = N; q.pf = pf; q.wfill = wfill;
+        GemmParams q = gemm_params(X, ldx, W, rows(), N, K);
+        q.out = parts; q.ldo = N; q.pf = pf; q.wfill = wfill; q.win = win;
+        GTAV_REQUIRE(!(inplace && win.segs), "deferred residual: the in-place epilogue takes no live-row window");
         if (inplace) {
             q.out = resid; q.bias = bias; q.gate = gt.gate; q.gate_stride = gt.stride; q.gate_rows = gt.rows; q.rows_per_gate = gt.rows_per_gate;
         } else {
@@ -348,6 +352,7 @@
     bool use_graph = true;
     bool fuse_tattn = false;
     bool fuse_sattn = false;
+    bool live_rows = true;
     bool w_prefetch = true;
     int w_prefetch_cls[4] = {1, 4, 4, 1};
     int w_fill_cls[4] = {0, 0, 0, 0};
diff --git a/ai-generated-gtav_amd/csrc/common.h b/ai-generated-gtav_amd/csrc/common.h
--- a/ai-generated-gtav_amd/csrc/common.h
+++ b/ai-generated-gtav_amd/csrc/common.h
@@ -106,9 +106,30 @@
     int rt, nkt, splitk;
     int kt_limit;
 };
+struct RowWindow {
+    int first, seg_rows, seg_stride, segs;
+    unsigned rcp_seg;
+    int total_rows;
+    __host__ __device__ __forceinline__ int row(int m) const {
+        const int s = (int)(((unsigned long long)(unsigned)m * rcp_seg) >> 32);
+        return first + s * seg_stride + (m - s * seg_rows);
+    }
+    __host__ __device__ __forceinline__ int rows() const { return segs * seg_rows; }
+};
+static inline RowWindow row_window(int first, int seg_rows, int seg_stride, int segs, int total_rows) {
+    return RowWindow{first, seg_rows, seg_stride, segs, seg_rows > 1 ? (unsigned)((0x100000000ull + (unsigned)seg_rows - 1) / (unsigned)seg_rows) : 0u, total_rows};
+}
+static inline bool row_window_ok(const RowWindow& w) {
+    return w.segs > 0 && w.seg_rows >= 8 && w.seg_rows % 8 == 0 && w.first >= 0 && w.first % 8 == 0 && w.seg_stride % 8 == 0 && w.seg_stride >= w.seg_rows &&
+           (long long)w.segs * w.seg_rows < 65536 && w.first + (long long)(w.segs - 1) * w.seg_stride + w.seg_rows <= w.total_rows &&
+           w.rcp_seg == (unsigned)((0x100000000ull + (unsigned)w.seg_rows - 1) / (unsigned)w.seg_rows);
+}
 }
 namespace gtav {
 using gtav_shared::PrefetchDesc;
+using gtav_shared::RowWindow;
+using gtav_shared::row_window;
+using gtav_shared::row_window_ok;
 __device__ __forceinline__ void l2_prefetch_slice(const PrefetchDesc& d, int xcd, int j, int nb, int t, int nt, unsigned& sink) {
     const int sk = d.splitk;
     int ks0, ksn, rt0, rtn;
diff --git a/ai-generated-gtav_amd/csrc/elementwise.hip b/ai-generated-gtav_amd/csrc/elementwise.hip
--- a/ai-generated-gtav_amd/csrc/elementwise.hip
+++ b/ai-generated-gtav_amd/csrc/elementwise.hip
@@ -71,15 +71,15 @@
 #else
 #define LN_DBG(pd, b) false
 #endif
-template <int MODE, bool PEND, int KS = 0>
+template <int MODE, bool PEND, int KS = 0, bool WIN = false>
 __global__ __launch_bounds__(512) void ln_row_block_kernel(float* __restrict__ x, int ldx, int D, const float* __restrict__ h_parts, size_t h_slab_stride, int h_ld,
                                                            int h_nsplit, int h_flags, int rows_per_mod, f16* __restrict__ out, int M,
                                                            const float* __restrict__ p0, const float* __restrict__ p1,
                                                            int mod_stride, const int* __restrict__ rows,
-                                                           LnPending pd) {
+                                                           LnPending pd, RowWindow win) {
     __shared__ float red[16];
     pd.parts = h_parts; pd.slab_stride = h_slab_stride; pd.ld = h_ld; pd.nsplit = h_nsplit; pd.flags = h_flags;
-    const int m = blockIdx.x;
+    const int m = WIN ? win.row((int)blockIdx.x) : (int)blockIdx.x;
     const int c = threadIdx.x * 4;
     const int nw = (blockDim.x + 63) >> 6, wid = threadIdx.x >> 6, lane = threadIdx.x & 63;
     float* xr = x + (size_t)m * ldx;
@@ -254,6 +254,32 @@
         const size_t m = ((size_t)nb * gh + yy / p) * gw + xx / p;
         const int f = order == 0 ? (ph * p + pw) * C + c : (c * p + ph) * p + pw;
         img[idx] = a * y[m * ldy + f] + b;
+    }
+}
+
+__global__ void unpatchify_frames_kernel(const float* __restrict__ y, int ldy, float* __restrict__ img, int n, int f0, int fstep, int C, int H, int W, int p,
+                                         int order, float a, float b) {
+    const int gh = H / p, gw = W / p;
+    const size_t fsz = (size_t)C * H * W, total = (size_t)n * fsz;
+    for (size_t idx = (size_t)blockIdx.x * blockDim.x + threadIdx.x; idx < total; idx += (size_t)gridDim.x * blockDim.x) {
+        const int xx = (int)(idx % W), yy = (int)((idx / W) % H), c = (int)((idx / ((size_t)W * H)) % C);
+        const int i = (int)(idx / fsz), nb = f0 + i * fstep;
+        const int ph = yy % p, pw = xx % p;
+        const size_t m = ((size_t)nb * gh + yy / p) * gw + xx / p;
+        const int f = order == 0 ? (ph * p + pw) * C + c : (c * p + ph) * p + pw;
+        img[(size_t)nb * fsz + (idx - (size_t)i * fsz)] = a * y[m * ldy + f] + b;
+    }
+}
+
+__global__ void poison_dead_rows_kernel(void* __restrict__ buf, int eb, int tiled, int ld, RowWindow win) {
+    const size_t total = (size_t)win.total_rows * ld;
+    for (size_t idx = (size_t)blockIdx.x * blockDim.x + threadIdx.x; idx < total; idx += (size_t)gridDim.x * blockDim.x) {
+        const int r = (int)(idx / ld), c = (int)(idx - (size_t)r * ld);
+        const int d = r - win.first;
+        const bool live = d >= 0 && d / win.seg_stride < win.segs && d % win.seg_stride < win.seg_rows;
+        if (live) continue;
+        if (eb == 4) ((unsigned*)buf)[idx] = 0x7FC00000u;
+        else ((unsigned short*)buf)[tiled ? tiled_off(r, c, ld) : idx] = (unsigned short)0x7FFF;
     }
 }
 
@@ -722,7 +748,7 @@
 
 #define LN_WAVE_ROW_(MODE, NV, P0, P1, STRIDE, ROWS, RPM) \
     GTAV_LAUNCH((ln_wave_row_kernel<MODE, NV>), dim3(cdiv(M, 4)), dim3(256), 0, stream, x, ldx, out, M, D, P0, P1, STRIDE, ROWS, RPM, pd_.flags, err_flag)
-#define LN_ROW_BLOCK_ARGS_(P0, P1, STRIDE, ROWS, RPM) x, ldx, D, pd_.parts, pd_.slab_stride, pd_.ld, pd_.nsplit, pd_.flags, RPM, out, M, P0, P1, STRIDE, ROWS, pd_
+#define LN_ROW_BLOCK_ARGS_(P0, P1, STRIDE, ROWS, RPM) x, ldx, D, pd_.parts, pd_.slab_stride, pd_.ld, pd_.nsplit, pd_.flags, RPM, out, M, P0, P1, STRIDE, ROWS, pd_, win_
 #define LN_DISPATCH(MODE, P0, P1, STRIDE, ROWS, RPM)                                                     \
     do {                                                                                                  \
         LnPending pd_;                                                                                    \
@@ -734,7 +760,13 @@
         const bool upd_ = pend && pend->parts;    \
         GTAV_REQUIRE(!pd_.k_save || (upd_ && !pd_.k_load), "ln: k_save needs a pending update and excludes k_load");                          \
         GTAV_REQUIRE(!pd_.k_load || !upd_, "ln: k_load excludes a pending update");                                                            \
-        if (pd_.k_save || pd_.k_load) {                  \
+        if (win_.segs) {  \
+            GTAV_REQUIRE(row_window_ok(win_) && M == win_.rows() && pd_.tperm_T == 0 && !pd_.k_save && !pd_.k_load && !pd_.x_out && !pd_.y_save, \
+                         "ln: bad live-row window (M=%d; no row permutation, kept shift or training outputs)", M);  \
+            const dim3 g_(M), b_(round_up(D / 4, 64));                                                    \
+            if (upd_) GTAV_LAUNCH((ln_row_block_kernel<MODE, true, 0, true>), g_, b_, 0, stream, LN_ROW_BLOCK_ARGS_(P0, P1, STRIDE, ROWS, RPM)); \
+            else GTAV_LAUNCH((ln_row_block_kernel<MODE, false, 0, true>), g_, b_, 0, stream, LN_ROW_BLOCK_ARGS_(P0, P1, STRIDE, ROWS, RPM));     \
+        } else if (pd_.k_save || pd_.k_load) {           \
             const dim3 g_(M), b_(round_up(D / 4, 64));                                                    \
             if (pd_.k_save) GTAV_LAUNCH((ln_row_block_kernel<MODE, true, 1>), g_, b_, 0, stream, LN_ROW_BLOCK_ARGS_(P0, P1, STRIDE, ROWS, RPM)); \
             else GTAV_LAUNCH((ln_row_block_kernel<MODE, false, 2>), g_, b_, 0, stream, LN_ROW_BLOCK_ARGS_(P0, P1, STRIDE, ROWS, RPM));      \
@@ -752,6 +784,11 @@
 
 int launch_ln_modulate(float* x, int ldx, f16* out, int ldo, int M, int D, const float* shift, const float* scale,
                        int mod_stride, const int* rows, int rows_per_mod, const LnPending* pend, int* err_flag, hipStream_t stream) {
+    return launch_ln_modulate_rows(x, ldx, out, ldo, M, D, shift, scale, mod_stride, rows, rows_per_mod, pend, nullptr, err_flag, stream);
+}
+int launch_ln_modulate_rows(float* x, int ldx, f16* out, int ldo, int M, int D, const float* shift, const float* scale,
+                            int mod_stride, const int* rows, int rows_per_mod, const LnPending* pend, const RowWindow* win, int* err_flag, hipStream_t stream) {
+    const RowWindow win_ = win ? *win : RowWindow{};
     GTAV_REQUIRE(D % 64 == 0 && D <= 2048 && rows_per_mod > 0 && ldo == D, "ln_modulate: D=%d must be %%64, <= 2048, ldo == D", D);
     GTAV_REQUIRE(!pend || !pend->parts || (pend->nsplit >= 1 && pend->nsplit <= 8 && pend->ld % 4 == 0 && (!pend->gate || pend->rows_per_gate > 0)),
                  "ln_modulate: bad pending update");
@@ -762,6 +799,7 @@
 
 int launch_ln_affine(float* x, int ldx, f16* out, int ldo, int M, int D, const float* gamma, const float* beta,
                      const LnPending* pend, int* err_flag, hipStream_t stream) {
+    const RowWindow win_ = {};
     GTAV_REQUIRE(D % 64 == 0 && D <= 2048 && ldo == D, "ln_affine: D=%d must be %%64, <= 2048, ldo == D", D);
     GTAV_REQUIRE(!pend || !pend->parts || (pend->nsplit >= 1 && pend->nsplit <= 8 && pend->ld % 4 == 0 && (!pend->gate || pend->rows_per_gate > 0)),
                  "ln_affine: bad pending update");
@@ -806,6 +844,21 @@
     return 0;
 }
 
+int launch_unpatchify_frames(const float* y, int ldy, float* img, int n, int f0, int fstep, int C, int H, int W, int p, int order, float a, float b,
+                             hipStream_t stream) {
+    GTAV_REQUIRE(H % p == 0 && W % p == 0 && ldy >= C * p * p && n > 0 && f0 >= 0 && fstep > 0, "unpatchify_frames: bad geometry");
+    hipLaunchKernelGGL(unpatchify_frames_kernel, dim3(grid_for((size_t)n * C * H * W)), dim3(256), 0, stream, y, ldy, img, n, f0, fstep, C, H, W, p, order, a, b);
+    GTAV_CHECK_HIP(hipGetLastError());
+    return 0;
+}
+
+int launch_poison_dead_rows(void* buf, int elem_bytes, int tiled, int ld, const RowWindow& win, hipStream_t stream) {
+    GTAV_REQUIRE(buf && (elem_bytes == 2 || (elem_bytes == 4 && !tiled)) && ld > 0 && (!tiled || ld % 64 == 0) && row_window_ok(win), "poison_dead_rows: bad arguments");
+    hipLaunchKernelGGL(poison_dead_rows_kernel, dim3(grid_for((size_t)win.total_rows * ld)), dim3(256), 0, stream, buf, elem_bytes, tiled, ld, win);
+    GTAV_CHECK_HIP(hipGetLastError());
+    return 0;
+}
+
 int launch_convert_pad_f16(const float* src, int lds, int R, int C, f16* dst, int Rp, int Cp, float scale, int tiled,
                            hipStream_t stream, int* err_flag) {
     GTAV_REQUIRE(Rp >= R && Cp >= C, "convert_pad: padded shape smaller than source");
diff --git a/ai-generated-gtav_amd/csrc/gemm.hip b/ai-generated-gtav_amd/csrc/gemm.hip
--- a/ai-generated-gtav_amd/csrc/gemm.hip
+++ b/ai-generated-gtav_amd/csrc/gemm.hip
@@ -848,7 +848,7 @@
     }
 }
 
-template <int EPIX, int FI, int FJ, int WM, int WN = 2, int WOFF = 0, bool PRE = false>
+template <int EPIX, int FI, int FJ, int WM, int WN = 2, int WOFF = 0, bool PRE = false, bool WIN = false>
 __device__ __forceinline__ void epilogue(const GemmParams& p, f32x4 (&acc)[FI][FJ], const f32x4 (&pbias)[FI], char* smem, int n0, int m0, int ks, bool tr,
                                          const f32x4 (&prope)[FI][FJ], FoldTok<FJ>& ft) {
     constexpr int EPI = epi_base(EPIX);
@@ -1000,9 +1000,13 @@
         auto copy_out = [&](void* out) {
             for (int q = wraw; q < CT * PR; q += (int)(blockDim.x >> 6)) {
                 const int cs = q / PR, pq = q - cs * PR;
-                const int gr = m0 + 8 * pq;
+                int gr = m0 + 8 * pq;
+                if constexpr (WIN) {
+                    if (gr >= p.M) continue;
+                    gr = p.win.row(gr);
+                }
                 const int rt = gr >> 7;
-                if (rt > last_rt || (n0 >> 6) + cs >= nkt_out) continue;
+                if ((!WIN && rt > last_rt) || (n0 >> 6) + cs >= nkt_out) continue;
                 const uint4 val = *(const uint4*)(smem + (cs * TM + 8 * pq) * 128 + lane * 16);
                 char* dst = (char*)out + ((size_t)rt * nkt_out + (n0 >> 6) + cs) * TILE_BYTES + ((gr & 127) >> 3) * 1024 + lane * 16;
                 if (p.out_sc1) store16q_sc1(dst, val);
@@ -1154,6 +1158,7 @@
         for (int j = 0; j < FJ; ++j) {
             const int m = m0 + 16 * FJ * wm + 16 * j + li;
             if (m >= p.M) continue;
+            const int mr = WIN ? p.win.row(m) : m;
             f32x4 v;
             if constexpr (FOLD) {
                 const float* cf = (const float*)ft.cb + fold_frame_of(ft, m0 + 16 * FJ * wm + 16 * j) * 2 * TNB + (n - n0);
@@ -1162,11 +1167,11 @@
                 v = acc[i][j] + bv;
             }
             if constexpr (EPI == EPI_PARTIAL) {
-                float* dst = (float*)p.out + ((size_t)ks * p.M + m) * p.ldo + n;
+                float* dst = (float*)p.out + ((size_t)ks * (WIN ? p.win.total_rows : p.M) + mr) * p.ldo + n;
                 if (p.out_sc1) store16_sc1(dst, v);
                 else *(f32x4*)dst = v;
             } else if constexpr (EPI == EPI_F32) {
-                *(f32x4*)((float*)p.out + (size_t)m * p.ldo + n) = v;
+                *(f32x4*)((float*)p.out + (size_t)mr * p.ldo + n) = v;
             } else if constexpr (EPI == EPI_F16) {
                 *(uint2*)((f16*)p.out + (size_t)m * p.ldo + n) = pack4(amax, v[0], v[1], v[2], v[3]);
             } else if constexpr (EPI == EPI_QKV) {
@@ -1604,7 +1609,7 @@
     epilogue<EPI_F32, FI, FJ, WM>(p, acc, pbias, smem, n0, m0, 0, false);
 }
 
-template <bool TR, int NS, int FI, int FJ, int WN, int WM, int NL, int TRI = FI, bool HALFSTEP = (FI * FJ >= 16), typename AfterPrologue>
+template <bool TR, int NS, int FI, int FJ, int WN, int WM, int NL, int TRI = FI, bool HALFSTEP = (FI * FJ >= 16), bool WIN = false, typename AfterPrologue>
 __device__ __forceinline__ void mainloop_l(const GemmParams& p, char* smem, int n0, int m0, int kt0, int nkt,
                                            f32x4 (&acc)[FI][FJ], BlockStamps& bs, AfterPrologue after_prologue) {
     static_assert(NS >= 3 && NL >= 1, "loader-wave ring: at least 3 stages and one loader wave");
@@ -1617,7 +1622,7 @@
     const int nktot = p.K / TK;
     if (wraw < NL) {
         const int lw = wraw;
-        const int last_wt = ((p.N + 127) >> 7) - 1, last_rt = (p.M - 1) >> 7;
+        const int last_wt = ((p.N + 127) >> 7) - 1, last_rt = ((WIN ? p.win.total_rows : p.M) - 1) >> 7;
         const unsigned voff = (unsigned)lane * 16u;
         const unsigned smem0 = lds_offset(smem);
         const char* sb[G];
@@ -1629,7 +1634,10 @@
             q = q < NP ? q : NP - 1;
             const bool isw = q < WPC;
             wmask |= (unsigned)isw << i;
-            const int row = isw ? n0 + 8 * q : m0 + 8 * (q - WPC);
+            int row = isw ? n0 + 8 * q : m0 + 8 * (q - WPC);
+            if constexpr (WIN) {
+                if (!isw) row = p.win.row(row < p.M ? row : p.M - 8);
+            }
             int rt = row >> 7;
             const int lim = isw ? last_wt : last_rt;
             rt = rt < lim ? rt : lim;
@@ -1775,9 +1783,10 @@
     }
 }
 
-template <int EPIX, int NS, int FI, int FJ, int WN, int WM, int NL>
+template <int EPIX, int NS, int FI, int FJ, int WN, int WM, int NL, bool WIN = false>
 __global__ __launch_bounds__(64 * (WN * WM + NL), 1) void gemm_l_kernel(GTAV_HEAD_PARAMS, GemmParams p) {
     constexpr int EPI = epi_base(EPIX);
+    static_assert(!WIN || (EPIX == EPI_PARTIAL || EPIX == EPI_GELU_TANH || EPIX == EPI_F32), "a live-row window: split-K slabs, the GELU operand image or plain fp32 rows");
     constexpr int TNB = 16 * FI * WN, TM = 16 * FJ * WM;
     constexpr int STAGE = (2 * FI * WN + 2 * FJ * WM) * 1024;
     constexpr int PNB = (TNB / 8 + 7) / 8 * 8 * 16, PTB = (TM / 8 + 7) / 8 * 8 * 16;
@@ -1834,9 +1843,9 @@
         epilogue<EPIX, FI, FJ, WM, WN, NL, true>(p, acc, pbias, smem, n0, m0, ks, tr, xpre, ft);
     } else {
         auto pf = [&]() { pin_args(); prefetch_bias<EPI, FI, WM, WN, NL>(p, n0, pbias); pff(); };
-        mainloop_l<false, NS, FI, FJ, WN, WM, NL>(p, smem, n0, m0, kt0, nkt, acc, bs, pf);
+        mainloop_l<false, NS, FI, FJ, WN, WM, NL, FI, (FI * FJ >= 16), WIN>(p, smem, n0, m0, kt0, nkt, acc, bs, pf);
         GTAV_STAMP(bs.t[2]);
-        epilogue<EPIX, FI, FJ, WM, WN, NL, false>(p, acc, pbias, smem, n0, m0, ks, tr, acc, ft);
+        epilogue<EPIX, FI, FJ, WM, WN, NL, false, WIN>(p, acc, pbias, smem, n0, m0, ks, tr, acc, ft);
     }
     bs.template end<true>(p);
 }
@@ -2310,15 +2319,15 @@
     GTAV_CHECK_HIP(hipGetLastError());
     return 0;
 }
-template <int EPI, int SHAPE>
+template <int EPI, int SHAPE, bool WIN = false>
 static int launch_l(const GemmParams& p, const GemmPlan& plan, hipStream_t stream) {
     constexpr GemmShape R = *gemm_shape(SHAPE);
     static_assert(R.family == GF_L, "gemm_l_kernel");
-    if (int rc_ = lds_opt_in<gemm_l_kernel<EPI, R.ns, R.fi, R.fj, R.wn, R.wm, R.nl>>(R.ring_bytes())) return rc_;
+    if (int rc_ = lds_opt_in<gemm_l_kernel<EPI, R.ns, R.fi, R.fj, R.wn, R.wm, R.nl, WIN>>(R.ring_bytes())) return rc_;
     GemmParams q = p;
     if (int rc_ = fill_tile_map(q.tm, p.M, p.N, R.tokens(), R.features(), plan.splitk, plan.gn)) return rc_;
     GTAV_REQUIRE(q.splitk >= 0 && q.splitk < 256, "gemm: %d K slices do not fit the launch-head arguments", q.splitk);
-    GTAV_LAUNCH((gemm_l_kernel<EPI, R.ns, R.fi, R.fj, R.wn, R.wm, R.nl>), dim3(plan.blocks), dim3(R.threads()), R.ring_bytes(), stream, GTAV_HEAD_VALUES(q), q);
+    GTAV_LAUNCH((gemm_l_kernel<EPI, R.ns, R.fi, R.fj, R.wn, R.wm, R.nl, WIN>), dim3(plan.blocks), dim3(R.threads()), R.ring_bytes(), stream, GTAV_HEAD_VALUES(q), q);
     GTAV_CHECK_HIP(hipGetLastError());
     return 0;
 }
@@ -2381,6 +2390,17 @@
     return 0;
 }
 
+template <int EPI>
+static int launch_live_rows(const GemmParams& p, const GemmPlan& plan, hipStream_t stream) {
+    static_assert(EPI == EPI_PARTIAL || EPI == EPI_GELU_TANH || EPI == EPI_F32, "gemm_plan_live_rows: the epilogues that take a window");
+    if (plan.shape == 20) return launch_l<EPI, 20, true>(p, plan, stream);
+    if (plan.shape == 24) return launch_l<EPI, 24, true>(p, plan, stream);
+    if (plan.shape == 26) return launch_l<EPI, 26, true>(p, plan, stream);
+    if (plan.shape == 29) return launch_l<EPI, 29, true>(p, plan, stream);
+    GTAV_REQUIRE(false, "gemm/live rows: block shape %d takes no row window", plan.shape);
+    return 0;
+}
+
 bool gemm_qkvt_attn_ok(int M, int D, int S, int Tq, int t0) {
     static const int max_blocks = GTAV_ENV_INT("GTAV_QKVT_MAX_BLOCKS", 256);
     return Tq == 5 && t0 == 0 && S % 16 == 0 && D % 64 == 0 && M % (Tq * S) == 0 && (M / 80) * (D / 64) <= max_blocks;
@@ -2526,6 +2546,14 @@
         if (epi == EPI_PARTIAL) GTAV_REQUIRE(p.splitk >= 1 && (p.K / TK) % p.splitk == 0, "gemm/partial: splitk=%d must divide K/64=%d", p.splitk, p.K / TK);
     }
     GemmPlan plan;
+    const bool live_rows = p.win.segs != 0;
+    if (live_rows) {
+        GTAV_REQUIRE(row_window_ok(p.win) && p.M == p.win.rows(), "gemm: bad live-row window (first %d, %d segments of %d rows every %d, of %d rows; M=%d): rows in whole groups of 8 inside the buffer",
+                     p.win.first, p.win.segs, p.win.seg_rows, p.win.seg_stride, p.win.total_rows, p.M);
+        GTAV_REQUIRE(epi_x == EPI_PARTIAL || epi_x == EPI_GELU_TANH || epi_x == EPI_F32, "gemm: epilogue %d takes no live-row window", epi_x);
+        GTAV_REQUIRE(!p.out2 && !p.gate, "gemm: a live-row window takes no second output and no gate");
+        if (int rc_ = gemm_plan_live_rows(GemmProblem{p.M, p.N, p.K, epi_x, p.qkv_mode, p.S, p.splitk, 0}, &plan)) return rc_;
+    } else
     if (int rc_ = gemm_plan(GemmProblem{p.M, p.N, p.K, epi_x, p.qkv_mode, p.S, p.splitk, p.gate ? p.rows_per_gate : 0}, &plan)) return rc_;
     if (fold_c || fold_p) {
         const int span = gemm_shape(plan.shape)->span();
@@ -2536,6 +2564,11 @@
     lab_fields(p, 3 | 16 | 32 | 2048 | 8192 | 16384 | 0x1F0000);
     p.out_sc1 = (dbg & 8) ? 0 : 1;
     if (dbg & 0x800000) p.pf.next = nullptr;
+    if (live_rows) {
+        if (epi_x == EPI_PARTIAL) return launch_live_rows<EPI_PARTIAL>(p, plan, stream);
+        if (epi_x == EPI_GELU_TANH) return launch_live_rows<EPI_GELU_TANH>(p, plan, stream);
+        return launch_live_rows<EPI_F32>(p, plan, stream);
+    }
     switch (epi_x) {
 #ifdef GTAV_EXPERIMENTS
         case EPI_RESID_FOLD: return launch_epi<EPI_RESID_FOLD>(p, plan, stream);
diff --git a/ai-generated-gtav_amd/csrc/gemm_plan.h b/ai-generated-gtav_amd/csrc/gemm_plan.h
--- a/ai-generated-gtav_amd/csrc/gemm_plan.h
+++ b/ai-generated-gtav_amd/csrc/gemm_plan.h
@@ -74,6 +74,8 @@
 constexpr bool GEMM_LAB_BUILD = GTAV_LAB_BUILD;
 
 int gemm_plan(const GemmProblem& g, GemmPlan* plan, bool lab = GEMM_LAB_BUILD);
+constexpr int GEMM_LIVE_ROW_SHAPES[] = {20, 24, 26, 29};
+int gemm_plan_live_rows(const GemmProblem& g, GemmPlan* plan, bool lab = GEMM_LAB_BUILD);
 int gemm_choose_gn(int M, int N, int K, int tmb, int tnb, int splitk, bool lab = GEMM_LAB_BUILD);
 bool gemm_pp_ok(int M, int N, int K, int epi, bool lab = GEMM_LAB_BUILD);
 bool gemm_resid_inplace_ok(int M, int N, int K, int rows_per_gate, bool lab = GEMM_LAB_BUILD);
diff --git a/ai-generated-gtav_amd/csrc/gemm_plan.hip b/ai-generated-gtav_amd/csrc/gemm_plan.hip
--- a/ai-generated-gtav_amd/csrc/gemm_plan.hip
+++ b/ai-generated-gtav_amd/csrc/gemm_plan.hip
@@ -161,4 +161,28 @@
     return 0;
 }
 
+int gemm_plan_live_rows(const GemmProblem& g, GemmPlan* plan, bool lab) {
+    const int splitk = g.epi == EPI_PARTIAL ? g.splitk : 1;
+    GTAV_REQUIRE(g.M > 0 && g.N > 0 && g.K > 0 && g.K % GEMM_TK == 0 && splitk >= 1 && (g.K / GEMM_TK) % splitk == 0, "gemm/live rows: bad M=%d N=%d K=%d splitk=%d", g.M, g.N, g.K, splitk);
+    GTAV_REQUIRE(g.epi == EPI_PARTIAL || g.epi == EPI_GELU_TANH || g.epi == EPI_F32, "gemm/live rows: epilogue %d takes no row window", g.epi);
+    auto takes = [](int shape) {
+        for (int s : GEMM_LIVE_ROW_SHAPES)
+            if (s == shape) return true;
+        return false;
+    };
+    int wm = forced_shape(lab);
+    if (!takes(wm)) wm = heuristic_shape(g, splitk, lab);
+    if (!takes(wm)) {
+        long long best = -1;
+        for (int s : GEMM_LIVE_ROW_SHAPES) {
+            const long long c = (long long)cdiv(gemm_tiles(s, g.M, g.N) * splitk, 256) * (gemm_shape(s)->features() + gemm_shape(s)->tokens());
+            if (best < 0 || c < best) best = c, wm = s;
+        }
+    }
+    const GemmShape* s = gemm_shape(wm);
+    const int gn = gemm_choose_gn(g.M, g.N, g.K, s->tokens(), s->features(), splitk, lab);
+    *plan = GemmPlan{wm, s->ns, splitk, gn, s->tokens(), s->features(), gemm_tiles(wm, g.M, g.N) * splitk, s->threads()};
+    return 0;
 }
+
+}
diff --git a/ai-generated-gtav_amd/csrc/gemm_typed.inc b/ai-generated-gtav_amd/csrc/gemm_typed.inc
--- a/ai-generated-gtav_amd/csrc/gemm_typed.inc
+++ b/ai-generated-gtav_amd/csrc/gemm_typed.inc
@@ -43,8 +43,9 @@
     float* sk_ws;
     int* sk_flags;
     int sk_dp, sk_r;
+    RowWindow win;
 };
-static_assert(sizeof(GemmParams) == 352, "GemmParams: every build and both operand types must see the same struct");
+static_assert(sizeof(GemmParams) == 376,"GemmParams: every build and both operand types must see the same struct");
 
 struct GemmGroup { const f16* X; const f16* W; float* out; const float* bias; int N; int ldo; };
 int launch_gemm_grouped(const GemmGroup* groups_dev, int n_groups, int max_N, int M, int K, hipStream_t stream);
diff --git a/ai-generated-gtav_amd/csrc/ops.h b/ai-generated-gtav_amd/csrc/ops.h
--- a/ai-generated-gtav_amd/csrc/ops.h
+++ b/ai-generated-gtav_amd/csrc/ops.h
@@ -29,6 +29,10 @@
 
 int launch_unpatchify(const float* y, int ldy, float* img, int NB, int C, int H, int W, int p, int order, float a,
                       float b, hipStream_t stream);
+int launch_unpatchify_frames(const float* y, int ldy, float* img, int n, int f0, int fstep, int C, int H, int W, int p, int order, float a, float b,
+                             hipStream_t stream);
+
+int launch_poison_dead_rows(void* buf, int elem_bytes, int tiled, int ld, const RowWindow& win, hipStream_t stream);
 
 int launch_copy_f32_strided(const float* src, int lds, int R, int C, float* dst, int ldd, hipStream_t stream);
 int launch_copy_rows_f32(const float* src, size_t src_stride, float* dst, size_t dst_stride, int rows, size_t n, hipStream_t stream);
diff --git a/ai-generated-gtav_amd/csrc/ops_bf16.h b/ai-generated-gtav_amd/csrc/ops_bf16.h
--- a/ai-generated-gtav_amd/csrc/ops_bf16.h
+++ b/ai-generated-gtav_amd/csrc/ops_bf16.h
@@ -4,6 +4,7 @@
 namespace gtav_bf16 {
 typedef __bf16 f16;
 using gtav_shared::PrefetchDesc;
+using gtav_shared::RowWindow;
 #include "gemm_typed.inc"
 #include "ops_typed.inc"
 }
@@ -13,6 +14,7 @@
 #define GTAV_OPERAND_OPS(F)                                 \
     F(gemm, launch_gemm)                                    \
     F(ln_modulate, launch_ln_modulate)                      \
+    F(ln_modulate_rows, launch_ln_modulate_rows)            \
     F(ln_affine, launch_ln_affine)                          \
     F(patchify, launch_patchify)                            \
     F(convert_pad, launch_convert_pad_f16)                  \
diff --git a/ai-generated-gtav_amd/csrc/ops_typed.inc b/ai-generated-gtav_amd/csrc/ops_typed.inc
--- a/ai-generated-gtav_amd/csrc/ops_typed.inc
+++ b/ai-generated-gtav_amd/csrc/ops_typed.inc
@@ -24,6 +24,8 @@
 
 int launch_ln_modulate(float* x, int ldx, f16* out, int ldo, int M, int D, const float* shift, const float* scale,
                        int mod_stride, const int* rows, int rows_per_mod, const LnPending* pend, int* err_flag, hipStream_t stream);
+int launch_ln_modulate_rows(float* x, int ldx, f16* out, int ldo, int M, int D, const float* shift, const float* scale,
+                            int mod_stride, const int* rows, int rows_per_mod, const LnPending* pend, const RowWindow* win, int* err_flag, hipStream_t stream);
 int launch_ln_affine(float* x, int ldx, f16* out, int ldo, int M, int D, const float* gamma, const float* beta,
                      const LnPending* pend, int* err_flag, hipStream_t stream);
 int launch_branch_rows(const float* parts, int nsplit, size_t slab_stride, int ld, const float* bias, f16* y, int M, int N, int* err_flag, hipStream_t stream);
diff --git a/ai-generated-gtav_amd/lib.py b/ai-generated-gtav_amd/lib.py
--- a/ai-generated-gtav_amd/lib.py
+++ b/ai-generated-gtav_amd/lib.py
@@ -91,6 +91,8 @@
     "gtav_dit_set_fused_temporal": [_p, _i],
     "gtav_dit_set_fused_spatial": [_p, _i],
     "gtav_dit_fused_launches": [_p, _i, _i, _i],
+    "gtav_dit_set_live_rows": [_p, _i],
+    "gtav_dit_poison_dead_rows": [_p, _i, _i, _p],
     "gtav_dit_set_weight_prefetch": [_p, _i],
     "gtav_dit_set_weight_fill_policy": [_p, _i],
     "gtav_dit_profile": [_p, _i],
@@ -151,6 +153,9 @@
     "gtav_op_gemm_splitk_ln": [_p, _i, _p, _p, _i, _i, _i, _i, _p, _p, _p, _i, _i, _p, _p, _p, _i, _p],
     "gtav_op_gemm_choose_splitk": [_i, _i, _i],
     "gtav_op_gemm_plan": [_i, _i, _i, _i, _i, _i, _i, _i, _p],
+    "gtav_op_gemm_live_rows": [_p, _p, _p, _p, _i, _i, _i, _i, _i, _i, _i, _i, _i, _i, _p],
+    "gtav_op_ln_live_rows": [_p, _p, _i, _p, _p, _i, _i, _p, _i, _l, _p, _p, _i, _i, _i, _i, _i, _i, _i, _p, _p],
+    "gtav_op_gemm_plan_live_rows": [_i, _i, _i, _i, _i, _p],
     "gtav_op_gemm_resid_inplace": [_i, _i, _i],
     "gtav_op_gemm_set_stages": [_i],
     "gtav_op_gemm_set_wm": [_i],
diff --git a/ai-generated-gtav_amd/model/dit.py b/ai-generated-gtav_amd/model/dit.py
--- a/ai-generated-gtav_amd/model/dit.py
+++ b/ai-generated-gtav_amd/model/dit.py
@@ -264,6 +264,8 @@
                     _lib.check(L.gtav_dit_set_fused_temporal(self._handle, 1))
                 if getattr(self, "_fused_spatial", None) is not None:
                     _lib.check(L.gtav_dit_set_fused_spatial(self._handle, int(self._fused_spatial)))
+                if getattr(self, "_live_rows", None) is not None:
+                    _lib.check(L.gtav_dit_set_live_rows(self._handle, int(self._live_rows)))
                 if getattr(self, "_fold", None) is not None:
                     _lib.check(L.gtav_dit_set_fold(self._handle, *self._fold))
                 if getattr(self, "_weight_prefetch", None) is not None:
@@ -587,6 +589,11 @@
         if self._handle:
             _lib.check(_lib.load().gtav_dit_set_fused_spatial(self._handle, int(self._fused_spatial)))
 
+    def set_live_rows(self, enable: bool):
+        self._live_rows = bool(enable)
+        if self._handle:
+            _lib.check(_lib.load().gtav_dit_set_live_rows(self._handle, int(self._live_rows)))
+
     def fused_launches(self, B: int, T: int, t0: int = 0) -> int:
         self._ensure(B, T)
         return int(_lib.load().gtav_dit_fused_launches(self._handle, int(B), int(T), int(t0)))
diff --git a/include/gtav_amd.h b/include/gtav_amd.h
--- a/include/gtav_amd.h
+++ b/include/gtav_amd.h
@@ -42,6 +42,8 @@
 int gtav_dit_set_fused_temporal(gtav_dit* h, int32_t enable);
 
 int gtav_dit_set_fused_spatial(gtav_dit* h, int32_t enable);
+int gtav_dit_set_live_rows(gtav_dit* h, int32_t enable);
+int gtav_dit_poison_dead_rows(gtav_dit* h, int32_t B, int32_t T, void* stream);
 int gtav_dit_fused_launches(gtav_dit* h, int32_t B, int32_t T, int32_t t0);
 
 int gtav_dit_set_weight_prefetch(gtav_dit* h, int32_t mode);
@@ -185,6 +187,13 @@
                            int32_t gate_stride, int32_t rows_per_gate, void* out_f16_dev, const float* shift_dev,
                            const float* scale_dev, int32_t mod_stride, void* stream);
 int gtav_op_gemm_choose_splitk(int32_t M, int32_t N, int32_t K);
+int gtav_op_gemm_live_rows(const void* x_dev, const void* w_dev, const float* bias_dev, void* out_dev, int32_t ldo, int32_t N, int32_t K, int32_t epilogue,
+                           int32_t splitk, int32_t first, int32_t seg_rows, int32_t seg_stride, int32_t segs, int32_t total_rows, void* stream);
+int gtav_op_ln_live_rows(float* x_dev, void* out_dev, int32_t D, const float* shift_dev, const float* scale_dev, int32_t mod_stride, int32_t rows_per_mod,
+                         const float* parts_dev, int32_t nsplit, int64_t slab_stride, const float* bias_dev, const float* gate_dev, int32_t gate_stride,
+                         int32_t rows_per_gate, int32_t first, int32_t seg_rows, int32_t seg_stride, int32_t segs, int32_t total_rows, int32_t* err_dev,
+                         void* stream);
+int gtav_op_gemm_plan_live_rows(int32_t M, int32_t N, int32_t K, int32_t epilogue, int32_t splitk, int32_t* plan8);
 int gtav_op_gemm_plan(int32_t M, int32_t N, int32_t K, int32_t epilogue, int32_t qkv_mode, int32_t S, int32_t splitk, int32_t rows_per_gate, int32_t* plan8);
 int gtav_op_gemm_resid_inplace(int32_t M, int32_t N, int32_t K);
 int gtav_op_convert_f16(const float* src_dev, int32_t lds, int32_t R, int32_t C, void* dst_f16_dev, int32_t Rp,
```
